# Jittor/PointCloudLib

Measured on AMD Instinct MI355X. Metric: point-clouds/sec fwd+bwd, PointNet++ SSG B=32 N=1024, higher is better.
Workload: dtype f32; 1 GPU; PointNet++ SSG cls train step (fwd+bwd+SGD), B=32/GPU, N=1024 xyz+normal, gauss_ball clouds (BASELINE configs[1]); global_batch=32, n_points=1024, parallelism=dp1, launch=eager, grad_overlap=False, cpu_affinity=numa node 1 (gpu0), 128 cpus, world_size=1, sync_bn=False, entry_points=per-stack (pcl_mlp_stack_*_f32)

## Files before the change

### include/pcl_hip.h

```cpp
#ifndef PCL_HIP_H
#define PCL_HIP_H

#include <stddef.h>
#include <stdint.h>

#ifdef __cplusplus
extern "C" {
#endif

#define PCL_OK 0
#define PCL_EINVAL (-1)
#define PCL_EHIP (-2)
#define PCL_ENOSUP (-3)
#define PCL_EWS (-4)

int pcl_version(void);
void pcl_time_tagged_launch(void* start_event, void* stop_event, const char* tag);
void pcl_time_next_launch(void* start_event, void* stop_event);
const char* pcl_last_launch_kernel(void);
const char* pcl_last_error(void);

int pcl_optimal_block(int batch_size);

void pcl_set_fps_tuning(int threads_per_cloud, int issue_priority);
int pcl_fps_f32(const float* xyz, int B, int N, int m, int tie_stride, double skip_sqnorm_le,
                const int32_t* start_idx, int32_t* idx_out, float* new_xyz_out, void* stream);

int pcl_fps_ragged_f32(const float* xyz, const int32_t* n_valid, int B, int N, int m, int tie_stride, double skip_sqnorm_le,
                       const int32_t* start_idx, int32_t* idx_out, float* new_xyz_out, void* stream);

int pcl_ball_query_f32(const float* new_xyz, const float* xyz, int B, int m, int N, float radius,
                       int nsample, int32_t* idx_out, int32_t* cnt_out, void* stream);
int pcl_ball_query_multi_f32(const float* new_xyz, const float* xyz, int B, int m, int N, int n_radii, const float* radii,
                             const int32_t* nsamples, int32_t* const* idx_out, int32_t* const* cnt_out, void* stream);
int pcl_ball_query_ragged_f32(const float* new_xyz, const float* xyz, const int32_t* n_valid, int B, int m, int N, float radius,
                              int nsample, int32_t* idx_out, int32_t* cnt_out, void* stream);
int pcl_ball_query_multi_ragged_f32(const float* new_xyz, const float* xyz, const int32_t* n_valid, int B, int m, int N, int n_radii,
                                    const float* radii, const int32_t* nsamples, int32_t* const* idx_out, int32_t* const* cnt_out,
                                    void* stream);

int pcl_group_f32(const float* xyz, const float* new_xyz, const float* feat, const int32_t* idx,
                  int B, int N, int m, int ns, int C, int use_xyz, float* out, void* stream);
int pcl_group_bwd_f32(const float* gout, const int32_t* idx, int B, int N, int m, int ns, int C,
                      int use_xyz, float* gfeat, void* stream);
int pcl_group_all_f32(const float* xyz, const float* feat, int B, int N, int C, int use_xyz,
                      float* out, void* stream);
int pcl_group_all_bwd_f32(const float* gout, int B, int N, int C, int use_xyz, float* gfeat,
                          void* stream);
int pcl_gather_rows_f32(const float* src, const int32_t* idx, int B, int N, int M, int C, float* out,
                        void* stream);
int pcl_gather_rows_bwd_f32(const float* gout, const int32_t* idx, int B, int N, int M, int C,
                            float* gsrc, void* stream);

int pcl_edge_feature_f32(const float* x, const int32_t* idx, int B, int N, int k, int C, float* out, void* stream);
int pcl_edge_feature_bwd_f32(const float* gout, const int32_t* idx, int B, int N, int k, int C, float* gx,
                             void* stream);

size_t pcl_knn_workspace_bytes(int B, int C, int Nr, int Nq, int k);
int pcl_knn_f32(const float* ref, const float* qry, int B, int C, int Nr, int Nq, int k,
                int32_t* idx_out, void* workspace, size_t workspace_bytes, void* stream);
int pcl_knn_nk_supported(int Nr);
int pcl_knn_nk_f32(const float* ref, const float* qry, int B, int C, int Nr, int Nq, int k, int32_t* idx_out, void* stream);
int pcl_knn_fma_f32(const float* ref, const float* qry, int B, int C, int Nr, int Nq, int k,
                    int32_t* idx_out, void* workspace, size_t workspace_bytes, void* stream);
int pcl_knn_point_matmul_f32(const float* xyz, const float* new_xyz, int B, int N, int S, int k, int fma_dot, int32_t* idx_out,
                             void* stream);

int pcl_three_nn_f32(const float* xyz1, const float* xyz2, int B, int N, int S, int32_t* idx3,
                     float* w3, void* stream);
int pcl_three_nn_ragged_f32(const float* xyz1, const int32_t* n1_valid, const float* xyz2, const int32_t* n2_valid, int B, int N,
                            int S, int32_t* idx3, float* w3, void* stream);
int pcl_three_interp_f32(const float* points2, const int32_t* idx3, const float* w3, int B, int N,
                         int S, int D, float* out, void* stream);
int pcl_three_interp_bwd_f32(const float* gout, const int32_t* idx3, const float* w3, int B, int N,
                             int S, int D, float* gpoints2, void* stream);

int pcl_density_f32(const float* xyz, int B, int N, float bandwidth, float* density_out, void* stream);

int pcl_group_linear_stat_rows(int B, int m);
int pcl_group_linear_f32(const float* xyz, const float* new_xyz, const float* Uf, const float* Wx, const float* feat_small,
                         const float* Wf_small, int CF, int ldw, const int32_t* idx, const int32_t* cnt, const int32_t* group_off,
                         int B, int N, int m, int ns, int C1, float* Y, int32_t* row_meta, int32_t* row_src,
                         float* row_loc , float* row_feat ,
                         double* stats_ws, void* stream);
int pcl_group_linear_bwd_f32(const float* row_loc, const float* row_feat, int CF, const float* dU, const float* Y,
                             const float* a, const float* k1, const float* k2, const float* mu, const int32_t* row_src,
                             const int32_t* n_rows_dev , int B, int N, int C1, float* dUf,
                             float* dWx_part, float* dWf_part, float* dW0, int ldw, int off, void* stream);
int pcl_group_rows_transpose_supported(int N, int m, int ns);
int pcl_group_rows_transpose_i32(const int32_t* row_src, const int32_t* group_off, int B, int N, int m, int ns, int32_t* in_off,
                                 int32_t* in_rows, void* stream);
int pcl_group_linear_bwd_gather_supported(int C1);
void pcl_set_pointconv_paths(int bwd_w_rows);
void pcl_set_scatter_form(int gather);
int pcl_group_linear_bwd_gather_f32(const float* row_loc, const float* dU, const float* Y, const float* a, const float* k1,
                                    const float* k2, const float* mu, const int32_t* in_off, const int32_t* in_rows, int B, int N,
                                    int C1, float* dUf, float* dWx_part, float* dW0, int ldw, void* stream);
int pcl_group_linear_bwd_regen_supported(int C1, int CF);
int pcl_group_linear_bwd_regen_f32(const float* row_loc, const float* row_feat, const float* Wx, const float* Wf_small, int CF, int ldw,
// ... 144 lines not shown
                            const int32_t* arg, const float* gz, int ns, const float* W, const float* Xprev,
                            const float* prev_scale, const float* prev_shift, float prev_slope, int masked, int P, int Cout, int Cin,
                            float* dUprev, double* stats_ws, int first_col, void* workspace, size_t workspace_bytes, void* stream);
int pcl_linear_bwd_pair_finish_f32(const void* workspace, size_t workspace_bytes, int P, int Cout, int Cin, float* dW, int dw_ld,
                                   const double* stats_ws, int stat_rows, const float* gamma_prev, const float* mean_prev,
                                   const float* invstd_prev, int P_bn, float* dgamma_prev, float* dbeta_prev,
                                   float* a_prev, float* k1_prev, float* k2_prev, float* dbias_zero_prev, void* stream);
void pcl_set_bwd_pair(int on);
int pcl_get_bwd_pair(void);
void pcl_set_matrix_form(int form);
int pcl_get_matrix_form(void);
int pcl_linear_bwd_fused_supported(int Cout, int Cin);
int pcl_linear_bwd_fused_stat_rows(int P, int Cin);
size_t pcl_linear_bwd_fused_workspace_bytes(int P, int Cout, int Cin);
int pcl_linear_bwd_fused_rows_f32(const float* dU, const float* Y, const float* a, const float* k1, const float* k2, const float* mu,
                                  const int32_t* arg, const float* gz, int ns, const float* W, int P, int Cout, int Cin,
                                  const float* Yprev, const float* prev_scale, const float* prev_shift, float prev_slope,
                                  float* dUprev, double* stats_ws, void* workspace, size_t workspace_bytes,
                                  const int32_t* row_meta, const int32_t* n_rows_dev, void* stream);
int pcl_linear_bwd_fused_finish_f32(const void* workspace, size_t workspace_bytes, int P, int Cout, int Cin, float* dW,
                                    const double* stats_ws, const float* gamma_prev, const float* mean_prev,
                                    const float* invstd_prev, int P_bn, float* dgamma_prev, float* dbeta_prev, float* a_prev,
                                    float* k1_prev, float* k2_prev, float* dbias_zero_prev, void* stream);
size_t pcl_linear_bwd_dw_workspace_bytes(int P, int Cout, int Cin);
int pcl_linear_bwd_dw_f32(const float* dU, const float* Y, const float* a, const float* k1, const float* k2, const float* mu,
                          const int32_t* arg, const float* gz, int ns, const float* Xprev,
                          const float* prev_scale, const float* prev_shift, float prev_slope, int P, int Cout,
                          int Cin, float* dW, void* workspace, size_t workspace_bytes, void* stream);

#define PCL_STACK_MAX_LAYERS 8
typedef struct pcl_stack_layer_t {
    const float* W;
    const float* bias;
    const float* gamma;
    const float* beta;
    float* running_mean;
    float* running_var;
    float* dW;
    float* dbias;
    float* dgamma;
    float* dbeta;
} pcl_stack_layer_t;
typedef struct pcl_mlp_stack_t {
    int32_t struct_bytes;
    int32_t n_layers;
    int32_t c[PCL_STACK_MAX_LAYERS + 1];
    int32_t P;
    int32_t pool;
    int32_t grouped;
    int32_t x_grad_from;
    int32_t need_dx;
    int32_t B, N, m, Cf, use_xyz;
    float slope, out_slope, eps, momentum;
    const float* x;
    const float* xyz;
    const float* new_xyz;
    const float* feature;
    float* Wf_dense;
    const int32_t* idx;
    const int32_t* cnt;
    const int32_t* group_off;
    pcl_stack_layer_t layer[PCL_STACK_MAX_LAYERS];
    float* out;
    void* save;
    size_t save_bytes;
    void* tmp;
    size_t tmp_bytes;
    const float* gout;
    float* dx;
    void* stream;
    int32_t defer_act;
    int32_t ext_stat_rows;
    const double* ext_stats;
    int32_t flush_k;
    int32_t gout_ld;
} pcl_mlp_stack_t;
int pcl_mlp_stack_last(const pcl_mlp_stack_t* desc, size_t* y_offset, size_t* scale_offset, size_t* shift_offset);
int pcl_mlp_stack_sizes(const pcl_mlp_stack_t* desc, size_t* save_bytes, size_t* fwd_tmp_bytes, size_t* bwd_tmp_bytes);
int pcl_mlp_stack_fwd_f32(const pcl_mlp_stack_t* desc);
int pcl_mlp_stack_bwd_f32(const pcl_mlp_stack_t* desc);

int pcl_frag_stat_rows(int P);
int pcl_frag_max_rows(void);
void pcl_frag_set_tuning(int max_rows, int force_tn, int force_ksw, int dw_tm, int dw_tn, int dw_ksw, int dw_ksg);
int pcl_frag_linear_fwd_f32(const float* X, int ldx, const float* W, int ldw, const float* bias, const float* in_scale,
                            const float* in_shift, float in_slope, int P, int Cin, int Cout, float* Y, int ldy,
                            float* Y_lo , double* stats_ws,
                            int flush_k, void* stream);
int pcl_frag_dy_f32(const float* dU, const float* Y, const float* a, const float* k1, const float* k2, const float* mu,
                    const int32_t* arg, const float* gz, int ns, int P, int C, float* dy, uint32_t* zero_words, int n_zero, void* stream);
int pcl_frag_linear_bwd_dx_f32(const float* dy, const float* W, int ldw, int P, int Cout, int Cin, const float* Yprev, int ldyp,
                               const float* prev_scale, const float* prev_shift, float prev_slope, float* dUprev, int ldu,
                               double* stats_ws, int first_col, void* stream);
size_t pcl_frag_dw_workspace_bytes(int P, int Cout, int Cin);
int pcl_frag_dw_counter_words(int P, int Cout, int Cin);
int pcl_frag_linear_bwd_dw_f32(const float* dy, const float* X, int ldx, const float* prev_scale, const float* prev_shift, float prev_slope,
                               int P, int Cout, int Cin, float* dW, int ldo, void* workspace, size_t workspace_bytes, int counters_cleared,
                               void* stream);

int pcl_group_offsets_i32(const int32_t* cnt, int G, int32_t* group_off, void* stream);
int pcl_group_offsets_multi_i32(int n, const int32_t* const* cnt, int G, int32_t* const* group_off, void* stream);
int pcl_group_compact_f32(const float* xyz, const float* new_xyz, const float* feat, const int32_t* idx,
                          const int32_t* cnt, const int32_t* group_off, int B, int N, int m, int ns, int C, int use_xyz,
                          int row_stride , float* rows,
                          int32_t* row_meta, int32_t* row_src, void* stream);
int pcl_linear_fwd_rows_f32(const float* X, const float* W, const float* bias, const float* in_scale,
                            const float* in_shift, float in_slope, int P, int Cin, int Cout, float* Y,
                            double* stats_ws, const int32_t* row_meta, const int32_t* n_rows_dev, void* stream);
int pcl_bn_act_max_rows_f32(const float* Y, const int32_t* group_off, const float* scale, const float* shift,
                            float slope, int G, int C, float* out, int32_t* arg, float* ymax, void* stream);
int pcl_linear_bwd_dx_rows_f32(const float* dU, const float* Y, const float* a, const float* k1, const float* k2, const float* mu,
                               const int32_t* arg, const float* gz, int ns, const float* W, int P, int Cout,
                               int Cin, const float* Yprev, const float* prev_scale, const float* prev_shift,
                               float prev_slope, float* dUprev, double* stats_ws, const int32_t* row_meta,
                               const int32_t* n_rows_dev, int first_col ,
                               int cin_stride , void* stream);
int pcl_linear_bwd_dw_rows_f32(const float* dU, const float* Y, const float* a, const float* k1, const float* k2, const float* mu,
                               const int32_t* arg, const float* gz, int ns, const float* Xprev,
                               const float* prev_scale, const float* prev_shift, float prev_slope, int P, int Cout,
                               int Cin, float* dW, void* workspace, size_t workspace_bytes, const int32_t* row_meta,
                               const int32_t* n_rows_dev, int dw_ld, void* stream);
int pcl_scatter_rows_add_f32(const float* grows, const int32_t* row_src, const int32_t* n_rows_dev, int rows_cap,
                             int D, int off, int C, int n_dst_rows, float* gfeat, void* stream);

int pcl_xconv_core_supported(int K, int dm, int C);
int pcl_xconv_core_partials(int R, int C);
int pcl_xconv_core_fwd_f32(const float* X, const float* F1, int C1, const float* F2, int C2, const float* wd, const float* bias,
                           int R, int K, int dm, float* D, void* stream);
int pcl_xconv_core_bwd_f32(const float* X, const float* F1, int C1, const float* F2, int C2, const float* wd, const float* dD,
                           int R, int K, int dm, float* dX, float* dF1, float* dF2, float* dwd_part, float* dbias_part,
// ... 57 lines not shown
```

### pointcloudlib_amd/csrc/group.hip

```cpp
#include "common.h"

namespace pcl {

__device__ __forceinline__ int in_cloud(int k, int N) { return min(max(k, 0), N - 1); }

constexpr int GT = 256;

__global__ __launch_bounds__(GT) void group_fwd_kernel(const float* __restrict__ xyz, const float* __restrict__ new_xyz,
                                                       const float* __restrict__ feat, const int32_t* __restrict__ idx,
                                                       int N, int m, int ns, int C, int use_xyz, size_t total,
                                                       float* __restrict__ out) {
    const int D = (use_xyz ? 3 : 0) + C;
    const int off = use_xyz ? 3 : 0;
    for (size_t g = (size_t)blockIdx.x * GT + threadIdx.x; g < total; g += (size_t)gridDim.x * GT) {
        const size_t row = g / D;
        const int c = (int)(g - row * D);
        const size_t bj = row / ns;
        const size_t b = bj / m;
        const int k = in_cloud(idx[row], N);
        float v;
        if (c < off) v = __fsub_rn(xyz[(b * N + k) * 3 + c], new_xyz[bj * 3 + c]);
        else v = feat[(b * N + k) * C + (c - off)];
        out[g] = v;
    }
}

__global__ __launch_bounds__(GT) void group_bwd_kernel(const float* __restrict__ gout, const int32_t* __restrict__ idx,
                                                       int N, int m, int ns, int C, int use_xyz, size_t total,
                                                       float* __restrict__ gfeat) {
    const int D = (use_xyz ? 3 : 0) + C;
    const int off = use_xyz ? 3 : 0;
    for (size_t g = (size_t)blockIdx.x * GT + threadIdx.x; g < total; g += (size_t)gridDim.x * GT) {
        const size_t row = g / C;
        const int c = (int)(g - row * C);
        const size_t b = row / ((size_t)m * ns);
        const int k = in_cloud(idx[row], N);
        unsafeAtomicAdd(&gfeat[(b * N + k) * C + c], gout[row * D + off + c]);
    }
}

__global__ __launch_bounds__(GT) void group_all_kernel(const float* __restrict__ xyz, const float* __restrict__ feat,
                                                       int C, int use_xyz, size_t total, float* __restrict__ out) {
    const int D = (use_xyz ? 3 : 0) + C;
    const int off = use_xyz ? 3 : 0;
    for (size_t g = (size_t)blockIdx.x * GT + threadIdx.x; g < total; g += (size_t)gridDim.x * GT) {
        const size_t p = g / D;
        const int c = (int)(g - p * D);
        out[g] = c < off ? xyz[p * 3 + c] : feat[p * C + (c - off)];
    }
}

__global__ __launch_bounds__(GT) void group_all_bwd_kernel(const float* __restrict__ gout, int C, int use_xyz,
                                                           size_t total, float* __restrict__ gfeat) {
    const int D = (use_xyz ? 3 : 0) + C;
    const int off = use_xyz ? 3 : 0;
    for (size_t g = (size_t)blockIdx.x * GT + threadIdx.x; g < total; g += (size_t)gridDim.x * GT) {
        const size_t p = g / C;
        const int c = (int)(g - p * C);
        gfeat[g] = gout[p * D + off + c];
    }
}

__global__ __launch_bounds__(GT) void gather_rows_kernel(const float* __restrict__ src, const int32_t* __restrict__ idx,
                                                         int N, int M, int C, size_t total, float* __restrict__ out) {
    for (size_t g = (size_t)blockIdx.x * GT + threadIdx.x; g < total; g += (size_t)gridDim.x * GT) {
        const size_t row = g / C;
        const int c = (int)(g - row * C);
        const size_t b = row / M;
        out[g] = src[(b * N + in_cloud(idx[row], N)) * C + c];
    }
}

__global__ __launch_bounds__(GT) void gather_rows_bwd_kernel(const float* __restrict__ gout, const int32_t* __restrict__ idx,
                                                             int N, int M, int C, size_t total, float* __restrict__ gsrc) {
    for (size_t g = (size_t)blockIdx.x * GT + threadIdx.x; g < total; g += (size_t)gridDim.x * GT) {
        const size_t row = g / C;
        const int c = (int)(g - row * C);
        const size_t b = row / M;
        unsafeAtomicAdd(&gsrc[(b * N + in_cloud(idx[row], N)) * C + c], gout[g]);
    }
}


__global__ __launch_bounds__(GT) void edge_feature_kernel(const float* __restrict__ x, const int32_t* __restrict__ idx,
                                                          int N, int k, int C, size_t total, float* __restrict__ out) {
    const int D = 2 * C;
    for (size_t g = (size_t)blockIdx.x * GT + threadIdx.x; g < total; g += (size_t)gridDim.x * GT) {
        const size_t row = g / D;
        const int c = (int)(g - row * D);
        const size_t bn = row / k;
        const size_t b = bn / N;
        if (c < C) out[g] = __fsub_rn(x[(b * N + in_cloud(idx[row], N)) * C + c], x[bn * C + c]);
        else out[g] = x[bn * C + (c - C)];
    }
}

__global__ __launch_bounds__(GT) void edge_feature_bwd_center_kernel(const float* __restrict__ gout, int k, int C,
                                                                     size_t total, float* __restrict__ gx) {
    const int D = 2 * C;
    for (size_t g = (size_t)blockIdx.x * GT + threadIdx.x; g < total; g += (size_t)gridDim.x * GT) {
        const size_t bn = g / C;
        const int c = (int)(g - bn * C);
        const float* base = gout + bn * k * D;
        float s = 0.f;
// ... 9 lines not shown
        const size_t row = g / C;
        const int c = (int)(g - row * C);
        const size_t b = row / ((size_t)N * k);
        unsafeAtomicAdd(&gx[(b * N + in_cloud(idx[row], N)) * C + c], gout[row * D + c]);
    }
}

static inline int grid_for(size_t total) {
    size_t blocks = (total + GT - 1) / GT;
    if (blocks > 256 * 16) blocks = 256 * 16;
    if (blocks < 1) blocks = 1;
    return (int)blocks;
}

}
using namespace pcl;

extern "C" int pcl_group_f32(const float* xyz, const float* new_xyz, const float* feat, const int32_t* idx, int B,
                             int N, int m, int ns, int C, int use_xyz, float* out, void* stream) {
    PCL_REQUIRE(idx && out, "pcl_group_f32: null pointer");
    PCL_REQUIRE(!use_xyz || (xyz && new_xyz), "pcl_group_f32: use_xyz needs xyz and new_xyz");
    PCL_REQUIRE(C == 0 || feat, "pcl_group_f32: C=%d needs feat", C);
    PCL_REQUIRE(B >= 0 && N >= 1 && m >= 0 && ns >= 1 && C >= 0 && (use_xyz || C > 0), "pcl_group_f32: bad sizes");
    const size_t total = (size_t)B * m * ns * ((use_xyz ? 3 : 0) + C);
    if (!total) return PCL_OK;
    hipLaunchKernelGGL(group_fwd_kernel, dim3(grid_for(total)), dim3(GT), 0, as_stream(stream), xyz, new_xyz, feat, idx,
                       N, m, ns, C, use_xyz, total, out);
    return check_launch("pcl_group_f32");
}

extern "C" int pcl_group_bwd_f32(const float* gout, const int32_t* idx, int B, int N, int m, int ns, int C,
                                 int use_xyz, float* gfeat, void* stream) {
    PCL_REQUIRE(gout && idx && gfeat, "pcl_group_bwd_f32: null pointer");
    PCL_REQUIRE(B >= 0 && N >= 1 && m >= 0 && ns >= 1 && C >= 1, "pcl_group_bwd_f32: bad sizes");
    hipStream_t st = as_stream(stream);
    if ((size_t)B * N * C) {
        hipError_t e = hipMemsetAsync(gfeat, 0, sizeof(float) * (size_t)B * N * C, st);
        if (e != hipSuccess) return fail(PCL_EHIP, "pcl_group_bwd_f32: memset: %s", hipGetErrorString(e));
    }
    const size_t total = (size_t)B * m * ns * C;
    if (!total) return PCL_OK;
    hipLaunchKernelGGL(group_bwd_kernel, dim3(grid_for(total)), dim3(GT), 0, st, gout, idx, N, m, ns, C, use_xyz, total, gfeat);
    return check_launch("pcl_group_bwd_f32");
}

extern "C" int pcl_group_all_f32(const float* xyz, const float* feat, int B, int N, int C, int use_xyz, float* out,
                                 void* stream) {
    PCL_REQUIRE(out && (!use_xyz || xyz) && (C == 0 || feat), "pcl_group_all_f32: null pointer");
    PCL_REQUIRE(B >= 0 && N >= 0 && C >= 0 && (use_xyz || C > 0), "pcl_group_all_f32: bad sizes");
    const size_t total = (size_t)B * N * ((use_xyz ? 3 : 0) + C);
    if (!total) return PCL_OK;
    hipLaunchKernelGGL(group_all_kernel, dim3(grid_for(total)), dim3(GT), 0, as_stream(stream), xyz, feat, C, use_xyz, total, out);
    return check_launch("pcl_group_all_f32");
}

extern "C" int pcl_group_all_bwd_f32(const float* gout, int B, int N, int C, int use_xyz, float* gfeat, void* stream) {
    PCL_REQUIRE(gout && gfeat && C >= 1 && B >= 0 && N >= 0, "pcl_group_all_bwd_f32: bad arguments");
    const size_t total = (size_t)B * N * C;
    if (!total) return PCL_OK;
    hipLaunchKernelGGL(group_all_bwd_kernel, dim3(grid_for(total)), dim3(GT), 0, as_stream(stream), gout, C, use_xyz, total, gfeat);
    return check_launch("pcl_group_all_bwd_f32");
}

extern "C" int pcl_gather_rows_f32(const float* src, const int32_t* idx, int B, int N, int M, int C, float* out,
                                   void* stream) {
    PCL_REQUIRE(src && idx && out && B >= 0 && N >= 1 && M >= 0 && C >= 1, "pcl_gather_rows_f32: bad arguments");
    const size_t total = (size_t)B * M * C;
    if (!total) return PCL_OK;
    hipLaunchKernelGGL(gather_rows_kernel, dim3(grid_for(total)), dim3(GT), 0, as_stream(stream), src, idx, N, M, C, total, out);
    return check_launch("pcl_gather_rows_f32");
}

extern "C" int pcl_gather_rows_bwd_f32(const float* gout, const int32_t* idx, int B, int N, int M, int C, float* gsrc,
                                       void* stream) {
    PCL_REQUIRE(gout && idx && gsrc && B >= 0 && N >= 1 && M >= 0 && C >= 1, "pcl_gather_rows_bwd_f32: bad arguments");
    hipStream_t st = as_stream(stream);
    if ((size_t)B * N * C) {
        hipError_t e = hipMemsetAsync(gsrc, 0, sizeof(float) * (size_t)B * N * C, st);
        if (e != hipSuccess) return fail(PCL_EHIP, "pcl_gather_rows_bwd_f32: memset: %s", hipGetErrorString(e));
    }
    const size_t total = (size_t)B * M * C;
    if (!total) return PCL_OK;
    hipLaunchKernelGGL(gather_rows_bwd_kernel, dim3(grid_for(total)), dim3(GT), 0, st, gout, idx, N, M, C, total, gsrc);
    return check_launch("pcl_gather_rows_bwd_f32");
}

extern "C" int pcl_edge_feature_f32(const float* x, const int32_t* idx, int B, int N, int k, int C, float* out, void* stream) {
    PCL_REQUIRE(x && idx && out && B >= 0 && N >= 1 && k >= 1 && C >= 1, "pcl_edge_feature_f32: bad arguments");
    const size_t total = (size_t)B * N * k * 2 * C;
    if (!total) return PCL_OK;
    hipLaunchKernelGGL(edge_feature_kernel, dim3(grid_for(total)), dim3(GT), 0, as_stream(stream), x, idx, N, k, C, total, out);
    return check_launch("pcl_edge_feature_f32");
}

extern "C" int pcl_edge_feature_bwd_f32(const float* gout, const int32_t* idx, int B, int N, int k, int C, float* gx,
                                        void* stream) {
    PCL_REQUIRE(gout && idx && gx && B >= 0 && N >= 1 && k >= 1 && C >= 1, "pcl_edge_feature_bwd_f32: bad arguments");
    hipStream_t st = as_stream(stream);
    const size_t tc = (size_t)B * N * C;
    if (!tc) return PCL_OK;
    hipLaunchKernelGGL(edge_feature_bwd_center_kernel, dim3(grid_for(tc)), dim3(GT), 0, st, gout, k, C, tc, gx);
    int rc = check_launch("pcl_edge_feature_bwd_f32(center)");
    if (rc) return rc;
    const size_t tn = tc * k;
    hipLaunchKernelGGL(edge_feature_bwd_nbr_kernel, dim3(grid_for(tn)), dim3(GT), 0, st, gout, idx, N, k, C, tn, gx);
    return check_launch("pcl_edge_feature_bwd_f32(nbr)");
// ... 2 lines not shown
```

### pointcloudlib_amd/csrc/mlp.hip

```cpp
#include <cstdlib>
#include "common.h"
#if defined(__HIP_DEVICE_COMPILE__) && !defined(__gfx950__)
#error "mlp.hip is written for gfx950 (MI355X) only: its buffer addressing relies on the range check covering the scalar offset (tools/ubench/bufcheck.hip)"
#endif

#ifndef PCL_EXP
#define PCL_EXP 0
#endif

namespace pcl {

typedef float f32x16 __attribute__((ext_vector_type(16)));

constexpr int BK = 32, LDS_LD = BK + 4;
constexpr int MLP_T = 256;
constexpr int STAT_ROWS = 1024;

enum AMode { A_PLAIN = 0, A_BNACT = 1, A_DY = 2, A_DY_SPARSE = 3 };
enum EMode { E_STORE_STATS = 0, E_MASK_STORE_STATS = 1, E_STORE = 2 };

struct LinArgs {
    const float* A;
    const float* A2;
    int ldb;
// ... 813 lines not shown
                    if (lh == 0 && cin && row0 < p.M) {
                        const size_t o = (size_t)(row0 / GM) * p.N + col;
                        p.gmax[o] = vmax; p.gmin[o] = vmin; p.gamax[o] = imax; p.gamin[o] = imin;
                    }
                }
            }
        }
    }

    if constexpr (EM != E_STORE) {
        __syncthreads();
        double* red = reinterpret_cast<double*>(sA);
#pragma unroll
        for (int tn = 0; tn < TN; ++tn) {
            double s = st_s[tn], q = st_q[tn];
            s += __shfl_xor(s, 32); q += __shfl_xor(q, 32);
            if (lh == 0) { red[((wave * TN + tn) * 32 + lr) * 2 + 0] = s; red[((wave * TN + tn) * 32 + lr) * 2 + 1] = q; }
        }
        __syncthreads();
        if (tid < TBN) {
            const int c = tid, wcc = c / (32 * TN), tn = (c >> 5) % TN, l = c & 31;
            const int col = n0 + c;
            if (col < p.N) {
                double s = 0.0, q = 0.0;
#pragma unroll
                for (int w = 0; w < 2; ++w) {
                    const int wv = w * 2 + wcc;
                    s += red[((wv * TN + tn) * 32 + l) * 2 + 0]; q += red[((wv * TN + tn) * 32 + l) * 2 + 1];
                }
                double* dst = p.stats + (size_t)bx * 2 * p.N;
                dst[col] = s; dst[p.N + col] = q;
            }
        }
    }
}
template <int AM, int EM, bool VEC, int TN, int GM, bool RAG, int TM = 2, bool SP = false>
__global__ __launch_bounds__(MLP_T, 2) void linear_nt_kernel(const LinArgs p_in) {
    linear_nt_body<AM, EM, VEC, TN, GM, RAG, TM, SP>(p_in, (int)blockIdx.x);
}

struct DwArgs {
    const float* A; const float* A2;
    const float* sc; const float* sh; const float* k2; const float* mu;
    const int32_t* arg; const float* gz; int ns;
    const float* Bsrc; const float* bsc; const float* bsh;
    float bslope;
    float* part;
    const int* p_dev;
    const int2* rmeta;
    int P, I, J;
    int a_mode, b_mode;
    int gx, ti, tj;
    int ldo;
};

constexpr int DW_BP = 32;

template <bool VEC, int W>
struct DwStage {
    static constexpr int CPR = VEC ? W / 4 : W;
    static constexpr int RP = MLP_T / CPR;
    static constexpr int NI = DW_BP / RP;
    float4 v[VEC ? NI : 1], v2[VEC ? NI : 1], vg[VEC ? NI : 1];
    int4 vi[VEC ? NI : 1];
    float s[VEC ? 1 : NI], s2[VEC ? 1 : NI], sg[VEC ? 1 : NI];
    int si[VEC ? 1 : NI];
    float rw[NI];
    int rs[NI];
    int2 raw[NI];
    int p0;
};

template <bool VEC, int W, bool RAG>
__device__ __forceinline__ void dw_fetch_meta(const DwArgs& p, int p0, int tid, DwStage<VEC, W>& st) {
    using S = DwStage<VEC, W>;
    if constexpr (RAG) {
#pragma unroll
        for (int i = 0; i < S::NI; ++i) st.raw[i] = p.rmeta[min(p0 + tid / S::CPR + S::RP * i, p.P - 1)];
    }
}

template <int AM, bool VEC, int W, bool RAG>
__device__ __forceinline__ void dw_load_a(const DwArgs& p, int p0, int c0, int tid, DwStage<VEC, W>& st) {
    using S = DwStage<VEC, W>;
    st.p0 = p0;
    const int c = min(c0 + (tid % S::CPR) * (VEC ? 4 : 1), p.I - (VEC ? 4 : 1));
#pragma unroll
    for (int i = 0; i < S::NI; ++i) {
        const int r = min(p0 + tid / S::CPR + S::RP * i, p.P - 1);
        const size_t off = (size_t)r * p.I + c;
        int g = 0, srow = 0;
        float w = 1.f;
        if constexpr (RAG) row_meta(st.raw[i], g, srow, w);
        else if constexpr (AM == A_DY_SPARSE) { g = r / p.ns; srow = r - g * p.ns; }
        st.rw[i] = w; st.rs[i] = srow;
        if constexpr (AM == A_PLAIN) {
            if constexpr (VEC) st.v[i] = *reinterpret_cast<const float4*>(p.A + off);
            else st.s[i] = p.A[off];
        } else if constexpr (VEC) {
            st.v2[i] = *reinterpret_cast<const float4*>(p.A2 + off);
            if constexpr (AM == A_DY) st.v[i] = *reinterpret_cast<const float4*>(p.A + off);
            else {
                const size_t go = (size_t)g * p.I + c;
                st.vi[i] = *reinterpret_cast<const int4*>(p.arg + go);
                st.vg[i] = *reinterpret_cast<const float4*>(p.gz + go);
            }
// ... 8 lines not shown
        }
    }
}

template <int AM, bool VEC, int W>
__device__ __forceinline__ void dw_store_a(const DwArgs& p, float* sX, int c0, int tid, const DwStage<VEC, W>& st,
                                           float4 sc, float4 sh, float4 k2, float4 mu) {
    using S = DwStage<VEC, W>;
    const int cl = (tid % S::CPR) * (VEC ? 4 : 1);
    const bool cin = c0 + cl < p.I;
#pragma unroll
    for (int i = 0; i < S::NI; ++i) {
        const int rl = tid / S::CPR + S::RP * i;
        const int r = st.p0 + rl;
        const bool in = cin && r < p.P;
        if constexpr (AM == A_PLAIN) {
            if constexpr (VEC) *reinterpret_cast<float4*>(&sX[rl * (W + 4) + cl]) = in ? st.v[i] : make_float4(0, 0, 0, 0);
            else sX[rl * (W + 4) + cl] = in ? st.s[i] : 0.f;
        } else if constexpr (VEC) {
            float4 a = make_float4(0, 0, 0, 0);
            if (in) {
                float4 du;
                if constexpr (AM == A_DY) du = st.v[i];
                else {
                    const int srow = st.rs[i];
                    const int4 ar = st.vi[i];
                    const float4 gz = st.vg[i];
                    du.x = ar.x == srow ? gz.x : 0.f; du.y = ar.y == srow ? gz.y : 0.f;
                    du.z = ar.z == srow ? gz.z : 0.f; du.w = ar.w == srow ? gz.w : 0.f;
                }
                const float4 y = st.v2[i];
                const float w = st.rw[i];
                a.x = fmaf(sc.x, du.x, -w * fmaf(k2.x, y.x - mu.x, sh.x)); a.y = fmaf(sc.y, du.y, -w * fmaf(k2.y, y.y - mu.y, sh.y));
                a.z = fmaf(sc.z, du.z, -w * fmaf(k2.z, y.z - mu.z, sh.z)); a.w = fmaf(sc.w, du.w, -w * fmaf(k2.w, y.w - mu.w, sh.w));
            }
            *reinterpret_cast<float4*>(&sX[rl * (W + 4) + cl]) = a;
        } else {
            float a = 0.f;
            if (in) {
                float du;
                if constexpr (AM == A_DY) du = st.s[i];
                else du = st.si[i] == st.rs[i] ? st.sg[i] : 0.f;
                a = fmaf(sc.x, du, -st.rw[i] * fmaf(k2.x, st.s2[i] - mu.x, sh.x));
            }
            sX[rl * (W + 4) + cl] = a;
        }
    }
}

template <bool VEC, int W>
__device__ __forceinline__ void dw_load_b(const DwArgs& p, int p0, int c0, int tid, DwStage<VEC, W>& st) {
    using S = DwStage<VEC, W>;
    st.p0 = p0;
    const int c = min(c0 + (tid % S::CPR) * (VEC ? 4 : 1), p.J - (VEC ? 4 : 1));
#pragma unroll
    for (int i = 0; i < S::NI; ++i) {
        const int r = min(p0 + tid / S::CPR + S::RP * i, p.P - 1);
        const size_t off = (size_t)r * p.J + c;
        if constexpr (VEC) st.v[i] = *reinterpret_cast<const float4*>(p.Bsrc + off);
        else st.s[i] = p.Bsrc[off];
    }
}

template <bool VEC, int W>
__device__ __forceinline__ void dw_store_b(const DwArgs& p, float* sX, int c0, int tid, const DwStage<VEC, W>& st,
                                           float4 sc, float4 sh) {
    using S = DwStage<VEC, W>;
    const int cl = (tid % S::CPR) * (VEC ? 4 : 1);
    const bool cin = c0 + cl < p.J;
    const bool act = p.b_mode == A_BNACT;
#pragma unroll
    for (int i = 0; i < S::NI; ++i) {
        const int rl = tid / S::CPR + S::RP * i;
        const bool in = cin && st.p0 + rl < p.P;
        if constexpr (VEC) {
            float4 b = make_float4(0, 0, 0, 0);
            if (in) {
                b = st.v[i];
                if (act) {
                    b.x = lrelu(fmaf(sc.x, b.x, sh.x), p.bslope); b.y = lrelu(fmaf(sc.y, b.y, sh.y), p.bslope);
                    b.z = lrelu(fmaf(sc.z, b.z, sh.z), p.bslope); b.w = lrelu(fmaf(sc.w, b.w, sh.w), p.bslope);
                }
            }
            *reinterpret_cast<float4*>(&sX[rl * (W + 4) + cl]) = b;
        } else {
            float b = 0.f;
            if (in) { b = st.s[i]; if (act) b = lrelu(fmaf(sc.x, b, sh.x), p.bslope); }
            sX[rl * (W + 4) + cl] = b;
        }
    }
}

template <int AM, bool VEC, int TM, int TN, bool RAG>
__device__ __forceinline__ void linear_dw_body(const DwArgs& p_in, const int block) {
    DwArgs p = p_in;
    if (p.p_dev) p.P = *p.p_dev;
    constexpr int WI = 64 * TM, WJ = 64 * TN;
    __shared__ __attribute__((aligned(16))) float sA[DW_BP * (WI + 4)];
    __shared__ __attribute__((aligned(16))) float sB[DW_BP * (WJ + 4)];
    const int tid = threadIdx.x, lane = tid & 63, wave = tid >> 6;
    const int wr = wave >> 1, wc = wave & 1, lr = lane & 31, lh = lane >> 5;
    int bx, bt;
    tile_of_block(block, p.gx, p.ti * p.tj, bx, bt);
    const int i0 = (bt % p.ti) * WI, j0 = (bt / p.ti) * WJ;
    const int chunks = (p.P + DW_BP - 1) / DW_BP;
    f32x16 acc[TM][TN];
#pragma unroll
    for (int i = 0; i < TM; ++i)
#pragma unroll
        for (int j = 0; j < TN; ++j)
#pragma unroll
// ... 1658 lines not shown
            else PCL_LAUNCH_TIMED((linear_nt_kernel<AM, EM, false, 1, 0, false, 1>), grid, dim3(MLP_T), st, a);
            return check_launch("pcl_linear");
        }
    }
    if (narrow || AM >= A_DY) {
        if (vec) PCL_LAUNCH_TIMED((linear_nt_kernel<AM, EM, true, 1, GM, RAG>), grid, dim3(MLP_T), st, a);
        else if constexpr (AM == A_DY_SPARSE && RAG && GM == 0) {
            PCL_LAUNCH_TIMED((linear_nt_kernel<AM, EM, false, 1, GM, RAG, 1>), grid, dim3(MLP_T), st, a);
        } else PCL_LAUNCH_TIMED((linear_nt_kernel<AM, EM, false, 1, GM, RAG>), grid, dim3(MLP_T), st, a);
    } else {
        if constexpr (AM < A_DY) {
            if (vec) PCL_LAUNCH_TIMED((linear_nt_kernel<AM, EM, true, 2, GM, RAG>), grid, dim3(MLP_T), st, a);
            else PCL_LAUNCH_TIMED((linear_nt_kernel<AM, EM, false, 2, GM, RAG>), grid, dim3(MLP_T), st, a);
        }
    }
    return check_launch("pcl_linear");
}

static int linear_stat_rows(int M, int N, bool bwd, bool rag) {
    int gx, n_tiles; bool narrow, low;
    linear_grid(M, N, bwd, rag, gx, n_tiles, narrow, low);
    return gx;
}

static int launch_linear(const LinArgs& a, hipStream_t st) {
    if (fwd_res_eligible(a)) return launch_fwd_res(a, linear_stat_rows(a.M, a.N, false, a.rmeta != nullptr), st);
    if (a.rmeta) {
        if (a.a_mode == A_PLAIN && a.e_mode == E_STORE_STATS) return launch_linear_t<A_PLAIN, E_STORE_STATS, 0, true>(a, st);
        if (a.a_mode == A_BNACT && a.e_mode == E_STORE_STATS) return launch_linear_t<A_BNACT, E_STORE_STATS, 0, true>(a, st);
        if (a.a_mode == A_DY && a.e_mode == E_MASK_STORE_STATS) return launch_linear_t<A_DY, E_MASK_STORE_STATS, 0, true>(a, st);
        if (a.a_mode == A_DY && a.e_mode == E_STORE) return launch_linear_t<A_DY, E_STORE, 0, true>(a, st);
        if (a.a_mode == A_DY_SPARSE && a.e_mode == E_MASK_STORE_STATS) return launch_linear_t<A_DY_SPARSE, E_MASK_STORE_STATS, 0, true>(a, st);
        if (a.a_mode == A_DY_SPARSE && a.e_mode == E_STORE) return launch_linear_t<A_DY_SPARSE, E_STORE, 0, true>(a, st);
        return fail(PCL_EINVAL, "pcl_linear: unsupported ragged mode combination %d/%d", a.a_mode, a.e_mode);
    }
    if (a.e_mode == E_STORE_STATS && a.gmax) {
        if (a.a_mode == A_PLAIN && a.ns == 64) return launch_linear_t<A_PLAIN, E_STORE_STATS, 64>(a, st);
        if (a.a_mode == A_BNACT && a.ns == 64) return launch_linear_t<A_BNACT, E_STORE_STATS, 64>(a, st);
        if (a.a_mode == A_PLAIN && a.ns == 32) return launch_linear_t<A_PLAIN, E_STORE_STATS, 32>(a, st);
        if (a.a_mode == A_BNACT && a.ns == 32) return launch_linear_t<A_BNACT, E_STORE_STATS, 32>(a, st);
        return fail(PCL_EINVAL, "pcl_linear_fwd_gmax_f32: group size %d not supported (32 or 64)", a.ns);
    }
    if (a.a_mode == A_PLAIN && a.e_mode == E_STORE_STATS) return launch_linear_t<A_PLAIN, E_STORE_STATS>(a, st);
    if (a.a_mode == A_BNACT && a.e_mode == E_STORE_STATS) return launch_linear_t<A_BNACT, E_STORE_STATS>(a, st);
    if (a.a_mode == A_PLAIN && a.e_mode == E_STORE) return launch_linear_t<A_PLAIN, E_STORE>(a, st);
    if (a.a_mode == A_BNACT && a.e_mode == E_STORE) return launch_linear_t<A_BNACT, E_STORE>(a, st);
    if (a.a_mode == A_DY && a.e_mode == E_MASK_STORE_STATS) return launch_linear_t<A_DY, E_MASK_STORE_STATS>(a, st);
    if (a.a_mode == A_DY && a.e_mode == E_STORE) return launch_linear_t<A_DY, E_STORE>(a, st);
    if (a.a_mode == A_DY_SPARSE && a.e_mode == E_MASK_STORE_STATS) return launch_linear_t<A_DY_SPARSE, E_MASK_STORE_STATS>(a, st);
    if (a.a_mode == A_DY_SPARSE && a.e_mode == E_STORE) return launch_linear_t<A_DY_SPARSE, E_STORE>(a, st);
    return fail(PCL_EINVAL, "pcl_linear: unsupported mode combination %d/%d", a.a_mode, a.e_mode);
}

}
using namespace pcl;

extern "C" int pcl_mlp_stat_rows(int P, int C, int flags) {
    if (P < 1 || C < 1) return 1;
    return linear_stat_rows(P, C, (flags & 1) != 0, (flags & 2) != 0);
}

extern "C" int pcl_linear_fwd_rows_f32(const float* X, const float* W, const float* bias, const float* in_scale,
                                       const float* in_shift, float in_slope, int P, int Cin, int Cout, float* Y,
                                       double* stats_ws, const int32_t* row_meta, const int32_t* n_rows_dev, void* stream) {
    PCL_REQUIRE(X && W && Y, "pcl_linear_fwd_f32: null pointer");
    PCL_REQUIRE(stats_ws || !row_meta, "pcl_linear_fwd_rows_f32: the stats-free form (stats_ws NULL) takes plain rows only");
    PCL_REQUIRE(P >= 1 && Cin >= 1 && Cout >= 1, "pcl_linear_fwd_f32: bad sizes P=%d Cin=%d Cout=%d", P, Cin, Cout);
    PCL_REQUIRE((in_scale == nullptr) == (in_shift == nullptr), "pcl_linear_fwd_f32: in_scale/in_shift must come together");
    PCL_REQUIRE((row_meta == nullptr) == (n_rows_dev == nullptr), "pcl_linear_fwd_rows_f32: row_meta and n_rows_dev come together");
    LinArgs a = {};
    a.A = X; a.B = W; a.bias = bias; a.sc = in_scale; a.sh = in_shift; a.slope = in_slope;
    a.C = Y; a.stats = stats_ws; a.M = P; a.N = Cout; a.K = Cin; a.ldc = Cout;
    a.rmeta = reinterpret_cast<const int2*>(row_meta); a.m_dev = n_rows_dev;
    a.a_mode = in_scale ? A_BNACT : A_PLAIN; a.e_mode = stats_ws ? E_STORE_STATS : E_STORE;
    return launch_linear(a, as_stream(stream));
}

extern "C" int pcl_linear_fwd_f32(const float* X, const float* W, const float* bias, const float* in_scale,
                                  const float* in_shift, float in_slope, int P, int Cin, int Cout, float* Y,
                                  double* stats_ws, void* stream) {
    return pcl_linear_fwd_rows_f32(X, W, bias, in_scale, in_shift, in_slope, P, Cin, Cout, Y, stats_ws, nullptr, nullptr, stream);
}

extern "C" int pcl_linear_fwd_gmax_f32(const float* X, const float* W, const float* bias, const float* in_scale,
                                       const float* in_shift, float in_slope, int P, int Cin, int Cout, int ns, float* Y,
                                       double* stats_ws, float* gmax, float* gmin, int32_t* gamax, int32_t* gamin,
                                       void* stream) {
    PCL_REQUIRE(X && W && Y && stats_ws && gmax && gmin && gamax && gamin, "pcl_linear_fwd_gmax_f32: null pointer");
    PCL_REQUIRE(P >= 1 && Cin >= 1 && Cout >= 1 && (ns == 32 || ns == 64) && P % ns == 0,
                "pcl_linear_fwd_gmax_f32: bad sizes P=%d Cin=%d Cout=%d ns=%d (ns must be 32 or 64 and divide P)", P, Cin, Cout, ns);
    PCL_REQUIRE((in_scale == nullptr) == (in_shift == nullptr), "pcl_linear_fwd_gmax_f32: in_scale/in_shift must come together");
    LinArgs a = {};
    a.A = X; a.B = W; a.bias = bias; a.sc = in_scale; a.sh = in_shift; a.slope = in_slope;
    a.C = Y; a.stats = stats_ws; a.M = P; a.N = Cout; a.K = Cin; a.ldc = Cout; a.ns = ns;
    a.gmax = gmax; a.gmin = gmin; a.gamax = gamax; a.gamin = gamin;
    a.a_mode = in_scale ? A_BNACT : A_PLAIN; a.e_mode = E_STORE_STATS;
    return launch_linear(a, as_stream(stream));
}

__global__ __launch_bounds__(256) void group_minmax_finalize_t_kernel(const float* __restrict__ gmax, const float* __restrict__ gmin,
                                                                      const int32_t* __restrict__ gamax, const int32_t* __restrict__ gamin,
                                                                      const float* __restrict__ scale, const float* __restrict__ shift,
                                                                      float slope, int C, int N, int tiles_c, size_t tiles, float* __restrict__ out,
                                                                      int32_t* __restrict__ arg, float* __restrict__ ymax,
                                                                      float* __restrict__ out2, int ld2, float* __restrict__ out_t) {
    __shared__ float tile[32][33];
// ... 23 lines not shown
        const size_t b = g0 / N, n0 = g0 % N;
#pragma unroll
        for (int i = 0; i < 4; ++i) {
            const int cl = ty + 8 * i;
            if (c0 + cl < C) out_t[(b * C + c0 + cl) * (size_t)N + n0 + tx] = tile[tx][cl];
        }
        __syncthreads();
    }
}

extern "C" int pcl_group_minmax_finalize_t_f32(const float* gmax, const float* gmin, const int32_t* gamax, const int32_t* gamin,
                                               const float* scale, const float* shift, float slope, int B, int N, int C, float* out,
                                               int32_t* arg, float* ymax, float* out2, int out2_ld, float* out_t, void* stream) {
    PCL_REQUIRE(gmax && gmin && gamax && gamin && scale && shift && out && arg && ymax && out_t && B >= 1 && N >= 32 && N % 32 == 0 && C >= 1 &&
                (!out2 || out2_ld >= C), "pcl_group_minmax_finalize_t_f32: bad arguments (N a multiple of 32)");
    const int tiles_c = (C + 31) / 32;
    const size_t tiles = (size_t)B * N / 32 * tiles_c;
    const int blocks = tiles < 8192 ? (int)tiles : 8192;
    hipLaunchKernelGGL(group_minmax_finalize_t_kernel, dim3(blocks), dim3(256), 0, as_stream(stream), gmax, gmin, gamax, gamin, scale, shift, slope, C, N,
                       tiles_c, tiles, out, arg, ymax, out2, out2_ld, out_t);
    return check_launch("pcl_group_minmax_finalize_t_f32");
}
extern "C" int pcl_group_minmax_finalize_f32(const float* gmax, const float* gmin, const int32_t* gamax, const int32_t* gamin,
                                             const float* scale, const float* shift, float slope, int G, int C, float* out,
                                             int32_t* arg, float* ymax, void* stream) {
    return pcl_group_minmax_finalize2_f32(gmax, gmin, gamax, gamin, scale, shift, slope, G, C, out, arg, ymax, nullptr, 0, stream);
}
extern "C" int pcl_group_minmax_finalize2_f32(const float* gmax, const float* gmin, const int32_t* gamax, const int32_t* gamin,
                                              const float* scale, const float* shift, float slope, int G, int C, float* out,
                                              int32_t* arg, float* ymax, float* out2, int out2_ld, void* stream) {
    PCL_REQUIRE(gmax && gmin && gamax && gamin && scale && shift && out && arg && ymax && G >= 1 && C >= 1 && (!out2 || out2_ld >= C),
                "pcl_group_minmax_finalize_f32: bad arguments");
    const size_t total = (size_t)G * C;
    int blocks = (int)((total + 255) / 256);
    if (blocks > 4096) blocks = 4096;
    hipLaunchKernelGGL(group_minmax_finalize_kernel, dim3(blocks), dim3(256), 0, as_stream(stream), gmax, gmin, gamax, gamin, scale,
                       shift, slope, C, total, out, arg, ymax, out2, out2_ld);
    return check_launch("pcl_group_minmax_finalize_f32");
}

extern "C" int pcl_linear_bwd_dx_f32(const float* dU, const float* Y, const float* a_, const float* k1, const float* k2, const float* mu,
                                     const int32_t* arg, const float* gz, int ns, const float* W, int P, int Cout,
                                     int Cin, const float* Yprev, const float* prev_scale, const float* prev_shift,
                                     float prev_slope, float* dUprev, double* stats_ws, void* stream) {
    return pcl_linear_bwd_dx_rows_f32(dU, Y, a_, k1, k2, mu, arg, gz, ns, W, P, Cout, Cin, Yprev, prev_scale, prev_shift, prev_slope,
                                      dUprev, stats_ws, nullptr, nullptr, 0, 0, stream);
}

extern "C" int pcl_linear_bwd_dx_rows_f32(const float* dU, const float* Y, const float* a_, const float* k1, const float* k2, const float* mu,
                                          const int32_t* arg, const float* gz, int ns, const float* W, int P, int Cout,
                                          int Cin, const float* Yprev, const float* prev_scale, const float* prev_shift,
                                          float prev_slope, float* dUprev, double* stats_ws, const int32_t* row_meta,
                                          const int32_t* n_rows_dev, int first_col, int cin_stride, void* stream) {
    PCL_REQUIRE(Y && a_ && k1 && k2 && mu && W && dUprev, "pcl_linear_bwd_dx_f32: null pointer");
    PCL_REQUIRE((dU != nullptr) != (arg != nullptr && gz != nullptr), "pcl_linear_bwd_dx_f32: pass dU or (arg,gz)");
    PCL_REQUIRE(P >= 1 && Cin >= 1 && Cout >= 1 && (dU || ns >= 1), "pcl_linear_bwd_dx_f32: bad sizes");
    PCL_REQUIRE(!Yprev || (prev_scale && prev_shift && stats_ws), "pcl_linear_bwd_dx_f32: masked mode needs scale/shift/stats");
    LinArgs a = {};
    a.A = dU; a.A2 = Y; a.B = W; a.sc = a_; a.sh = k1; a.k2 = k2; a.mu = mu; a.arg = arg; a.gz = gz; a.ns = ns;
    a.C = dUprev; a.stats = stats_ws; a.Yprev = Yprev; a.esc = prev_scale; a.esh = prev_shift; a.eslope = prev_slope;
    PCL_REQUIRE(first_col >= 0 && first_col < Cin && (first_col == 0 || !Yprev), "pcl_linear_bwd_dx_rows_f32: first_col=%d only for the input gradient", first_col);
    a.M = P; a.N = Cin; a.K = Cout; a.n_begin = first_col; a.ldc = a.ldb = cin_stride > 0 ? cin_stride : Cin;
    PCL_REQUIRE(a.ldc >= Cin && (a.ldc == Cin || !Yprev), "pcl_linear_bwd_dx_rows_f32: cin_stride=%d", cin_stride);
    a.rmeta = reinterpret_cast<const int2*>(row_meta); a.m_dev = n_rows_dev;
    a.a_mode = dU ? A_DY : A_DY_SPARSE; a.e_mode = Yprev ? E_MASK_STORE_STATS : E_STORE;
    return launch_linear(a, as_stream(stream));
}

extern "C" size_t pcl_linear_bwd_dw_workspace_bytes(int P, int Cout, int Cin) {
    if (P < 1 || Cout < 1 || Cin < 1) return 0;
    int gx, ti, tj, tm, tn;
    dw_grid(P, Cout, Cin, gx, ti, tj, tm, tn);
    return sizeof(float) * (size_t)gx * Cout * Cin;
}

extern "C" int pcl_linear_bwd_dw_f32(const float* dU, const float* Y, const float* a_, const float* k1, const float* k2, const float* mu,
                                     const int32_t* arg, const float* gz, int ns, const float* Xprev,
                                     const float* prev_scale, const float* prev_shift, float prev_slope, int P, int Cout,
                                     int Cin, float* dW, void* workspace, size_t workspace_bytes, void* stream) {
    return pcl_linear_bwd_dw_rows_f32(dU, Y, a_, k1, k2, mu, arg, gz, ns, Xprev, prev_scale, prev_shift, prev_slope, P, Cout, Cin, dW,
                                      workspace, workspace_bytes, nullptr, nullptr, 0, stream);
}

extern "C" int pcl_linear_bwd_dw_rows_f32(const float* dU, const float* Y, const float* a_, const float* k1, const float* k2, const float* mu,
                                          const int32_t* arg, const float* gz, int ns, const float* Xprev,
                                          const float* prev_scale, const float* prev_shift, float prev_slope, int P, int Cout,
                                          int Cin, float* dW, void* workspace, size_t workspace_bytes, const int32_t* row_meta,
                                          const int32_t* n_rows_dev, int dw_ld, void* stream) {
    PCL_REQUIRE(Y && a_ && k1 && k2 && mu && Xprev && dW, "pcl_linear_bwd_dw_f32: null pointer");
    PCL_REQUIRE(dw_ld == 0 || dw_ld >= Cin, "pcl_linear_bwd_dw_f32: dw_ld=%d < Cin=%d", dw_ld, Cin);
    PCL_REQUIRE((dU != nullptr) != (arg != nullptr && gz != nullptr), "pcl_linear_bwd_dw_f32: pass dU or (arg,gz)");
    PCL_REQUIRE((prev_scale == nullptr) == (prev_shift == nullptr), "pcl_linear_bwd_dw_f32: scale/shift together");
    PCL_REQUIRE(P >= 1 && Cin >= 1 && Cout >= 1 && (dU || ns >= 1), "pcl_linear_bwd_dw_f32: bad sizes");
    const size_t need = pcl_linear_bwd_dw_workspace_bytes(P, Cout, Cin);
    if (!workspace || workspace_bytes < need) return fail(PCL_EWS, "pcl_linear_bwd_dw_f32: workspace %zu < %zu", workspace_bytes, need);
    hipStream_t st = as_stream(stream);
    int gx, ti, tj, tm, tn;
    dw_grid(P, Cout, Cin, gx, ti, tj, tm, tn);
    DwArgs d = {};
    d.A = dU; d.A2 = Y; d.sc = a_; d.sh = k1; d.k2 = k2; d.mu = mu; d.arg = arg; d.gz = gz; d.ns = ns;
    d.Bsrc = Xprev; d.bsc = prev_scale; d.bsh = prev_shift; d.bslope = prev_slope;
    d.part = static_cast<float*>(workspace); d.P = P; d.I = Cout; d.J = Cin;
    d.rmeta = reinterpret_cast<const int2*>(row_meta); d.p_dev = n_rows_dev;
    d.a_mode = dU ? A_DY : A_DY_SPARSE; d.b_mode = prev_scale ? A_BNACT : A_PLAIN;
    const bool vec = (Cout % 4 == 0) && (Cin % 4 == 0) && al16(Y, Xprev, dU) && (!gz || al16(gz, arg));
    d.gx = gx; d.ti = ti; d.tj = tj; d.ldo = Cin;
    const bool direct = gx == 1;
    if (direct) { d.part = dW; d.ldo = dw_ld ? dw_ld : Cin; }
    dim3 grid(gx * ti * tj);
    if (dU) { if (vec) launch_dw_t<A_DY, true>(d, grid, tm, tn, st); else launch_dw_t<A_DY, false>(d, grid, tm, tn, st); }
    else { if (vec) launch_dw_t<A_DY_SPARSE, true>(d, grid, tm, tn, st); else launch_dw_t<A_DY_SPARSE, false>(d, grid, tm, tn, st); }
    int rc = check_launch("pcl_linear_bwd_dw_f32");
    if (rc || direct) return rc;
    const size_t n = (size_t)Cout * Cin;
    const int blocks = (int)((n + 31) / 32);
    hipLaunchKernelGGL(reduce_rows_kernel, dim3(blocks), dim3(256), 0, st, d.part, gx, n, Cin, dw_ld ? dw_ld : Cin, dW);
    return check_launch("pcl_linear_bwd_dw_f32(reduce)");
}

extern "C" int pcl_linear_bwd_pair_supported(int P, int Cout, int Cin, int first_col) {
    if (!g_lab.bwd_pair || P < 1 || Cout <= 64 || Cin <= 64 || (g_lab.split_mfma & 2)) return 0;
    int gx, ti, tj, tm, tn;
    dw_grid(P, Cout, Cin, gx, ti, tj, tm, tn);
    if (gx == 1 || tm != 2 || tn != 2) return 0;
    int gxl, n_tiles; bool narrow, low;
    linear_grid(P, Cin - first_col, true, false, gxl, n_tiles, narrow, low);
    return low ? 1 : 0;
}

extern "C" int pcl_linear_bwd_pair_f32(const float* dU, const float* Y, const float* a_, const float* k1, const float* k2, const float* mu,
                                       const int32_t* arg, const float* gz, int ns, const float* W, const float* Xprev,
                                       const float* prev_scale, const float* prev_shift, float prev_slope, int masked, int P, int Cout, int Cin,
                                       float* dUprev, double* stats_ws, int first_col, void* workspace, size_t workspace_bytes, void* stream) {
    PCL_REQUIRE(Y && a_ && k1 && k2 && mu && W && Xprev && dUprev, "pcl_linear_bwd_pair_f32: null pointer");
    PCL_REQUIRE((dU != nullptr) != (arg != nullptr && gz != nullptr), "pcl_linear_bwd_pair_f32: pass dU or (arg,gz)");
    PCL_REQUIRE((prev_scale == nullptr) == (prev_shift == nullptr), "pcl_linear_bwd_pair_f32: scale/shift together");
    PCL_REQUIRE(!masked || (prev_scale && stats_ws), "pcl_linear_bwd_pair_f32: masked mode needs scale/shift/stats");
    PCL_REQUIRE(first_col >= 0 && first_col < Cin && (first_col == 0 || !masked), "pcl_linear_bwd_pair_f32: first_col=%d only for the input gradient", first_col);
    PCL_REQUIRE(pcl_linear_bwd_pair_supported(P, Cout, Cin, first_col), "pcl_linear_bwd_pair_f32: shape P=%d Cout=%d Cin=%d not eligible", P, Cout, Cin);
    const size_t need = pcl_linear_bwd_dw_workspace_bytes(P, Cout, Cin);
    if (!workspace || workspace_bytes < need) return fail(PCL_EWS, "pcl_linear_bwd_pair_f32: workspace %zu < %zu", workspace_bytes, need);
    hipStream_t st = as_stream(stream);
    int gx, ti, tj, tm, tn;
    dw_grid(P, Cout, Cin, gx, ti, tj, tm, tn);
    DwArgs d = {};
    d.A = dU; d.A2 = Y; d.sc = a_; d.sh = k1; d.k2 = k2; d.mu = mu; d.arg = arg; d.gz = gz; d.ns = ns;
    d.Bsrc = Xprev; d.bsc = prev_scale; d.bsh = prev_shift; d.bslope = prev_slope;
    d.part = static_cast<float*>(workspace); d.P = P; d.I = Cout; d.J = Cin;
    d.a_mode = dU ? A_DY : A_DY_SPARSE; d.b_mode = prev_scale ? A_BNACT : A_PLAIN;
    d.gx = gx; d.ti = ti; d.tj = tj; d.ldo = Cin;
    LinArgs a = {};
    a.A = dU; a.A2 = Y; a.B = W; a.sc = a_; a.sh = k1; a.k2 = k2; a.mu = mu; a.arg = arg; a.gz = gz; a.ns = ns;
    a.C = dUprev; a.stats = stats_ws; a.Yprev = masked ? Xprev : nullptr; a.esc = prev_scale; a.esh = prev_shift; a.eslope = prev_slope;
    a.M = P; a.N = Cin; a.K = Cout; a.n_begin = first_col; a.ldc = a.ldb = Cin;
    a.a_mode = d.a_mode; a.e_mode = masked ? E_MASK_STORE_STATS : E_STORE;
    int gxl, n_tiles; bool narrow, low;
    linear_grid(P, Cin - first_col, true, false, gxl, n_tiles, narrow, low);
    a.gx = gxl; a.nt = n_tiles;
    const bool vec_dw = (Cout % 4 == 0) && (Cin % 4 == 0) && al16(Y, Xprev, dU) && (!gz || al16(gz, arg));
    const bool vec_nt = (a.K % 4 == 0) && al16(a.A, a.B, a.A2) && a.ldb % 4 == 0;
    const int n_dw = gx * ti * tj;
    if (vec_dw != vec_nt) {
        if (dU) { if (vec_dw) launch_dw_t<A_DY, true>(d, dim3(n_dw), tm, tn, st); else launch_dw_t<A_DY, false>(d, dim3(n_dw), tm, tn, st); }
        else { if (vec_dw) launch_dw_t<A_DY_SPARSE, true>(d, dim3(n_dw), tm, tn, st); else launch_dw_t<A_DY_SPARSE, false>(d, dim3(n_dw), tm, tn, st); }
        if (const int rc = check_launch("pcl_linear_bwd_pair_f32(dw)")) return rc;
        return launch_linear(a, st);
    }
    const bool vec = vec_dw;
    const dim3 grid(n_dw + gxl * n_tiles), blk(MLP_T);
#define PCL_PAIR(AMv, EMv, VECv) PCL_LAUNCH_TIMED((linear_bwd_pair_kernel<AMv, EMv, VECv>), grid, blk, st, d, a, n_dw)
    if (dU) {
        if (masked) { if (vec) PCL_PAIR(A_DY, E_MASK_STORE_STATS, true); else PCL_PAIR(A_DY, E_MASK_STORE_STATS, false); }
        else { if (vec) PCL_PAIR(A_DY, E_STORE, true); else PCL_PAIR(A_DY, E_STORE, false); }
    } else {
        if (masked) { if (vec) PCL_PAIR(A_DY_SPARSE, E_MASK_STORE_STATS, true); else PCL_PAIR(A_DY_SPARSE, E_MASK_STORE_STATS, false); }
        else { if (vec) PCL_PAIR(A_DY_SPARSE, E_STORE, true); else PCL_PAIR(A_DY_SPARSE, E_STORE, false); }
    }
#undef PCL_PAIR
    return check_launch("pcl_linear_bwd_pair_f32");
}

namespace pcl {
int pair_finish_impl(const void* workspace, size_t workspace_bytes, int P, int Cout, int Cin, float* dW, int dw_ld,
                     const double* stats_ws, int stat_rows, const float* gamma_prev, const float* mean_prev,
                     const float* invstd_prev, int P_bn, float* dgamma_prev, float* dbeta_prev,
                     float* a_prev, float* k1_prev, float* k2_prev, float* dbias_zero_prev, void* stream,
                     const float* xpart, int xrows, int xC1, int xld, float* xdW0);
}
extern "C" int pcl_linear_bwd_pair_finish_f32(const void* workspace, size_t workspace_bytes, int P, int Cout, int Cin, float* dW, int dw_ld,
                                              const double* stats_ws, int stat_rows, const float* gamma_prev, const float* mean_prev,
                                              const float* invstd_prev, int P_bn, float* dgamma_prev, float* dbeta_prev,
                                              float* a_prev, float* k1_prev, float* k2_prev, float* dbias_zero_prev, void* stream) {
    return pair_finish_impl(workspace, workspace_bytes, P, Cout, Cin, dW, dw_ld, stats_ws, stat_rows, gamma_prev, mean_prev, invstd_prev, P_bn, dgamma_prev,
                            dbeta_prev, a_prev, k1_prev, k2_prev, dbias_zero_prev, stream, nullptr, 0, 0, 0, nullptr);
}
int pcl::pair_finish_impl(const void* workspace, size_t workspace_bytes, int P, int Cout, int Cin, float* dW, int dw_ld,
                          const double* stats_ws, int stat_rows, const float* gamma_prev, const float* mean_prev,
                          const float* invstd_prev, int P_bn, float* dgamma_prev, float* dbeta_prev,
                          float* a_prev, float* k1_prev, float* k2_prev, float* dbias_zero_prev, void* stream,
                          const float* xpart, int xrows, int xC1, int xld, float* xdW0) {
    PCL_REQUIRE(workspace && dW && P >= 1 && Cout >= 1 && Cin >= 1 && (dw_ld == 0 || dw_ld >= Cin), "pcl_linear_bwd_pair_finish_f32: bad arguments");
    const size_t need = pcl_linear_bwd_dw_workspace_bytes(P, Cout, Cin);
    if (workspace_bytes < need) return fail(PCL_EWS, "pcl_linear_bwd_pair_finish_f32: workspace %zu < %zu", workspace_bytes, need);
    int gx, ti, tj, tm, tn;
    dw_grid(P, Cout, Cin, gx, ti, tj, tm, tn);
    BnConstsArgs q = {};
    int extra = 0;
    if (stats_ws) {
        PCL_REQUIRE(mean_prev && invstd_prev && a_prev && k1_prev && k2_prev && P_bn >= 1 && stat_rows >= 1, "pcl_linear_bwd_pair_finish_f32: null pointer");
        q = BnConstsArgs{stats_ws, stat_rows, gamma_prev, mean_prev, invstd_prev, P_bn, Cin, dgamma_prev, dbeta_prev, a_prev, k1_prev, k2_prev, dbias_zero_prev};
        extra = (Cin + 3) / 4;
    }
    const size_t n = (size_t)Cout * Cin;
    const int nred = (int)((n + 31) / 32);
    FinishXJob xj = {nullptr, 0, 0, 0, nullptr, 0};
    int xblocks = 0;
    if (xpart && xdW0) { xj = FinishXJob{xpart, xrows, xC1, xld, xdW0, nred + extra}; xblocks = (xC1 * 3 + 3) / 4; }
    hipLaunchKernelGGL(fused_finish_kernel, dim3(nred + extra + xblocks), dim3(256), 0, as_stream(stream), static_cast<const float*>(workspace), gx, n, Cin, dW, nred, q,
                       dw_ld, xj);
    return check_launch("pcl_linear_bwd_pair_finish_f32");
}

extern "C" int pcl_bn_bwd_dy_supported(int P, int C) { return P >= 1 && C >= 32 && C % 32 == 0; }

extern "C" int pcl_bn_bwd_dy_f32(const double* stats_ws, int stat_rows, const float* gamma, const float* mean, const float* invstd, int P_bn, int C,
                                 float* dgamma, float* dbeta, float* a_out, float* k1, float* k2, float* dbias_zero, const float* dU, const float* Y,
                                 const int32_t* arg, const float* gz, int ns, int P, float* dy, void* stream) {
    PCL_REQUIRE(stats_ws && mean && invstd && a_out && k1 && k2 && Y && dy, "pcl_bn_bwd_dy_f32: null pointer");
    PCL_REQUIRE(stat_rows >= 1 && P_bn >= 1 && pcl_bn_bwd_dy_supported(P, C), "pcl_bn_bwd_dy_f32: bad sizes P=%d C=%d (C must be a multiple of 32) stat_rows=%d", P, C, stat_rows);
    PCL_REQUIRE((dU != nullptr) != (arg != nullptr && gz != nullptr), "pcl_bn_bwd_dy_f32: pass dU or (arg, gz)");
    PCL_REQUIRE(dU || ns >= 1, "pcl_bn_bwd_dy_f32: ns = %d", ns);
    PCL_REQUIRE(al16(Y, dy, dU) && (!gz || al16(gz, arg)), "pcl_bn_bwd_dy_f32: operands must be 16-byte aligned");
    BnDyArgs a = {};
    a.q = BnConstsArgs{stats_ws, stat_rows, gamma, mean, invstd, P_bn, C, dgamma, dbeta, a_out, k1, k2, dbias_zero};
    a.dU = dU; a.Y = Y; a.arg = arg; a.gz = gz; a.ns = ns; a.dy = dy; a.M = P;
    const int cg = C / 32;
    int rs = (512 + cg - 1) / cg;
    if (rs > (P + 63) / 64) rs = (P + 63) / 64;
    if (rs < 1) rs = 1;
    hipLaunchKernelGGL(bn_bwd_dy_kernel, dim3(cg, rs), dim3(256), 0, as_stream(stream), a);
    return check_launch("pcl_bn_bwd_dy_f32");
}

static void dw_plain_grid(int P, int I, int J, int& gx, int& ti, int& tj, int& tm, int& tn) {
    dw_grid(P, I, J, gx, ti, tj, tm, tn);
    if (g_lab.dw_force_gx) {
        const int chunks = (P + DW_BP - 1) / DW_BP;
        gx = g_lab.dw_force_gx < chunks ? g_lab.dw_force_gx : chunks;
    }
}
extern "C" size_t pcl_linear_bwd_dw_plain_workspace_bytes(int P, int Cout, int Cin) {
    if (P < 1 || Cout < 1 || Cin < 1) return 0;
    int gx, ti, tj, tm, tn;
    dw_plain_grid(P, Cout, Cin, gx, ti, tj, tm, tn);
    return sizeof(float) * (size_t)gx * Cout * Cin;
}
extern "C" int pcl_linear_bwd_dw_plain_f32(const float* dy, const float* Xprev, const float* prev_scale, const float* prev_shift, float prev_slope, int P,
                                           int Cout, int Cin, float* dW, void* workspace, size_t workspace_bytes, int dw_ld, void* stream) {
    PCL_REQUIRE(dy && Xprev && dW, "pcl_linear_bwd_dw_plain_f32: null pointer");
    PCL_REQUIRE(dw_ld == 0 || dw_ld >= Cin, "pcl_linear_bwd_dw_plain_f32: dw_ld=%d < Cin=%d", dw_ld, Cin);
    PCL_REQUIRE((prev_scale == nullptr) == (prev_shift == nullptr), "pcl_linear_bwd_dw_plain_f32: scale/shift together");
    PCL_REQUIRE(P >= 1 && Cin >= 1 && Cout >= 1, "pcl_linear_bwd_dw_plain_f32: bad sizes");
    const size_t need = pcl_linear_bwd_dw_plain_workspace_bytes(P, Cout, Cin);
    if (!workspace || workspace_bytes < need) return fail(PCL_EWS, "pcl_linear_bwd_dw_plain_f32: workspace %zu < %zu", workspace_bytes, need);
    hipStream_t st = as_stream(stream);
    int gx, ti, tj, tm, tn;
    dw_plain_grid(P, Cout, Cin, gx, ti, tj, tm, tn);
    DwArgs d = {};
    d.A = dy; d.Bsrc = Xprev; d.bsc = prev_scale; d.bsh = prev_shift; d.bslope = prev_slope;
    d.part = static_cast<float*>(workspace); d.P = P; d.I = Cout; d.J = Cin;
    d.a_mode = A_PLAIN; d.b_mode = prev_scale ? A_BNACT : A_PLAIN;
    const bool vec = (Cout % 4 == 0) && (Cin % 4 == 0) && al16(dy, Xprev);
    d.gx = gx; d.ti = ti; d.tj = tj; d.ldo = Cin;
    const bool direct = gx == 1;
    if (direct) { d.part = dW; d.ldo = dw_ld ? dw_ld : Cin; }
    dim3 grid(gx * ti * tj);
    if (vec) launch_dw_t2<A_PLAIN, true, false>(d, grid, tm, tn, st); else launch_dw_t2<A_PLAIN, false, false>(d, grid, tm, tn, st);
    int rc = check_launch("pcl_linear_bwd_dw_plain_f32");
    if (rc || direct) return rc;
    const size_t n = (size_t)Cout * Cin;
    const int blocks = (int)((n + 31) / 32);
    hipLaunchKernelGGL(reduce_rows_kernel, dim3(blocks), dim3(256), 0, st, d.part, gx, n, Cin, dw_ld ? dw_ld : Cin, dW);
    return check_launch("pcl_linear_bwd_dw_plain_f32(reduce)");
}

extern "C" int pcl_linear_bwd_fused_supported(int Cout, int Cin) {
    return ((Cout == 64 || Cout == 128) && (Cin == 64 || Cin == 128)) || (Cout == 256 && Cin == 128);
}
extern "C" int pcl_linear_bwd_fused_stat_rows(int P, int Cin) { return P < 1 ? 1 : fb_grid(P, Cin); }
extern "C" size_t pcl_linear_bwd_fused_workspace_bytes(int P, int Cout, int Cin) {
    if (P < 1 || Cout < 1 || Cin < 1) return 0;
    return sizeof(float) * (size_t)fb_grid(P, Cin) * fb_ksplit(Cout, Cin) * Cout * Cin;
}

template <bool SPARSE, bool RAG>
static int launch_fb(const FbArgs& a_in, int Cout, int Cin, hipStream_t st) {
#if PCL_EXP == 7
    FbArgs a = a_in;
    {
        static int n_launch[2][8][8];
        a.lab_slot = n_launch[SPARSE][Cout / 64][Cin / 64]++;
    }
#else
    const FbArgs& a = a_in;
#endif
    const dim3 grid(a.gx), blk(FB_T);
#define PCL_FB(CO, CI) PCL_LAUNCH_TIMED((linear_bwd_fused_kernel<SPARSE, RAG, CO, CI>), grid, blk, st, a)
    if (Cout == 64 && Cin == 64) PCL_FB(1, 1);
    else if (Cout == 64 && Cin == 128) PCL_FB(1, 2);
    else if (Cout == 128 && Cin == 64) {
        if (g_lab.fb_two) PCL_LAUNCH_TIMED((linear_bwd_fused_kernel<SPARSE, RAG, 2, 1, true>), grid, blk, st, a);
        else PCL_FB(2, 1);
    }
    else if (Cout == 128 && Cin == 128) PCL_FB(2, 2);
    else PCL_FB(4, 2);
#undef PCL_FB
    return check_launch("pcl_linear_bwd_fused_rows_f32");
}

extern "C" int pcl_linear_bwd_fused_rows_f32(const float* dU, const float* Y, const float* a_, const float* k1, const float* k2, const float* mu,
                                             const int32_t* arg, const float* gz, int ns, const float* W, int P, int Cout, int Cin,
                                             const float* Yprev, const float* prev_scale, const float* prev_shift, float prev_slope,
                                             float* dUprev, double* stats_ws, void* workspace, size_t workspace_bytes,
                                             const int32_t* row_meta, const int32_t* n_rows_dev, void* stream) {
    PCL_REQUIRE(Y && a_ && k1 && k2 && mu && W && Yprev && prev_scale && prev_shift && dUprev && stats_ws, "pcl_linear_bwd_fused_rows_f32: null pointer");
    PCL_REQUIRE((dU != nullptr) != (arg != nullptr && gz != nullptr), "pcl_linear_bwd_fused_rows_f32: pass dU or (arg,gz)");
// ... 186 lines not shown
```

### pointcloudlib_amd/csrc/stack.hip

```cpp
#include "common.h"
#include <string.h>

namespace pcl {

static inline size_t al256(size_t n) { return (n + 255) & ~(size_t)255; }

struct Carver {
    char* base; size_t off;
    explicit Carver(void* p) : base(static_cast<char*>(p)), off(0) {}
    template <typename T> T* take(size_t count) {
        T* r = base ? reinterpret_cast<T*>(base + off) : nullptr;
        off += al256(count * sizeof(T));
        return r;
    }
};

struct SaveLayout {
    float* Y[PCL_STACK_MAX_LAYERS];
    float* vec[PCL_STACK_MAX_LAYERS];
    int32_t* arg; float* ymax;
    int32_t* row_meta; int32_t* row_src; float* row_loc; float* row_feat;
    int32_t* in_off; int32_t* in_rows;
    float* Uf;
    size_t bytes;
// ... 128 lines not shown
    size_t wsb = 0;
    for (int l = 0; l < L; ++l) {
        if (l == 0 && d.grouped) continue;
        const int cin = d.c[l], cout = d.c[l + 1];
        size_t b = pcl_linear_bwd_dw_workspace_bytes(d.P, cout, cin);
        if (fewrow_layer(d, l)) {
            const size_t f = pcl_linear_bwd_dw_plain_workspace_bytes(d.P, cout, cin);
            if (f > b) b = f;
        }
        if (l > 0 && pcl_linear_bwd_fused_supported(cout, cin)) {
            const size_t f = pcl_linear_bwd_fused_workspace_bytes(d.P, cout, cin);
            if (f > b) b = f;
        }
        if (b > wsb) wsb = b;
    }
    t.ws_bytes = wsb;
    t.ws = c.take<float>((wsb + 3) / 4);
    for (int l = 0; l < L; ++l)
        if (fewrow_layer(d, l)) t.dy_l[l] = c.take<float>((size_t)d.P * d.c[l + 1]);
    if (side_dw(d)) {
        for (int l = 0; l < L; ++l) {
            t.consts_l[l] = c.take<float>((size_t)3 * d.c[l + 1]);
            if (l < L - 1 || !G) t.dU_l[l] = c.take<float>((size_t)d.P * d.c[l + 1]);
        }
    }
    if (d.grouped) {
        const int rows = pcl_group_linear_stat_rows(d.B, d.m), C1 = d.c[1];
        if (grouped_wide(d)) {
            t.dUf = c.take<float>(((size_t)d.B * d.N * C1 + 3) / 4 * 4);
            t.unit = c.take<float>((size_t)3 * C1);
            t.ptws_bytes = pcl_linear_bwd_dw_workspace_bytes(d.B * d.N, C1, d.Cf);
            t.ptws = c.take<float>((t.ptws_bytes + 3) / 4);
        }
        if (d.use_xyz) t.dWxp = c.take<float>((size_t)rows * C1 * 3);
        if (grouped_inline(d)) t.dWfp = c.take<float>((size_t)rows * C1 * d.Cf);
    }
    t.bytes = c.off;
    return t;
}

bool narrow_supported(const pcl_mlp_stack_t& d);
size_t narrow_save_bytes();
size_t narrow_fwd_tmp_bytes();
size_t narrow_bwd_tmp_bytes();
int narrow_fwd(const pcl_mlp_stack_t& d);
int narrow_bwd(const pcl_mlp_stack_t& d);
int maxgrad_prep_impl(const float* gout, const float* out, const float* ymax, float slope, int G, int C, float* gz, double* stats_ws,
                      int* stat_rows_out, void* stream, float* zero, size_t n_zero, float* ones, int n_one, int n_one0, int ldg);
int pair_finish_impl(const void* workspace, size_t workspace_bytes, int P, int Cout, int Cin, float* dW, int dw_ld,
                     const double* stats_ws, int stat_rows, const float* gamma_prev, const float* mean_prev,
                     const float* invstd_prev, int P_bn, float* dgamma_prev, float* dbeta_prev,
                     float* a_prev, float* k1_prev, float* k2_prev, float* dbias_zero_prev, void* stream,
                     const float* xpart, int xrows, int xC1, int xld, float* xdW0);
int group_linear_fwd_impl(const float* xyz, const float* new_xyz, const float* Uf, const float* Wx, const float* feat_small,
                          const float* Wf_small, int CF, int ldw, const int32_t* idx, const int32_t* cnt, const int32_t* group_off, int B,
                          int N, int m, int ns, int C1, float* Y, int32_t* row_meta, int32_t* row_src, float* row_loc, float* row_feat,
                          double* stats_ws, void* stream, int phase, const float* dense_src, float* dense_dst, int dense_cols);
int group_linear_bwd_impl(const float* row_loc, const float* row_feat, int CF, const float* dU, const float* Y, const float* a,
                          const float* k1, const float* k2, const float* mu, const int32_t* row_src, const int32_t* n_rows_dev, int B, int N,
                          int C1, float* dUf, float* dWx_part, float* dWf_part, float* dW0, int ldw, int off, void* stream, bool duf_is_zero);

__global__ __launch_bounds__(256) void aux_fill_kernel(float4* zero, size_t n4, float* ones, int n_one, int n_zero) {
    for (size_t e = (size_t)blockIdx.x * 256 + threadIdx.x; e < n4; e += (size_t)gridDim.x * 256) zero[e] = make_float4(0.f, 0.f, 0.f, 0.f);
    if (blockIdx.x == 0 && ones)
        for (int e = threadIdx.x; e < n_one + n_zero; e += 256) ones[e] = e < n_one ? 1.f : 0.f;
}

static int validate(const pcl_mlp_stack_t* dp, const char* who) {
    PCL_REQUIRE(dp, "%s: null descriptor", who);
    const pcl_mlp_stack_t& d = *dp;
    PCL_REQUIRE(d.struct_bytes == (int32_t)sizeof(pcl_mlp_stack_t), "%s: descriptor is %d bytes, this library expects %zu (header mismatch)",
                who, d.struct_bytes, sizeof(pcl_mlp_stack_t));
    PCL_REQUIRE(d.n_layers >= 1 && d.n_layers <= PCL_STACK_MAX_LAYERS, "%s: n_layers=%d (1..%d)", who, d.n_layers, PCL_STACK_MAX_LAYERS);
    PCL_REQUIRE(d.P >= 1, "%s: P=%d", who, d.P);
    for (int l = 0; l <= d.n_layers; ++l) PCL_REQUIRE(d.c[l] >= 1, "%s: c[%d]=%d", who, l, d.c[l]);
    PCL_REQUIRE(d.pool >= 0 && (d.pool == 0 || d.grouped || d.P % d.pool == 0), "%s: pool=%d does not divide P=%d", who, d.pool, d.P);
    PCL_REQUIRE(!d.defer_act || d.pool == 0 || d.grouped, "%s: defer_act: a plain stack must have no max (a grouped one keeps its rows: no pooling)", who);
    if (d.grouped) {
        PCL_REQUIRE(d.n_layers >= 2, "%s: a grouped stack needs >= 2 layers (the folded layer's gradient arrives dense from the second)", who);
        PCL_REQUIRE(d.B >= 1 && d.N >= 1 && d.m >= 1 && d.pool >= 1 && d.P == d.B * d.m * d.pool, "%s: grouped: P=%d must be B*m*ns = %d*%d*%d", who, d.P, d.B, d.m, d.pool);
        PCL_REQUIRE(d.idx && d.cnt && d.group_off && d.xyz && d.new_xyz, "%s: grouped: null index / coordinate pointer", who);
        PCL_REQUIRE(d.Cf >= 0 && (d.Cf == 0 || d.feature), "%s: grouped: Cf=%d without features", who, d.Cf);
        PCL_REQUIRE(d.use_xyz || d.Cf > 0, "%s: grouped: neither coordinates nor features", who);
        PCL_REQUIRE(d.c[0] == (d.use_xyz ? 3 : 0) + d.Cf, "%s: grouped: c[0]=%d must be the first layer's fan-in %d", who, d.c[0], (d.use_xyz ? 3 : 0) + d.Cf);
        PCL_REQUIRE(!grouped_wide(d) || d.Wf_dense, "%s: grouped: wide features need Wf_dense", who);
        PCL_REQUIRE(!d.layer[0].bias || grouped_wide(d), "%s: grouped: a conv bias of the folded first layer rides in the per-point product (wide features only)", who);
    } else {
        PCL_REQUIRE(d.x, "%s: null input", who);
    }
    for (int l = 0; l < d.n_layers; ++l)
        PCL_REQUIRE(d.layer[l].W && d.layer[l].gamma && d.layer[l].beta, "%s: layer %d: W / gamma / beta must be given (training-mode BatchNorm on every layer)", who, l);
    PCL_REQUIRE(d.flush_k == 0 || d.flush_k == 8 || d.flush_k == 32, "%s: flush_k = %d (0, 8 or 32)", who, d.flush_k);
    return PCL_OK;
}

#define PCL_TRY(expr) do { int rc_ = (expr); if (rc_) return rc_; } while (0)

static void tagf(const char* fmt, int a, int b) {
    char buf[32];
    snprintf(buf, sizeof buf, fmt, a, b);
    set_launch_tag(buf);
}

struct PadItem { const float* src; float* dst; int rows, cols, lds, ldd, rows_p, cols_p; };
constexpr int PAD_ITEMS = PCL_STACK_MAX_LAYERS * 6;
struct PadTable {
// ... 11 lines not shown
}
static int launch_pad(const PadTable& t, void* st) {
    if (t.n == 0) return PCL_OK;
    hipLaunchKernelGGL(pad_copy_kernel, dim3(16, t.n), dim3(256), 0, as_stream(st), t);
    return check_launch("pcl_mlp_stack(pad)");
}
static inline int padded_width(const pcl_mlp_stack_t& d, int l) {
    if (l >= 1 && l < d.n_layers && d.c[l] == 96 && d.P >= 32768 && !d.defer_act) return 128;
    return d.c[l];
}
struct PadPlan {
    bool on;
    int cp[PCL_STACK_MAX_LAYERS + 1];
    size_t w_off[PCL_STACK_MAX_LAYERS], v_off[PCL_STACK_MAX_LAYERS], save_floats;
    size_t dw_off[PCL_STACK_MAX_LAYERS], dv_off[PCL_STACK_MAX_LAYERS], bwd_floats;
    bool wpad[PCL_STACK_MAX_LAYERS], opad[PCL_STACK_MAX_LAYERS];
};
static PadPlan pad_plan(const pcl_mlp_stack_t& d) {
    PadPlan p = {};
    const int L = d.n_layers;
    for (int l = 0; l <= L; ++l) { p.cp[l] = padded_width(d, l); p.on = p.on || p.cp[l] != d.c[l]; }
    if (!p.on) return p;
    size_t so = 0, bo = 0;
    auto take = [](size_t& o, size_t n) { const size_t r = o; o += (n + 63) & ~(size_t)63; return r; };
    for (int l = 0; l < L; ++l) {
        p.opad[l] = p.cp[l + 1] != d.c[l + 1];
        p.wpad[l] = p.opad[l] || p.cp[l] != d.c[l];
        if (p.wpad[l]) { p.w_off[l] = take(so, (size_t)p.cp[l + 1] * p.cp[l]); p.dw_off[l] = take(bo, (size_t)p.cp[l + 1] * p.cp[l]); }
        if (p.opad[l]) { p.v_off[l] = take(so, (size_t)5 * p.cp[l + 1]); p.dv_off[l] = take(bo, (size_t)3 * p.cp[l + 1]); }
    }
    p.save_floats = so; p.bwd_floats = bo;
    return p;
}
static pcl_mlp_stack_t padded_desc(const pcl_mlp_stack_t& d, const PadPlan& p, float* save_x, float* bwd_x) {
    pcl_mlp_stack_t q = d;
    const int L = d.n_layers;
    for (int l = 0; l <= L; ++l) q.c[l] = p.cp[l];
    for (int l = 0; l < L; ++l) {
        pcl_stack_layer_t& y = q.layer[l];
        if (p.wpad[l]) { y.W = save_x + p.w_off[l]; y.dW = bwd_x ? bwd_x + p.dw_off[l] : nullptr; }
        if (p.opad[l]) {
            float* v = save_x + p.v_off[l];
            const int cp = p.cp[l + 1];
            y.gamma = v; y.beta = v + cp;
            y.running_mean = d.layer[l].running_mean ? v + 2 * cp : nullptr; y.running_var = d.layer[l].running_var ? v + 3 * cp : nullptr;
            y.bias = d.layer[l].bias ? v + 4 * cp : nullptr;
            if (bwd_x) { float* g = bwd_x + p.dv_off[l]; y.dgamma = g; y.dbeta = g + cp; y.dbias = d.layer[l].bias ? g + 2 * cp : nullptr; }
            else { y.dgamma = y.dbeta = y.dbias = nullptr; }
        }
    }
    return q;
}

}
using namespace pcl;

static int stack_sizes_impl(const pcl_mlp_stack_t* d, size_t* save_bytes, size_t* fwd_tmp_bytes, size_t* bwd_tmp_bytes);
static int stack_fwd_impl(const pcl_mlp_stack_t* dp);
static int stack_bwd_impl(const pcl_mlp_stack_t* dp);

extern "C" int pcl_mlp_stack_sizes(const pcl_mlp_stack_t* d, size_t* save_bytes, size_t* fwd_tmp_bytes, size_t* bwd_tmp_bytes) {
    PCL_TRY(validate(d, "pcl_mlp_stack_sizes"));
    const PadPlan p = narrow_supported(*d) ? PadPlan{} : pad_plan(*d);
    if (!p.on) return stack_sizes_impl(d, save_bytes, fwd_tmp_bytes, bwd_tmp_bytes);
    const pcl_mlp_stack_t q = padded_desc(*d, p, reinterpret_cast<float*>(uintptr_t(4096)), reinterpret_cast<float*>(uintptr_t(4096)));
    size_t sv = 0, ft = 0, bt = 0;
    PCL_TRY(stack_sizes_impl(&q, &sv, &ft, &bt));
    if (save_bytes) *save_bytes = al256(sv) + p.save_floats * 4;
    if (fwd_tmp_bytes) *fwd_tmp_bytes = ft;
    if (bwd_tmp_bytes) *bwd_tmp_bytes = al256(bt) + p.bwd_floats * 4;
    return PCL_OK;
}

extern "C" int pcl_mlp_stack_fwd_f32(const pcl_mlp_stack_t* dp) {
    PCL_TRY(validate(dp, "pcl_mlp_stack_fwd_f32"));
    const pcl_mlp_stack_t& d = *dp;
    const PadPlan p = narrow_supported(d) ? PadPlan{} : pad_plan(d);
    if (!p.on) return stack_fwd_impl(dp);
    PCL_REQUIRE(d.save && d.tmp, "pcl_mlp_stack_fwd_f32: null save / tmp");
    size_t sv = 0, ft = 0, bt = 0;
    pcl_mlp_stack_t q = padded_desc(d, p, nullptr, nullptr);
    {
        pcl_mlp_stack_t probe = padded_desc(d, p, reinterpret_cast<float*>(uintptr_t(4096)), nullptr);
        PCL_TRY(stack_sizes_impl(&probe, &sv, &ft, &bt));
    }
    if (d.save_bytes < al256(sv) + p.save_floats * 4) return fail(PCL_EWS, "pcl_mlp_stack_fwd_f32: save %zu < %zu", d.save_bytes, al256(sv) + p.save_floats * 4);
    float* sx = reinterpret_cast<float*>(static_cast<char*>(d.save) + al256(sv));
    q = padded_desc(d, p, sx, nullptr);
    q.save_bytes = sv;
    PadTable t = {};
    const int L = d.n_layers;
    for (int l = 0; l < L; ++l) {
        const pcl_stack_layer_t& y = d.layer[l];
        bool ok = true;
        if (p.wpad[l]) ok = t.push(PadItem{y.W, sx + p.w_off[l], d.c[l + 1], d.c[l], d.c[l], p.cp[l], p.cp[l + 1], p.cp[l]}) && ok;
        if (p.opad[l]) {
            float* v = sx + p.v_off[l];
            const int c = d.c[l + 1], cp = p.cp[l + 1];
            const float* srcs[5] = {y.gamma, y.beta, y.running_mean, y.running_var, y.bias};
            for (int k = 0; k < 5; ++k) if (srcs[k]) ok = t.push(PadItem{srcs[k], v + (size_t)k * cp, 1, c, c, cp, 1, cp}) && ok;
        }
        PCL_REQUIRE(ok, "pcl_mlp_stack_fwd_f32: more padded layers than the pad table holds");
    }
    PCL_TRY(launch_pad(t, d.stream));
    PCL_TRY(stack_fwd_impl(&q));
    PadTable u = {};
    for (int l = 0; l < L; ++l) {
        if (!p.opad[l]) continue;
        const pcl_stack_layer_t& y = d.layer[l];
        float* v = sx + p.v_off[l];
        const int c = d.c[l + 1], cp = p.cp[l + 1];
        bool ok = true;
        if (y.running_mean) ok = u.push(PadItem{v + 2 * (size_t)cp, y.running_mean, 1, c, cp, c, 0, 0}) && ok;
        if (y.running_var) ok = u.push(PadItem{v + 3 * (size_t)cp, y.running_var, 1, c, cp, c, 0, 0}) && ok;
        PCL_REQUIRE(ok, "pcl_mlp_stack_fwd_f32: more padded layers than the pad table holds");
    }
    return launch_pad(u, d.stream);
}

extern "C" int pcl_mlp_stack_bwd_f32(const pcl_mlp_stack_t* dp) {
    PCL_TRY(validate(dp, "pcl_mlp_stack_bwd_f32"));
    const pcl_mlp_stack_t& d = *dp;
    const PadPlan p = narrow_supported(d) ? PadPlan{} : pad_plan(d);
    if (!p.on) return stack_bwd_impl(dp);
    PCL_REQUIRE(d.save && d.tmp, "pcl_mlp_stack_bwd_f32: null save / tmp");
    const int L = d.n_layers;
    for (int l = 0; l < L; ++l)
        PCL_REQUIRE(d.layer[l].dW && d.layer[l].dgamma && d.layer[l].dbeta && (!d.layer[l].bias || d.layer[l].dbias), "pcl_mlp_stack_bwd_f32: layer %d: null gradient output", l);
    size_t sv = 0, ft = 0, bt = 0;
    {
        pcl_mlp_stack_t probe = padded_desc(d, p, reinterpret_cast<float*>(uintptr_t(4096)), reinterpret_cast<float*>(uintptr_t(4096)));
        PCL_TRY(stack_sizes_impl(&probe, &sv, &ft, &bt));
    }
    if (d.save_bytes < al256(sv) + p.save_floats * 4 || d.tmp_bytes < al256(bt) + p.bwd_floats * 4)
        return fail(PCL_EWS, "pcl_mlp_stack_bwd_f32: save %zu < %zu or tmp %zu < %zu", d.save_bytes, al256(sv) + p.save_floats * 4, d.tmp_bytes, al256(bt) + p.bwd_floats * 4);
    float* sx = reinterpret_cast<float*>(static_cast<char*>(d.save) + al256(sv));
    float* bx = reinterpret_cast<float*>(static_cast<char*>(d.tmp) + al256(bt));
    pcl_mlp_stack_t q = padded_desc(d, p, sx, bx);
    q.save_bytes = sv; q.tmp_bytes = bt;
    PCL_TRY(stack_bwd_impl(&q));
    PadTable u = {};
    for (int l = 0; l < L; ++l) {
        const pcl_stack_layer_t& y = d.layer[l];
        bool ok = true;
        if (p.wpad[l]) ok = u.push(PadItem{bx + p.dw_off[l], y.dW, d.c[l + 1], d.c[l], p.cp[l], d.c[l], 0, 0}) && ok;
        if (p.opad[l]) {
            float* g = bx + p.dv_off[l];
            const int c = d.c[l + 1], cp = p.cp[l + 1];
            ok = u.push(PadItem{g, y.dgamma, 1, c, cp, c, 0, 0}) && ok;
            ok = u.push(PadItem{g + cp, y.dbeta, 1, c, cp, c, 0, 0}) && ok;
            if (y.bias) ok = u.push(PadItem{g + 2 * (size_t)cp, y.dbias, 1, c, cp, c, 0, 0}) && ok;
        }
        PCL_REQUIRE(ok, "pcl_mlp_stack_bwd_f32: more padded layers than the pad table holds");
    }
    return launch_pad(u, d.stream);
}

static int stack_sizes_impl(const pcl_mlp_stack_t* d, size_t* save_bytes, size_t* fwd_tmp_bytes, size_t* bwd_tmp_bytes) {
    PCL_TRY(validate(d, "pcl_mlp_stack_sizes"));
    if (narrow_supported(*d)) {
        if (save_bytes) *save_bytes = narrow_save_bytes();
        if (fwd_tmp_bytes) *fwd_tmp_bytes = narrow_fwd_tmp_bytes();
        if (bwd_tmp_bytes) *bwd_tmp_bytes = narrow_bwd_tmp_bytes();
        return PCL_OK;
    }
    if (save_bytes) *save_bytes = save_layout(*d, nullptr).bytes;
    if (fwd_tmp_bytes) *fwd_tmp_bytes = fwd_tmp(*d, nullptr).bytes;
    if (bwd_tmp_bytes) *bwd_tmp_bytes = bwd_tmp(*d, nullptr).bytes;
    return PCL_OK;
}

extern "C" int pcl_mlp_stack_last(const pcl_mlp_stack_t* d, size_t* y_offset, size_t* scale_offset, size_t* shift_offset) {
    PCL_TRY(validate(d, "pcl_mlp_stack_last"));
    char* const base = reinterpret_cast<char*>(uintptr_t(4096));
    const SaveLayout s = save_layout(*d, base);
    const int L = d->n_layers;
    if (y_offset) *y_offset = (size_t)(reinterpret_cast<char*>(s.Y[L - 1]) - base);
    if (scale_offset) *scale_offset = (size_t)(reinterpret_cast<char*>(s.vec[L - 1]) - base);
    if (shift_offset) *shift_offset = (size_t)(reinterpret_cast<char*>(s.vec[L - 1] + d->c[L]) - base);
    return PCL_OK;
}

static int stack_fwd_impl(const pcl_mlp_stack_t* dp) {
    PCL_TRY(validate(dp, "pcl_mlp_stack_fwd_f32"));
    const pcl_mlp_stack_t& d = *dp;
    PCL_REQUIRE((d.out || d.defer_act) && d.save && d.tmp, "pcl_mlp_stack_fwd_f32: null out / save / tmp");
    if (narrow_supported(d)) {
        if (d.save_bytes < narrow_save_bytes() || d.tmp_bytes < narrow_fwd_tmp_bytes())
            return fail(PCL_EWS, "pcl_mlp_stack_fwd_f32: save %zu < %zu or tmp %zu < %zu", d.save_bytes, narrow_save_bytes(), d.tmp_bytes, narrow_fwd_tmp_bytes());
        return narrow_fwd(d);
    }
    const SaveLayout s = save_layout(d, d.save);
    const FwdTmp t = fwd_tmp(d, d.tmp);
    if (d.save_bytes < s.bytes || d.tmp_bytes < t.bytes)
        return fail(PCL_EWS, "pcl_mlp_stack_fwd_f32: save %zu < %zu or tmp %zu < %zu", d.save_bytes, s.bytes, d.tmp_bytes, t.bytes);
    const int L = d.n_layers, P = d.P;
    const int G = pooled_groups(d);
    const int32_t* rmeta = d.grouped ? s.row_meta : nullptr;
    const int32_t* nrows = d.grouped ? d.group_off + G : nullptr;
    void* st = d.stream;
    const float* cur = d.x;
    const float *in_scale = nullptr, *in_shift = nullptr;
    for (int l = 0; l < L; ++l) {
        const pcl_stack_layer_t& ly = d.layer[l];
        const int cin = d.c[l], cout = d.c[l + 1];
        float* Y = s.Y[l];
        int rows;
        if (l == 0 && d.grouped) {
            const int off = d.use_xyz ? 3 : 0, ldw = d.c[0];
            const bool inl = grouped_inline(d), wide = grouped_wide(d);
            float* const Uf = s.Uf ? s.Uf : t.Uf;
            if (wide) {
                PCL_TRY(group_linear_fwd_impl(d.xyz, d.new_xyz, nullptr, d.use_xyz ? ly.W : nullptr, nullptr, nullptr, 0, ldw, d.idx, d.cnt,
                                              d.group_off, d.B, d.N, d.m, d.pool, cout, Y, s.row_meta, s.row_src, s.row_loc, s.row_feat, t.stats,
                                              st, 1, ly.W + off, d.Wf_dense, d.Cf));
                tagf("pt%dx%d", d.Cf, cout);
                if (d.flush_k) PCL_TRY(pcl_frag_linear_fwd_f32(d.feature, d.Cf, d.Wf_dense, d.Cf, ly.bias, nullptr, nullptr, 0.f, d.B * d.N, d.Cf, cout, Uf, cout,
                                                               nullptr, nullptr, d.flush_k, st));
                else PCL_TRY(pcl_linear_fwd_rows_f32(d.feature, d.Wf_dense, ly.bias, nullptr, nullptr, 0.f, d.B * d.N, d.Cf, cout, Uf,
                                                     t.pt_stats, nullptr, nullptr, st));
            }
            if (gather_scatter(d))
                PCL_TRY(pcl_group_rows_transpose_i32(s.row_src, d.group_off, d.B, d.N, d.m, d.pool, s.in_off, s.in_rows, st));
            tagf("glin%d", cout, 0);
            PCL_TRY(group_linear_fwd_impl(d.xyz, d.new_xyz, wide ? Uf : nullptr, d.use_xyz ? ly.W : nullptr, inl ? d.feature : nullptr,
                                          inl ? ly.W + off : nullptr, inl ? d.Cf : 0, ldw, d.idx, d.cnt, d.group_off, d.B, d.N, d.m,
                                          d.pool, cout, Y, s.row_meta, s.row_src, s.row_loc, s.row_feat, t.stats, st, wide ? 2 : 3, nullptr,
                                          nullptr, 0));
            rows = pcl_group_linear_stat_rows(d.B, d.m);
        } else if (l == L - 1 && use_gmax(d)) {
            tagf("fwd%dx%d", cin, cout);
            PCL_TRY(pcl_linear_fwd_gmax_f32(cur, ly.W, ly.bias, in_scale, in_shift, d.slope, P, cin, cout, d.pool, Y, t.stats, t.gmax,
                                            t.gmin, t.gamax, t.gamin, st));
            rows = pcl_mlp_stat_rows(P, cout, 0);
        } else if (frag_fwd(d)) {
            tagf("fwd%dx%d", cin, cout);
            PCL_TRY(pcl_frag_linear_fwd_f32(cur, cin, ly.W, cin, ly.bias, in_scale, in_shift, d.slope, P, cin, cout, Y, cout, nullptr, t.stats, d.flush_k, st));
            rows = pcl_frag_stat_rows(P);
        } else {
            tagf("fwd%dx%d", cin, cout);
            PCL_TRY(pcl_linear_fwd_rows_f32(cur, ly.W, ly.bias, in_scale, in_shift, d.slope, P, cin, cout, Y, t.stats, rmeta, nrows, st));
            rows = pcl_mlp_stat_rows(P, cout, d.grouped ? 2 : 0);
        }
        float* v = s.vec[l];
        PCL_TRY(pcl_bn_finalize_f32(t.stats, rows, ly.gamma, ly.beta, P, cout, d.eps, d.momentum, v, v + cout, v + 2 * cout, v + 3 * cout,
                                    ly.running_mean, ly.running_var, st));
        cur = Y; in_scale = v; in_shift = v + cout;
    }
    const int cl = d.c[L];
    if (G && !d.defer_act) {
        if (use_gmax(d)) PCL_TRY(pcl_group_minmax_finalize_f32(t.gmax, t.gmin, t.gamax, t.gamin, in_scale, in_shift, d.out_slope, G, cl, d.out, s.arg, s.ymax, st));
        else if (d.grouped) { tagf("maxrows%d", cl, 0); PCL_TRY(pcl_bn_act_max_rows_f32(cur, d.group_off, in_scale, in_shift, d.out_slope, G, cl, d.out, s.arg, s.ymax, st)); }
        else { tagf("max%d", cl, 0); PCL_TRY(pcl_bn_act_max_f32(cur, in_scale, in_shift, d.out_slope, G, d.pool, cl, d.out, s.arg, s.ymax, st)); }
    } else if (!d.defer_act) {
        PCL_TRY(pcl_bn_act_f32(cur, in_scale, in_shift, d.out_slope, P, cl, d.out, st));
    }
    set_launch_tag("");
    return PCL_OK;
}

static int stack_bwd_impl(const pcl_mlp_stack_t* dp) {
    PCL_TRY(validate(dp, "pcl_mlp_stack_bwd_f32"));
    const pcl_mlp_stack_t& d = *dp;
    PCL_REQUIRE((d.out || d.defer_act) && d.save && d.tmp && d.gout, "pcl_mlp_stack_bwd_f32: null out / save / tmp / gout");
    PCL_REQUIRE(d.gout_ld == 0 || d.gout_ld == d.c[d.n_layers] || (d.gout_ld > d.c[d.n_layers] && !d.defer_act && pooled_groups(d) > 0),
                "pcl_mlp_stack_bwd_f32: gout_ld %d (a row stride for gout is taken by pooled stacks only, and is at least the width %d)", d.gout_ld, d.c[d.n_layers]);
    PCL_REQUIRE(!d.defer_act || (d.ext_stats && d.ext_stat_rows >= 1), "pcl_mlp_stack_bwd_f32: defer_act needs ext_stats / ext_stat_rows");
    if (narrow_supported(d)) {
        if (d.save_bytes < narrow_save_bytes() || d.tmp_bytes < narrow_bwd_tmp_bytes())
            return fail(PCL_EWS, "pcl_mlp_stack_bwd_f32: save %zu < %zu or tmp %zu < %zu", d.save_bytes, narrow_save_bytes(), d.tmp_bytes, narrow_bwd_tmp_bytes());
        for (int l = 0; l < d.n_layers; ++l)
            PCL_REQUIRE(d.layer[l].dW && d.layer[l].dgamma && d.layer[l].dbeta && (!d.layer[l].bias || d.layer[l].dbias),
                        "pcl_mlp_stack_bwd_f32: layer %d: null gradient output", l);
        return narrow_bwd(d);
    }
    const SaveLayout s = save_layout(d, d.save);
    const BwdTmp t = bwd_tmp(d, d.tmp);
    if (d.save_bytes < s.bytes || d.tmp_bytes < t.bytes)
        return fail(PCL_EWS, "pcl_mlp_stack_bwd_f32: save %zu < %zu or tmp %zu < %zu", d.save_bytes, s.bytes, d.tmp_bytes, t.bytes);
    const int L = d.n_layers, P = d.P;
    const int G = pooled_groups(d);
    const int ns = d.pool ? d.pool : 1;
    for (int l = 0; l < L; ++l)
        PCL_REQUIRE(d.layer[l].dW && d.layer[l].dgamma && d.layer[l].dbeta && (!d.layer[l].bias || d.layer[l].dbias),
                    "pcl_mlp_stack_bwd_f32: layer %d: null gradient output", l);
    const int32_t* rmeta = d.grouped ? s.row_meta : nullptr;
    const int32_t* nrows = d.grouped ? d.group_off + G : nullptr;
    void* st = d.stream;
    const int cl = d.c[L];
    int rows = 0, cur_stats = 0, cur_du = 0, cur_c = 0;
    const float* dU = nullptr;
    const double* ext_stats = nullptr;
    bool sparse;
    const float* vL = s.vec[L - 1];
// ... 44 lines not shown
            PCL_TRY(pcl_bn_bwd_dy_f32(ext_stats ? ext_stats : t.stats[cur_stats], rows, ly.gamma, mean, invstd, P, cout, ly.dgamma, ly.dbeta, a, k1, k2,
                                      ly.dbias, sparse ? nullptr : dU, s.Y[l], sparse ? s.arg : nullptr, sparse ? t.gz : nullptr, ns, P, t.dy_l[l], st));
        else if (!have_pre)
            PCL_TRY(pcl_bn_bwd_consts_f32(ext_stats ? ext_stats : t.stats[cur_stats], rows, ly.gamma, mean, invstd, P, cout, ly.dgamma, ly.dbeta, a, k1,
                                          k2, ly.dbias, st));
        if (ext_stats) { ext_stats = nullptr; cur_stats = 1 - cur_stats; }
        have_pre = false;
        if (l == 0 && d.grouped) {
            const int off = d.use_xyz ? 3 : 0, fan_in = d.c[0], C1 = cout;
            const bool inl = grouped_inline(d), wide = grouped_wide(d);
            const bool pt_pair = wide && d.need_dx && pcl_linear_bwd_pair_supported(d.B * d.N, C1, d.Cf, 0);
            const bool x_in_finish = pt_pair && gather_scatter(d) && t.dWxp;
            tagf("glinbwd%d", C1, 0);
            if (gather_scatter(d))
                PCL_TRY(pcl_group_linear_bwd_gather_regen_f32(s.row_loc, dU, s.Uf, d.use_xyz ? ly.W : nullptr, fan_in, a, k1, k2, mean, s.in_off,
                                                              s.in_rows, d.B, d.N, C1, t.dUf, t.dWxp,
                                                              (t.dWxp && !x_in_finish) ? ly.dW : nullptr, fan_in, st));
            else if (!t.dUf && (t.dWxp || t.dWfp) && pcl_group_linear_bwd_regen_supported(C1, inl ? d.Cf : 0) && al16(dU))
                PCL_TRY(pcl_group_linear_bwd_regen_f32(s.row_loc, s.row_feat, d.use_xyz ? ly.W : nullptr, inl ? ly.W + off : nullptr, inl ? d.Cf : 0,
                                                       fan_in, dU, a, k1, k2, mean, nrows, C1, t.dWxp, t.dWfp, ly.dW, fan_in, off, st));
            else
            PCL_TRY(group_linear_bwd_impl(s.row_loc, s.row_feat, inl ? d.Cf : 0, dU, s.Y[0], a, k1, k2, mean, s.row_src, nrows, d.B, d.N, C1,
                                          t.dUf, t.dWxp, t.dWfp, (t.dWxp || t.dWfp) ? ly.dW : nullptr, fan_in, off, st, true));
            if (wide) {
                float* one = t.unit;
                float* zero = one + C1;
                const int Pp = d.B * d.N;
                if (pt_pair) {
                    PCL_REQUIRE(d.dx, "pcl_mlp_stack_bwd_f32: need_dx without dx");
                    tagf("ptpair%dx%d", C1, d.Cf);
                    PCL_TRY(pcl_linear_bwd_pair_f32(t.dUf, t.dUf, one, zero, zero, zero, nullptr, nullptr, 1, d.Wf_dense, d.feature, nullptr, nullptr, 0.f, 0, Pp,
                                                    C1, d.Cf, d.dx, nullptr, 0, t.ptws, t.ptws_bytes, st));
                    PCL_TRY(pair_finish_impl(t.ptws, t.ptws_bytes, Pp, C1, d.Cf, ly.dW + off, fan_in, nullptr, 0, nullptr, nullptr, nullptr, 0,
                                             nullptr, nullptr, nullptr, nullptr, nullptr, nullptr, st,
                                             x_in_finish ? t.dWxp : nullptr, pcl_group_linear_stat_rows(d.B, d.m), C1, fan_in, ly.dW));
                    break;
                }
                tagf("ptdw%dx%d", C1, d.Cf);
                PCL_TRY(pcl_linear_bwd_dw_rows_f32(t.dUf, t.dUf, one, zero, zero, zero, nullptr, nullptr, 1, d.feature, nullptr, nullptr, 0.f, Pp,
                                                   C1, d.Cf, ly.dW + off, t.ptws, t.ptws_bytes, nullptr, nullptr, fan_in, st));
                if (d.need_dx) {
                    PCL_REQUIRE(d.dx, "pcl_mlp_stack_bwd_f32: need_dx without dx");
                    tagf("ptdx%dx%d", C1, d.Cf);
                    PCL_TRY(pcl_linear_bwd_dx_rows_f32(t.dUf, t.dUf, one, zero, zero, zero, nullptr, nullptr, 1, d.Wf_dense, Pp, C1, d.Cf, nullptr,
                                                       nullptr, nullptr, 0.f, d.dx, nullptr, nullptr, nullptr, 0, 0, st));
                }
            }
            break;
        }
        const float* Xprev = l > 0 ? s.Y[l - 1] : d.x;
        const float* psc = l > 0 ? s.vec[l - 1] : nullptr;
        const float* psh = l > 0 ? s.vec[l - 1] + cin : nullptr;
        const float* Yl = s.Y[l];
        if (l > 0 && fused_bwd_enabled() && pcl_linear_bwd_fused_supported(cout, cin)) {
            float* dUp = t.dU[cur_du];
            double* stn = t.stats[1 - cur_stats];
            tagf("fb%dx%d", cout, cin);
            PCL_TRY(pcl_linear_bwd_fused_rows_f32(dU, Yl, a, k1, k2, mean, sparse ? s.arg : nullptr, sparse ? t.gz : nullptr, ns, ly.W, P, cout, cin,
                                                  Xprev, psc, psh, d.slope, dUp, stn, t.ws, t.ws_bytes, rmeta, nrows, st));
            const pcl_stack_layer_t& lp = d.layer[l - 1];
            float* kp = t.consts[1 - cur_c];
            const float* vp = s.vec[l - 1];
            PCL_TRY(pcl_linear_bwd_fused_finish_f32(t.ws, t.ws_bytes, P, cout, cin, ly.dW, stn, lp.gamma, vp + 2 * cin, vp + 3 * cin, P, lp.dgamma,
                                                    lp.dbeta, kp, kp + cin, kp + 2 * cin, lp.dbias, st));
            have_pre = true;
            dU = dUp; sparse = false; cur_du = 1 - cur_du; cur_stats = 1 - cur_stats; cur_c = 1 - cur_c;
            rows = pcl_linear_bwd_fused_stat_rows(P, cin);
            continue;
        }
        if (!sd && !fr && !rmeta && (l > 0 || d.need_dx) && pcl_linear_bwd_pair_supported(P, cout, cin, l == 0 ? d.x_grad_from : 0)) {
            float* dUp = l > 0 ? t.dU[cur_du] : d.dx;
            PCL_REQUIRE(dUp, "pcl_mlp_stack_bwd_f32: need_dx without dx");
            double* stn = l > 0 ? t.stats[1 - cur_stats] : nullptr;
            tagf("pair%dx%d", cout, cin);
            PCL_TRY(pcl_linear_bwd_pair_f32(dU, Yl, a, k1, k2, mean, sparse ? s.arg : nullptr, sparse ? t.gz : nullptr, ns, ly.W, Xprev, psc, psh, d.slope,
                                            l > 0 ? 1 : 0, P, cout, cin, dUp, stn, l == 0 ? d.x_grad_from : 0, t.ws, t.ws_bytes, st));
            if (l > 0) {
                const pcl_stack_layer_t& lp = d.layer[l - 1];
                float* kp = t.consts[1 - cur_c];
                const float* vp = s.vec[l - 1];
                const int rows_below = pcl_mlp_stat_rows(P, cin, 1);
                PCL_TRY(pcl_linear_bwd_pair_finish_f32(t.ws, t.ws_bytes, P, cout, cin, ly.dW, 0, stn, rows_below, lp.gamma, vp + 2 * cin, vp + 3 * cin, P,
                                                       lp.dgamma, lp.dbeta, kp, kp + cin, kp + 2 * cin, lp.dbias, st));
                have_pre = true;
                rows = rows_below;
                dU = dUp; sparse = false; cur_du = 1 - cur_du; cur_stats = 1 - cur_stats; cur_c = 1 - cur_c;
            } else
                PCL_TRY(pcl_linear_bwd_pair_finish_f32(t.ws, t.ws_bytes, P, cout, cin, ly.dW, 0, nullptr, 0, nullptr, nullptr, nullptr, 0, nullptr, nullptr,
                                                       nullptr, nullptr, nullptr, nullptr, st));
            continue;
        }
        void* dw_st = st;
        if (sd) {
            if (hipEventRecord(sc->fork, as_stream(st)) != hipSuccess || hipStreamWaitEvent(sc->st, sc->fork, 0) != hipSuccess)
                return fail(PCL_EHIP, "pcl_mlp_stack_bwd_f32: fork to the side stream failed");
            dw_st = sc->st; join.forked = true;
        }
        tagf("dw%dx%d", cout, cin);
        if (fr) {
            PCL_TRY(pcl_linear_bwd_dw_plain_f32(t.dy_l[l], Xprev, psc, psh, d.slope, P, cout, cin, ly.dW, t.ws, t.ws_bytes, 0, dw_st));
            if (l > 0 || d.need_dx) {
                float* dUp = l > 0 ? (sd ? t.dU_l[l - 1] : t.dU[cur_du]) : d.dx;
                PCL_REQUIRE(dUp, "pcl_mlp_stack_bwd_f32: need_dx without dx");
                double* stn = l > 0 ? t.stats[1 - cur_stats] : nullptr;
                tagf("dx%dx%d", cout, cin);
                PCL_TRY(pcl_frag_linear_bwd_dx_f32(t.dy_l[l], ly.W, cin, P, cout, cin, l > 0 ? Xprev : nullptr, cin, l > 0 ? psc : nullptr, l > 0 ? psh : nullptr,
                                                   d.slope, dUp, cin, stn, l == 0 ? d.x_grad_from : 0, st));
                if (l > 0) {
                    rows = frag_stat_rows(P);
                    dU = dUp; sparse = false; cur_du = 1 - cur_du; cur_stats = 1 - cur_stats; cur_c = 1 - cur_c;
                }
            }
            continue;
        }
        PCL_TRY(pcl_linear_bwd_dw_rows_f32(dU, Yl, a, k1, k2, mean, sparse ? s.arg : nullptr, sparse ? t.gz : nullptr, ns, Xprev, psc, psh, d.slope,
                                           P, cout, cin, ly.dW, t.ws, t.ws_bytes, rmeta, nrows, 0, dw_st));
        if (l > 0 || d.need_dx) {
            float* dUp = l > 0 ? (sd ? t.dU_l[l - 1] : t.dU[cur_du]) : d.dx;
            PCL_REQUIRE(dUp, "pcl_mlp_stack_bwd_f32: need_dx without dx");
            double* stn = l > 0 ? t.stats[1 - cur_stats] : nullptr;
            tagf("dx%dx%d", cout, cin);
            PCL_TRY(pcl_linear_bwd_dx_rows_f32(dU, Yl, a, k1, k2, mean, sparse ? s.arg : nullptr, sparse ? t.gz : nullptr, ns, ly.W, P, cout, cin,
                                               l > 0 ? Xprev : nullptr, psc, psh, d.slope, dUp, stn, rmeta, nrows, l == 0 ? d.x_grad_from : 0, 0, st));
            if (l > 0) {
                rows = pcl_mlp_stat_rows(P, cin, 1 | (rmeta ? 2 : 0));
                dU = dUp; sparse = false; cur_du = 1 - cur_du; cur_stats = 1 - cur_stats; cur_c = 1 - cur_c;
            }
        }
    }
    PCL_TRY(join.now());
    set_launch_tag("");
    return PCL_OK;
}

extern "C" int pcl_mlp_fewrow_layer(int P, int Cout, int Cin, int first_layer) {
    if (!g_lab.fewrow || !frag_rows_eligible(P)) return 0;
    if (!first_layer && fused_bwd_enabled() && pcl_linear_bwd_fused_supported(Cout, Cin)) return 0;
    return pcl_bn_bwd_dy_supported(P, Cout);
}
```

### pointcloudlib_amd/misc/mlp_hip.py

```python
import ctypes
import os

import torch

from .. import _lib, syncbn

_P = lambda t: None if t is None else t.data_ptr()
_FUSED_BWD = os.environ.get("PCL_FUSED_BWD", "1") != "0"


def _stream():
    return torch._C._cuda_getCurrentRawStream(torch.cuda.current_device())


def _rows_cost(nrows_dev, P, per_row, const):
    if nrows_dev is None:
        return per_row * P + const
    return lambda: per_row * int(nrows_dev.item()) + const


def _empty(shape, dev, dtype=torch.float32):
    return torch.empty(shape, dtype=dtype, device=dev)


class _Pack:

    def __init__(self):
        self.tensors, self.layout = [], []

    def add(self, name, t):
        self.layout.append((name, None if t is None else len(self.tensors), False))
        if t is not None:
            self.tensors.append(t)

    def add_list(self, name, ts):
        idx = []
        for t in ts:
            idx.append(None if t is None else len(self.tensors))
            if t is not None:
                self.tensors.append(t)
        self.layout.append((name, idx, True))

    @staticmethod
    def unpack(layout, saved):
        out = {}
        for name, idx, is_list in layout:
            if is_list:
                out[name] = [None if i is None else saved[i] for i in idx]
            else:
                out[name] = None if idx is None else saved[idx]
        return out


_UNIT_CONSTS = {}


def _unit_consts(dev, c):
    key = (dev.type, dev.index, c)
    v = _UNIT_CONSTS.get(key)
    if v is None:
        v = _UNIT_CONSTS[key] = (torch.ones(c, device=dev), torch.zeros(c, device=dev))
    return v


class _FusedMLP(torch.autograd.Function):

    @staticmethod
    def forward(ctx, x, cfg, *params):
        ns, slope, eps, momentum, training, bn, last_act, rowset, x_grad_from, link = cfg[:10]
        flush_k = cfg[10] if len(cfg) > 10 else 0
        L = len(params) // 6
        dev = x.device
        x = x.contiguous()
        P, C0 = x.shape
        Pbn = P
        rmeta = nrows = None
        if rowset is not None:
            assert ns == rowset.ns and P == rowset.capacity
            rmeta, nrows = rowset.row_meta, rowset.n_rows_dev
        st = _stream()
        Ys, scales, shifts, means, invstds = [], [], [], [], []
        cur, in_scale, in_shift = x, None, None
        cin = C0
        W0p = None
        for l in range(L):
            W, bias, gamma, beta, rmean, rvar = params[6 * l:6 * l + 6]
            cout = W.shape[0]
            if l == 0 and link is None and W.shape[1] != cin:
                assert W.shape[1] < cin, f"input has {cin} columns, first layer expects {W.shape[1]}"
                W = W0p = torch.nn.functional.pad(W.detach(), (0, cin - W.shape[1]))
            fused_max = (l == L - 1) and ns in (32, 64) and rowset is None and not flush_k
            folded = l == 0 and link is not None
            flushed = bool(flush_k) and rowset is None and not folded
            if folded:
                assert cout == cin and L >= 2, "folded first layer: x must be the layer's own output"
                Y, stats, rows = x, link.stats, link.rows
            else:
                Y = _empty((P, cout), dev)
                rows = _lib.size_query("pcl_frag_stat_rows", P) if flushed else _lib.size_query("pcl_mlp_stat_rows", P, cout, 2 if rowset is not None else 0)
                stats = _empty((rows, 2, cout), dev, torch.float64)
            if folded:
                pass
            elif flushed:
                _lib.call("pcl_frag_linear_fwd_f32", _P(cur), cin, _P(W), cin, _P(bias), _P(in_scale), _P(in_shift), slope, P, cin, cout, _P(Y), cout,
                          None, _P(stats), flush_k, st, algo_bytes=4 * P * (cin + cout) + 4 * cin * cout, algo_flops=2 * P * cin * cout, tag=f"fwd{cin}x{cout}")
            elif fused_max:
                G = P // ns
                gmax, gmin = _empty((G, cout), dev), _empty((G, cout), dev)
                gamax, gamin = _empty((G, cout), dev, torch.int32), _empty((G, cout), dev, torch.int32)
                _lib.call("pcl_linear_fwd_gmax_f32", _P(cur), _P(W), _P(bias), _P(in_scale), _P(in_shift), slope, P, cin,
                          cout, ns, _P(Y), _P(stats), _P(gmax), _P(gmin), _P(gamax), _P(gamin), st,
                          algo_bytes=4 * P * (cin + cout) + 4 * cin * cout, algo_flops=2 * P * cin * cout,
                          tag=f"fwd{cin}x{cout}")
            else:
                _lib.call("pcl_linear_fwd_rows_f32", _P(cur), _P(W), _P(bias), _P(in_scale), _P(in_shift), slope, P, cin, cout,
                          _P(Y), _P(stats), _P(rmeta), _P(nrows), st,
                          algo_bytes=_rows_cost(nrows, P, 4 * (cin + cout), 4 * cin * cout),
                          algo_flops=_rows_cost(nrows, P, 2 * cin * cout, 0), tag=f"fwd{cin}x{cout}")
            if bn and training:
                scale, shift, mean, invstd = _empty((4, cout), dev).unbind(0)
                f_stats, f_rows, f_P = (stats, rows, Pbn) if not syncbn.active() else syncbn.reduce_rows(stats, rows, Pbn)
                _lib.call("pcl_bn_finalize_f32", _P(f_stats), f_rows, _P(gamma), _P(beta), f_P, cout, eps, momentum, _P(scale),
                          _P(shift), _P(mean), _P(invstd), _P(rmean), _P(rvar), st)
            elif bn:
                invstd = torch.rsqrt(rvar + eps)
                mean = rmean
                scale = gamma * invstd
                shift = beta - scale * rmean
            else:
                scale, shift = _unit_consts(dev, cout)
                mean, invstd = shift, scale
            Ys.append(Y); scales.append(scale); shifts.append(shift); means.append(mean); invstds.append(invstd)
            cur, in_scale, in_shift, cin = Y, scale, shift, cout
        out_slope = slope if last_act else 1.0
        if ns:
            G = P // ns
            out = _empty((G, cin), dev)
            arg = _empty((G, cin), dev, torch.int32)
            ymax = _empty((G, cin), dev)
            if fused_max:
                _lib.call("pcl_group_minmax_finalize_f32", _P(gmax), _P(gmin), _P(gamax), _P(gamin), _P(in_scale),
                          _P(in_shift), out_slope, G, cin, _P(out), _P(arg), _P(ymax), st)
            elif rowset is not None:
# ... 356 lines not shown
                _lib.call("pcl_linear_bwd_dw_rows_f32", _P(dUf), _P(dUf), _P(one), _P(zero), _P(zero), _P(zero), None, None, 1,
                          _P(feat2), None, None, 0.0, P, C1, C, _P(dW0[:, off:]), _P(ws), nbytes, None, None, fan_in, st,
                          tag=f"ptdw{C1}x{C}")
            if ctx.needs_input_grad[2]:
                dfeat = _empty((P, C), dev)
                _lib.call("pcl_linear_bwd_dx_rows_f32", _P(dUf), _P(dUf), _P(one), _P(zero), _P(zero), _P(zero), None, None, 1,
                          _P(Wf), P, C1, C, None, None, None, 0.0, _P(dfeat), None, None, None, 0, 0, st, tag=f"ptdx{C1}x{C}")
                dfeat = dfeat.view(B, N, C)
        return None, None, dfeat, dW0, None, None, None, None, None


def can_fold_first_layer(module, use_xyz, feature):
    return (module.n_layers >= 2 and module.biases is None and module.spec[1] <= 256 and (use_xyz or feature is not None))


def grouped_mlp(module, xyz, new_xyz, feature, idx, cnt, group_off, use_xyz):
    from .ops import RowSet
    if not xyz.is_cuda:
        raise RuntimeError("fused HIP MLP needs GPU tensors (no CPU fallback)")
    B, m, ns = idx.shape
    if _stack_eligible(module):
        return stack_grouped(module, xyz.contiguous(), new_xyz.contiguous(), feature, idx, cnt, group_off, use_xyz)
    link = _Link()
    Y0, row_meta, row_src = _GroupLinear.apply(xyz.contiguous(), new_xyz.contiguous(), feature, module.weights[0], idx, cnt,
                                               group_off, link, bool(use_xyz))
    rowset = RowSet(B, m, ns, row_meta, row_src, group_off)
    params = []
    for i in range(module.n_layers):
        params += [module.weights[i] if i > 0 else None, None,
                   module.gammas[i] if module.bn else None, module.betas[i] if module.bn else None,
                   getattr(module, f"running_mean_{i}") if module.bn else None,
                   getattr(module, f"running_var_{i}") if module.bn else None]
    params[0] = module.weights[0].detach()
    cfg = (ns, module.slope, module.eps, module.momentum, module.training, module.bn, module.last_act, rowset, 0, link)
    params, finish = _profiling_pad(module, B * m * ns, params, folded_first=True)
    out = _FusedMLP.apply(Y0, cfg, *params)
    if finish is not None:
        finish()
    return out.reshape(B, m, out.shape[-1])


USE_STACK = os.environ.get("PCL_STACK", "1") != "0"
_MAXL = _lib.define("PCL_STACK_MAX_LAYERS")
_CLayer = _lib.struct("pcl_stack_layer_t")
_CStack = _lib.struct("pcl_mlp_stack_t")


_GOUT_IN_PLACE = __import__("os").environ.get("PCL_GOUT_IN_PLACE", "1") != "0"
COUNTERS = {"strided_gout": 0}


class _StackPlan:
    __slots__ = ("desc", "ref", "save_bytes", "fwd_tmp", "bwd_tmp", "G", "cl", "L", "has_bias", "gsizes", "gshapes", "gtotal",
                 "spec", "grouped", "wide", "off", "P", "c0", "defer", "last_off", "out_slope")


_PLANS = {}
_lib.on_switch_change(_PLANS.clear)


def _stack_plan(module, P, c0, pool, grouped, geom, need_dx, x_grad_from, defer=False):
    flush_k = int(getattr(module, "flush_k", 0))
    key = (id(module), P, c0, pool, grouped, geom, need_dx, x_grad_from, module.slope, module.last_act, defer,
           module.eps, module.momentum, module.biases is not None, flush_k)
    plan = _PLANS.get(key)
    if plan is not None and plan.spec is module.spec:
        return plan
    L = module.n_layers
    d = _CStack()
    d.struct_bytes = ctypes.sizeof(_CStack)
    d.n_layers = L
    spec = module.spec
    d.c[0] = c0
    for l in range(L):
        d.c[l + 1] = spec[l + 1]
    d.P, d.pool, d.grouped, d.x_grad_from, d.need_dx = P, pool, int(grouped), int(x_grad_from), int(need_dx)
    d.defer_act = int(defer)
    d.flush_k = flush_k
    if grouped:
        d.B, d.N, d.m, d.Cf, d.use_xyz = geom
    d.slope, d.out_slope, d.eps, d.momentum = module.slope, (module.slope if module.last_act else 1.0), module.eps, module.momentum
    d.x = 1
    d.xyz = d.new_xyz = d.idx = d.cnt = d.group_off = 1
    d.feature = d.Wf_dense = 1
    for l in range(L):
        d.layer[l].W = d.layer[l].gamma = d.layer[l].beta = 1
    sv, ft, bt = ctypes.c_size_t(), ctypes.c_size_t(), ctypes.c_size_t()
    _lib.check(_lib.lib().pcl_mlp_stack_sizes(ctypes.byref(d), ctypes.byref(sv), ctypes.byref(ft), ctypes.byref(bt)), "pcl_mlp_stack_sizes")
    plan = _StackPlan()
    plan.desc, plan.ref = d, ctypes.byref(d)
    plan.save_bytes, plan.fwd_tmp, plan.bwd_tmp = sv.value, ft.value, bt.value
    plan.defer, plan.last_off, plan.out_slope = bool(defer), None, (module.slope if module.last_act else 1.0)
    if defer:
        yo, so, ho = ctypes.c_size_t(), ctypes.c_size_t(), ctypes.c_size_t()
        _lib.check(_lib.lib().pcl_mlp_stack_last(ctypes.byref(d), ctypes.byref(yo), ctypes.byref(so), ctypes.byref(ho)), "pcl_mlp_stack_last")
        plan.last_off = (yo.value, so.value, ho.value)
    plan.L, plan.cl, plan.spec, plan.grouped, plan.P, plan.c0 = L, spec[L], module.spec, grouped, P, c0
    plan.G = (geom[0] * geom[2]) if grouped else (P // pool if pool else 0)
    plan.has_bias = module.biases is not None
    plan.off = 3 if (grouped and geom[4]) else 0
    plan.wide = bool(grouped and geom[3] > 0 and (geom[3] > 4 or need_dx))
    sizes, shapes = [], []
    for l in range(L):
        cin, cout = (c0 if l == 0 else spec[l]), spec[l + 1]
        sizes += [cout * cin, cout, cout] + ([cout] if plan.has_bias else [])
        shapes.append((cout, cin))
    plan.gsizes, plan.gshapes, plan.gtotal = sizes, shapes, sum(sizes)
    _PLANS[key] = plan
    return plan


class per_kernel_path:

    def __enter__(self):
        global USE_STACK
        from . import head
        self.prev = (USE_STACK, head.USE_STACK)
        USE_STACK = head.USE_STACK = False

    def __exit__(self, *a):
        global USE_STACK
        from . import head
        USE_STACK, head.USE_STACK = self.prev


def _stack_eligible(module):
    return (USE_STACK and module.bn and module.training and module.n_layers <= _MAXL and not syncbn.active())


class _StackFn(torch.autograd.Function):

    @staticmethod
    def forward(ctx, t_in, aux, *params):
        plan, geo, running = aux[0], aux[1], aux[2]
        d = type(plan.desc).from_buffer_copy(plan.desc)
        L = plan.L
        dev = params[0].device
        npl = 4 if plan.has_bias else 3
        st = _stream()
        save = torch.empty((plan.save_bytes,), dtype=torch.uint8, device=dev)
        tmp = torch.empty((plan.fwd_tmp,), dtype=torch.uint8, device=dev)
        if plan.defer:
            yo, so, ho = plan.last_off
            out = save[yo:yo + 4 * plan.P * plan.cl].view(torch.float32).view(plan.P, plan.cl)
            link = aux[3]
            link.scale = save[so:so + 4 * plan.cl].view(torch.float32)
            link.shift = save[ho:ho + 4 * plan.cl].view(torch.float32)
            link.slope = plan.out_slope
        else:
            out = torch.empty((plan.G if plan.G else plan.P, plan.cl), dtype=torch.float32, device=dev)
        Wf = None
        if plan.grouped:
            xyz, new_xyz, idx, cnt, group_off = geo
            d.xyz, d.new_xyz, d.idx, d.cnt, d.group_off = xyz.data_ptr(), new_xyz.data_ptr(), idx.data_ptr(), cnt.data_ptr(), group_off.data_ptr()
            d.feature = None if t_in is None else t_in.data_ptr()
            if plan.wide:
                Wf = torch.empty((params[0].shape[0], params[0].shape[1] - plan.off), dtype=torch.float32, device=dev)
            d.Wf_dense = None if Wf is None else Wf.data_ptr()
            d.x = None
        else:
            d.x = t_in.data_ptr()
        for l in range(L):
            ly, q = d.layer[l], params[npl * l:npl * l + npl]
            ly.W, ly.gamma, ly.beta = q[0].data_ptr(), q[1].data_ptr(), q[2].data_ptr()
            ly.bias = q[3].data_ptr() if plan.has_bias else None
            ly.running_mean, ly.running_var = running[2 * l].data_ptr(), running[2 * l + 1].data_ptr()
        d.out = None if plan.defer else out.data_ptr()
        d.save, d.save_bytes, d.tmp, d.tmp_bytes, d.stream = save.data_ptr(), plan.save_bytes, tmp.data_ptr(), plan.fwd_tmp, st
        _lib.call("pcl_mlp_stack_fwd_f32", ctypes.byref(d), tag="stack_fwd")
        ctx.plan = plan
        ctx.link = aux[3] if plan.defer else None
        ctx.save_for_backward(t_in, out, save, Wf, *(geo if plan.grouped else ()), *params)
        return out

    @staticmethod
    def backward(ctx, gout):
        plan = ctx.plan
        d = type(plan.desc).from_buffer_copy(plan.desc)
        L = plan.L
        sv = ctx.saved_tensors
        t_in, out, save, Wf = sv[0], sv[1], sv[2], sv[3]
        n0 = 4
        if plan.grouped:
            xyz, new_xyz, idx, cnt, group_off = sv[4:9]
            n0 = 9
        params = sv[n0:]
        dev = out.device
        npl = 4 if plan.has_bias else 3
        d.gout_ld = 0
        if (_GOUT_IN_PLACE and plan.G and not plan.defer and gout.dim() == 2 and gout.stride(1) == 1 and gout.stride(0) > gout.shape[1]
                and gout.stride(0) < 2 ** 31 and gout.dtype == torch.float32):
            d.gout_ld = gout.stride(0)
            COUNTERS["strided_gout"] += 1
        else:
            gout = gout.contiguous()
        tmp = torch.empty((plan.bwd_tmp,), dtype=torch.uint8, device=dev)
        flat = torch.empty((plan.gtotal,), dtype=torch.float32, device=dev)
        pieces = flat.split_with_sizes(plan.gsizes)
        dx = None
        need_dx = ctx.needs_input_grad[0]
        if need_dx:
            dx = torch.empty_like(t_in)
        if plan.grouped:
            d.xyz, d.new_xyz, d.idx, d.cnt, d.group_off = xyz.data_ptr(), new_xyz.data_ptr(), idx.data_ptr(), cnt.data_ptr(), group_off.data_ptr()
            d.feature = None if t_in is None else t_in.data_ptr()
            d.Wf_dense = None if Wf is None else Wf.data_ptr()
            d.x = None
        else:
            d.x = t_in.data_ptr()
        base, o = flat.data_ptr(), 0
        grads = []
        for l in range(L):
            ly, q = d.layer[l], params[npl * l:npl * l + npl]
            ly.W, ly.gamma, ly.beta = q[0].data_ptr(), q[1].data_ptr(), q[2].data_ptr()
            ly.bias = q[3].data_ptr() if plan.has_bias else None
            cout, cin = plan.gshapes[l]
            k = npl * l
            ly.dW = base + 4 * o; o += cout * cin
            ly.dgamma = base + 4 * o; o += cout
            ly.dbeta = base + 4 * o; o += cout
            grads += [pieces[k].view(cout, cin), pieces[k + 1], pieces[k + 2]]
            if plan.has_bias:
                ly.dbias = base + 4 * o; o += cout
                grads.append(pieces[k + 3])
            else:
                ly.dbias = None
        d.out = None if plan.defer else out.data_ptr()
        d.save, d.save_bytes, d.tmp, d.tmp_bytes = save.data_ptr(), plan.save_bytes, tmp.data_ptr(), plan.bwd_tmp
        d.gout, d.dx, d.stream = gout.data_ptr(), (None if dx is None else dx.data_ptr()), _stream()
        if plan.defer:
            link = ctx.link
            d.ext_stats, d.ext_stat_rows = link.stats.data_ptr(), link.rows
            link.stats = None
        _lib.call("pcl_mlp_stack_bwd_f32", ctypes.byref(d), tag="stack_bwd")
        return (dx, None) + tuple(grads)


def _stack_params(module):
    cached = module.__dict__.get("_stack_params_cache")
    if (cached is not None and cached[0][0] is module.weights[0] and cached[1][0] is module._buffers.get("running_mean_0")
            and cached[0][-1] is (module.biases[-1] if module.biases is not None else module.betas[-1]) and cached[1][-1] is module._buffers.get(f"running_var_{module.n_layers - 1}")):
        return cached
    ps, running = [], []
    for i in range(module.n_layers):
        ps += [module.weights[i], module.gammas[i], module.betas[i]] + ([module.biases[i]] if module.biases is not None else [])
        running += [getattr(module, f"running_mean_{i}"), getattr(module, f"running_var_{i}")]
    module.__dict__["_stack_params_cache"] = (ps, running)
    return ps, running


def stack_plain(module, x2, ns, x_grad_from):
    P, c0 = x2.shape
    need_dx = x2.requires_grad
    plan = _stack_plan(module, P, c0, ns, False, None, need_dx, x_grad_from if need_dx else 0)
    ps, running = _stack_params(module)
    return _StackFn.apply(x2, (plan, None, running), *ps)


class DeferLink:
    __slots__ = ("scale", "shift", "slope", "stats", "rows")

    def __init__(self):
        self.scale = self.shift = self.stats = None
        self.slope, self.rows = 0.0, 0


def stack_plain_deferred(module, x2):
    if not (_stack_eligible(module) and module.weights[0].shape[1] == x2.shape[1]):
        return None
    P, c0 = x2.shape
    need_dx = x2.requires_grad
    plan = _stack_plan(module, P, c0, 0, False, None, need_dx, 0, defer=True)
    ps, running = _stack_params(module)
    link = DeferLink()
    return _StackFn.apply(x2, (plan, None, running, link), *ps), link


_FULL = {}


def stack_grouped_deferred(module, xyz, new_xyz, feature, idx, use_xyz=True):
    if feature is None or feature.shape[-1] <= 4 or not use_xyz:
        return None
    if not (_stack_eligible(module) and module.n_layers >= 2 and module.spec[1] <= 256):
        return None
    B, m, ns = idx.shape
    N = xyz.shape[1]
    Cf = feature.shape[-1]
    key = (xyz.device, B * m, ns)
    full = _FULL.get(key)
    if full is None:
        full = _FULL[key] = (torch.full((B, m), ns, dtype=torch.int32, device=xyz.device),
                             (torch.arange(B * m + 1, dtype=torch.int64, device=xyz.device) * ns).to(torch.int32))
    cnt, group_off = full
    need_dx = feature.requires_grad
    plan = _stack_plan(module, B * m * ns, 3 + Cf, ns, True, (B, N, m, Cf, 1), need_dx, 0, defer=True)
    ps, running = _stack_params(module)
    link = DeferLink()
    Y = _StackFn.apply(feature.contiguous(), (plan, (xyz.contiguous(), new_xyz.contiguous(), idx.contiguous(), cnt, group_off), running, link), *ps)
    return Y, link


def stack_grouped(module, xyz, new_xyz, feature, idx, cnt, group_off, use_xyz):
    B, m, ns = idx.shape
    N = xyz.shape[1]
    Cf = 0 if feature is None else feature.shape[-1]
    need_dx = feature is not None and feature.requires_grad
    c0 = (3 if use_xyz else 0) + Cf
    plan = _stack_plan(module, B * m * ns, c0, ns, True, (B, N, m, Cf, int(bool(use_xyz))), need_dx, 0)
# ... 5 lines not shown
```

### pointcloudlib_amd/misc/ops.py

```python
import math

import os

import torch
from torch import nn

from .. import _lib

__all__ = [
    "optimal_block", "furthest_point_sample", "ball_query", "ball_query_multi", "group_offsets_multi", "group_points", "group_points_compact", "RowSet", "group_all",
    "index_points",
    "knn_indices", "edge_features", "three_nn", "three_interpolate", "row_offsets", "pack_rows", "unpack_rows", "interpolate_pack",
    "row_cloud", "packed_layout", "segment_max", "mlp_segment_max", "broadcast_rows",
    "FurthestPointSampler", "BallQueryGrouper", "GroupAll",
    "KNN", "PointNetFeaturePropagation",
]


def _dev(t, name, dtype=torch.float32):
    if t is None:
        return None
    if not t.is_cuda:
        raise RuntimeError(f"{name}: expected a tensor on the GPU (libpcl_hip has no CPU path), got {t.device}")
    if t.dtype != dtype:
        raise TypeError(f"{name}: expected {dtype}, got {t.dtype}")
    return t.contiguous()


def _p(t):
    return None if t is None else t.data_ptr()


def _stream():
    return torch._C._cuda_getCurrentRawStream(torch.cuda.current_device())


def _lengths(lengths, B, N, device, name="lengths", n_samples=None):
    if lengths is None:
        return None
    if isinstance(lengths, torch.Tensor) and lengths.is_cuda:
        if lengths.dtype != torch.int32:
            raise TypeError(f"{name}: a device tensor must be torch.int32, got {lengths.dtype}")
        if lengths.dim() != 1 or lengths.shape[0] != B:
            raise ValueError(f"{name}: expected shape [{B}], got {tuple(lengths.shape)}")
        if lengths.device != device:
            raise ValueError(f"{name}: on {lengths.device}, the clouds on {device}")
        return lengths.contiguous()
    host = lengths.detach() if isinstance(lengths, torch.Tensor) else torch.as_tensor(lengths)
    if host.dtype.is_floating_point or host.dtype == torch.bool or host.dtype.is_complex:
        raise TypeError(f"{name}: expected integers, got {host.dtype}")
    if host.dim() != 1 or host.shape[0] != B:
        raise ValueError(f"{name}: expected shape [{B}] (one count per cloud), got {tuple(host.shape)}")
    vals = host.tolist()
    for b, v in enumerate(vals):
        if not 1 <= v <= N:
            raise ValueError(f"{name}[{b}]={v} must be in [1, N={N}]")
        if n_samples is not None and v < n_samples:
            raise ValueError(f"{name}[{b}]={v} is less than n_samples={n_samples}: a cloud cannot be sampled beyond its own points")
    return torch.tensor(vals, dtype=torch.int32).to(device)


def _xyz_shape(xyz, name="xyz"):
    if not isinstance(xyz, torch.Tensor) or xyz.dim() != 3 or xyz.shape[2] != 3:
# ... 162 lines not shown
        ctx.save_for_backward(idx)
        ctx.dims = (B, N, m, ns, C, int(use_xyz))
        return out

    @staticmethod
    def backward(ctx, gout):
        (idx,) = ctx.saved_tensors
        B, N, m, ns, C, use_xyz = ctx.dims
        gfeat = None
        if C > 0 and ctx.needs_input_grad[2]:
            gout = _dev(gout, "grad")
            gfeat = torch.empty((B, N, C), dtype=torch.float32, device=gout.device)
            _lib.call("pcl_group_bwd_f32", _p(gout), _p(idx), B, N, m, ns, C, use_xyz, _p(gfeat), _stream(),
                      algo_bytes=B * (4 * m * ns * C + 4 * m * ns + 4 * N * C))
        return None, None, gfeat, None, None


def group_points(xyz, new_xyz, feature, idx, use_xyz=True):
    if not use_xyz and feature is None:
        raise ValueError("use_xyz=False needs features")
    return _GroupPoints.apply(xyz, new_xyz, feature, idx, bool(use_xyz))


_GROUP_ALL_BWD_VIEW = __import__("os").environ.get("PCL_GROUP_ALL_BWD_VIEW", "1") != "0"


class _GroupAll(torch.autograd.Function):
    @staticmethod
    def forward(ctx, xyz, feat, use_xyz):
        xyz = _dev(xyz, "xyz")
        feat = _dev(feat, "feature")
        B, N, _ = xyz.shape
        C = 0 if feat is None else feat.shape[2]
        D = (3 if use_xyz else 0) + C
        out = torch.empty((B, 1, N, D), dtype=torch.float32, device=xyz.device)
        _lib.call("pcl_group_all_f32", _p(xyz), _p(feat), B, N, C, int(use_xyz), _p(out), _stream())
        ctx.dims = (B, N, C, int(use_xyz))
        return out

    @staticmethod
    def backward(ctx, gout):
        B, N, C, use_xyz = ctx.dims
        gfeat = None
        if C > 0 and ctx.needs_input_grad[1]:
            D = (3 if use_xyz else 0) + C
            if _GROUP_ALL_BWD_VIEW and gout.is_contiguous() and gout.is_cuda and gout.dtype == torch.float32:
                return None, gout.view(B, N, D)[:, :, D - C:], None
            gout = _dev(gout, "grad")
            gfeat = torch.empty((B, N, C), dtype=torch.float32, device=gout.device)
            _lib.call("pcl_group_all_bwd_f32", _p(gout), B, N, C, use_xyz, _p(gfeat), _stream())
        return None, gfeat, None


class RowSet:

    def __init__(self, B, m, ns, row_meta, row_src, group_off):
        self.B, self.m, self.ns = B, m, ns
        self.G = B * m
        self.row_meta, self.row_src, self.group_off = row_meta, row_src, group_off
        self.n_rows_dev = group_off[self.G:]

    @property
    def capacity(self):
        return self.G * self.ns


def group_offsets(cnt):
    cnt = _dev(cnt, "cnt", torch.int32)
    G = cnt.numel()
    group_off = torch.empty((G + 1,), dtype=torch.int32, device=cnt.device)
    _lib.call("pcl_group_offsets_i32", _p(cnt), G, _p(group_off), _stream())
    return group_off


def group_offsets_multi(cnts):
    import ctypes
    cnts = [_dev(c, "cnt", torch.int32) for c in cnts]
    n, G = len(cnts), cnts[0].numel()
    if not 1 <= n <= BALL_QUERY_MULTI_MAX or any(c.numel() != G for c in cnts):
        raise ValueError("group_offsets_multi: 1..4 count arrays of equal size")
    offs = [torch.empty((G + 1,), dtype=torch.int32, device=cnts[0].device) for _ in range(n)]
    c_c = (ctypes.c_void_p * n)(*[t.data_ptr() for t in cnts])
    c_o = (ctypes.c_void_p * n)(*[t.data_ptr() for t in offs])
    _lib.call("pcl_group_offsets_multi_i32", n, c_c, G, c_o, _stream())
    return offs


class _GroupCompact(torch.autograd.Function):
    @staticmethod
    def forward(ctx, xyz, new_xyz, feat, idx, cnt, group_off, use_xyz, pad_to):
        idx = _dev(idx, "idx", torch.int32)
        cnt = _dev(cnt, "cnt", torch.int32)
        group_off = _dev(group_off, "group_off", torch.int32)
        B, m, ns = idx.shape
        xyz = _dev(xyz, "xyz")
        new_xyz = _dev(new_xyz, "new_xyz")
        feat = _dev(feat, "feature")
        N = xyz.shape[1]
        C = 0 if feat is None else feat.shape[2]
        D = (3 if use_xyz else 0) + C
        S = (D + pad_to - 1) // pad_to * pad_to
        cap = B * m * ns
        dev = idx.device
        rows = torch.empty((cap, S), dtype=torch.float32, device=dev)
        row_meta = torch.empty((cap, 2), dtype=torch.int32, device=dev)
        row_src = torch.empty((cap,), dtype=torch.int32, device=dev)
# ... 452 lines not shown
```

### pointcloudlib_amd/networks/cls/pointnet2.py

```python
import os
from typing import List, Optional

import torch
from torch import nn

from ...misc.head import fc_head
from ...misc.layers import PointwiseMLP
from ...misc.ops import (BALL_QUERY_MULTI_MAX, BallQueryGrouper, FurthestPointSampler, GroupAll, ball_query, ball_query_multi, group_offsets,
                         group_offsets_multi, group_points, _lengths)


_MULTI_BALL_QUERY = os.environ.get("PCL_MULTI_BALL_QUERY", "1") != "0"


class PointNetModuleBase(nn.Module):
    def __init__(self):
        super().__init__()
        self.n_points = None
        self.sampler = None
        self.groupers = None
        self.mlps = None
        self.compact_duplicates = True

    def build_mlps(self, mlp_spec: List[int], use_xyz: bool = True, bn: bool = True) -> PointwiseMLP:
        spec = list(mlp_spec)
        if use_xyz:
            spec[0] += 3
        return PointwiseMLP(spec, bias=not bn, bn=bn, slope=0.0)

    def sample(self, xyz: torch.Tensor, lengths=None):
        if self.n_points is None:
            if lengths is not None:
                raise NotImplementedError("GroupAll directly on a ragged cloud needs a masked max (out of scope, DESIGN.md section 14)")
            return None, [None] * len(self.groupers)
        if lengths is not None:
            lengths = _lengths(lengths, xyz.shape[0], xyz.shape[1], xyz.device, n_samples=self.n_points)
        new_xyz = self.sampler(xyz, lengths=lengths)
        out = []
        gs = list(self.groupers)
        if 1 < len(gs) <= BALL_QUERY_MULTI_MAX and _MULTI_BALL_QUERY:
            lists = ball_query_multi(new_xyz, xyz, [g.radius for g in gs], [g.n_samples for g in gs], return_cnt=True, lengths=lengths)
        else:
            lists = [ball_query(new_xyz, xyz, g.radius, g.n_samples, return_cnt=True, lengths=lengths) for g in gs]
        if self.compact_duplicates and 1 < len(gs) <= BALL_QUERY_MULTI_MAX and _MULTI_BALL_QUERY:
            offs = group_offsets_multi([cnt for _, cnt in lists])
        else:
            offs = [group_offsets(cnt) if self.compact_duplicates else None for _, cnt in lists]
        for (idx, cnt), off in zip(lists, offs):
            out.append((idx, cnt, off))
        return new_xyz, out

    def forward(self, xyz: torch.Tensor, feature: Optional[torch.Tensor], sampling=None, lengths=None):
        new_xyz, idxs = sampling if sampling is not None else self.sample(xyz, lengths)
        new_feature_list = []
        for grouper, mlp, ic in zip(self.groupers, self.mlps, idxs):
            if ic is None:
                grouped = grouper(new_xyz, xyz, feature)
                new_feature_list.append(mlp(grouped, group_max=grouped.shape[2]))
            elif self.compact_duplicates and mlp.resolved_backend(xyz) == "hip":
                new_feature_list.append(mlp.forward_grouped(xyz, new_xyz, feature, ic[0], ic[1], ic[2], grouper.use_xyz))
            else:
                grouped = group_points(xyz, new_xyz, feature, ic[0], grouper.use_xyz)
                new_feature_list.append(mlp(grouped, group_max=grouped.shape[2]))
        new_feature = new_feature_list[0] if len(new_feature_list) == 1 else torch.cat(new_feature_list, dim=-1)
        return new_xyz, new_feature

    def execute(self, *a, **k):
        return self(*a, **k)


class PointnetModule(PointNetModuleBase):
    def __init__(self, mlp: List[int], n_points=None, radius=None, n_samples=None, bn=True, use_xyz=True):
        super().__init__()
        self.n_points = n_points
        self.groupers = nn.ModuleList()
        if self.n_points is not None:
            self.sampler = FurthestPointSampler(n_points)
            self.groupers.append(BallQueryGrouper(radius, n_samples, use_xyz))
        else:
            self.groupers.append(GroupAll(use_xyz))
        self.mlps = nn.ModuleList()
        self.mlps.append(self.build_mlps(mlp, use_xyz, bn))


class PointnetModuleMSG(PointNetModuleBase):
    def __init__(self, n_points: int, radius: List[float], n_samples: List[int], mlps: List[List[int]], bn=True,
                 use_xyz=True):
        super().__init__()
        self.n_points = n_points
        self.sampler = FurthestPointSampler(n_points)
        self.groupers = nn.ModuleList()
        for r, s in zip(radius, n_samples):
            self.groupers.append(BallQueryGrouper(r, s, use_xyz))
        self.mlps = nn.ModuleList()
        for mlp in mlps:
            self.mlps.append(self.build_mlps(mlp, use_xyz, bn))


_AB_RECORD_STREAM = bool(os.environ.get("PCL_AB_RECORD_STREAM"))


_OWN_SAMPLING_STREAM = {}
_OWN_LAST_CONSUMER = {}


def sampling_stream(owner, stream, device=None):
    if isinstance(stream, str):
        if stream != "own":
            raise ValueError(f"stream={stream!r}: pass a torch.cuda.Stream, None or 'own'")
        dev = torch.cuda.current_device() if device is None or device.index is None else device.index
        s = _OWN_SAMPLING_STREAM.get(dev)
# ... 115 lines not shown
```

Measured before the change: 18450 point-clouds/s.

## Pad group-all rows and first-layer weights to a multiple-of-four pitch

Adds a group-all kernel that writes grouped rows with a leading dimension rounded up to a multiple of 4 and, in the same launch, writes a zero-padded copy of the first-layer weight matrix. The MLP stack forward and backward paths (dx, dW, fused pair) accept separate x and W strides, so the first layer can use float4 vectorised loads even when fan-in is not divisible by 4 (e.g. 3+256=259 in the SSG group-all stage). This adds a padded weight copy on every step and extra stride plumbing through several backward entry points, and it falls back to the old path when the module or stack reports it is ineligible.

```diff
diff --git a/include/pcl_hip.h b/include/pcl_hip.h
--- a/include/pcl_hip.h
+++ b/include/pcl_hip.h
@@ -45,6 +45,9 @@
                       int use_xyz, float* gfeat, void* stream);
 int pcl_group_all_f32(const float* xyz, const float* feat, int B, int N, int C, int use_xyz,
                       float* out, void* stream);
+int pcl_group_all_pitch_ld(int D);
+int pcl_group_all_pitch_f32(const float* xyz, const float* feat, int B, int N, int C, int use_xyz, int ld, float* out,
+                            const float* W, int Cout, float* Wp, void* stream);
 int pcl_group_all_bwd_f32(const float* gout, int B, int N, int C, int use_xyz, float* gfeat,
                           void* stream);
 int pcl_gather_rows_f32(const float* src, const int32_t* idx, int B, int N, int M, int C, float* out,
@@ -295,6 +298,7 @@
     int32_t need_dx;
     int32_t B, N, m, Cf, use_xyz;
     float slope, out_slope, eps, momentum;
+    int32_t x_ld;
     const float* x;
     const float* xyz;
     const float* new_xyz;
@@ -319,6 +323,7 @@
     int32_t gout_ld;
 } pcl_mlp_stack_t;
 int pcl_mlp_stack_last(const pcl_mlp_stack_t* desc, size_t* y_offset, size_t* scale_offset, size_t* shift_offset);
+int pcl_mlp_stack_pitch_supported(const pcl_mlp_stack_t* desc);
 int pcl_mlp_stack_sizes(const pcl_mlp_stack_t* desc, size_t* save_bytes, size_t* fwd_tmp_bytes, size_t* bwd_tmp_bytes);
 int pcl_mlp_stack_fwd_f32(const pcl_mlp_stack_t* desc);
 int pcl_mlp_stack_bwd_f32(const pcl_mlp_stack_t* desc);
diff --git a/pointcloudlib_amd/csrc/group.hip b/pointcloudlib_amd/csrc/group.hip
--- a/pointcloudlib_amd/csrc/group.hip
+++ b/pointcloudlib_amd/csrc/group.hip
@@ -50,6 +50,27 @@
     }
 }
 
+struct PadWJob { const float* src; float* dst; int rows, first, blocks; };
+__global__ __launch_bounds__(GT) void group_all_pitch_kernel(const float* __restrict__ xyz, const float* __restrict__ feat,
+                                                             int C, int use_xyz, int ld, size_t total, float* __restrict__ out,
+                                                             PadWJob wj) {
+    const int D = (use_xyz ? 3 : 0) + C;
+    const int off = use_xyz ? 3 : 0;
+    if ((int)blockIdx.x >= wj.first) {
+        const int n = wj.rows * ld;
+        for (int i = ((int)blockIdx.x - wj.first) * GT + (int)threadIdx.x; i < n; i += wj.blocks * GT) {
+            const int r = i / ld, c = i - r * ld;
+            wj.dst[i] = c < D ? wj.src[(size_t)r * D + c] : 0.f;
+        }
+        return;
+    }
+    for (size_t g = (size_t)blockIdx.x * GT + threadIdx.x; g < total; g += (size_t)wj.first * GT) {
+        const size_t p = g / ld;
+        const int c = (int)(g - p * ld);
+        out[g] = c < off ? xyz[p * 3 + c] : c < D ? feat[p * C + (c - off)] : 0.f;
+    }
+}
+
 __global__ __launch_bounds__(GT) void group_all_bwd_kernel(const float* __restrict__ gout, int C, int use_xyz,
                                                            size_t total, float* __restrict__ gfeat) {
     const int D = (use_xyz ? 3 : 0) + C;
@@ -165,6 +186,24 @@
     if (!total) return PCL_OK;
     hipLaunchKernelGGL(group_all_kernel, dim3(grid_for(total)), dim3(GT), 0, as_stream(stream), xyz, feat, C, use_xyz, total, out);
     return check_launch("pcl_group_all_f32");
+}
+
+extern "C" int pcl_group_all_pitch_ld(int D) { return D < 1 ? 0 : (D + 3) / 4 * 4; }
+
+extern "C" int pcl_group_all_pitch_f32(const float* xyz, const float* feat, int B, int N, int C, int use_xyz, int ld, float* out,
+                                       const float* W, int Cout, float* Wp, void* stream) {
+    PCL_REQUIRE(out && (!use_xyz || xyz) && (C == 0 || feat), "pcl_group_all_pitch_f32: null pointer");
+    PCL_REQUIRE(B >= 0 && N >= 0 && C >= 0 && (use_xyz || C > 0), "pcl_group_all_pitch_f32: bad sizes");
+    const int D = (use_xyz ? 3 : 0) + C;
+    PCL_REQUIRE(ld >= D && ld % 4 == 0, "pcl_group_all_pitch_f32: ld=%d must be a multiple of 4 and at least %d", ld, D);
+    PCL_REQUIRE((W == nullptr) == (Wp == nullptr) && (!W || Cout >= 1) && (size_t)(W ? Cout : 0) * ld < 0x7fffffffull,
+                "pcl_group_all_pitch_f32: W [Cout][%d] and Wp [Cout][%d] come together, Cout=%d", D, ld, Cout);
+    const size_t total = (size_t)B * N * ld;
+    if (!total && !W) return PCL_OK;
+    PadWJob wj = {W, Wp, W ? Cout : 0, total ? grid_for(total) : 0, 0};
+    if (W) { const int nb = (Cout * ld + GT - 1) / GT; wj.blocks = nb < 64 ? nb : 64; }
+    hipLaunchKernelGGL(group_all_pitch_kernel, dim3(wj.first + wj.blocks), dim3(GT), 0, as_stream(stream), xyz, feat, C, use_xyz, ld, total, out, wj);
+    return check_launch("pcl_group_all_pitch_f32");
 }
 
 extern "C" int pcl_group_all_bwd_f32(const float* gout, int B, int N, int C, int use_xyz, float* gfeat, void* stream) {
diff --git a/pointcloudlib_amd/csrc/mlp.hip b/pointcloudlib_amd/csrc/mlp.hip
--- a/pointcloudlib_amd/csrc/mlp.hip
+++ b/pointcloudlib_amd/csrc/mlp.hip
@@ -889,6 +889,7 @@
     int a_mode, b_mode;
     int gx, ti, tj;
     int ldo;
+    int ldb;
 };
 
 constexpr int DW_BP = 32;
@@ -1003,11 +1004,11 @@
 __device__ __forceinline__ void dw_load_b(const DwArgs& p, int p0, int c0, int tid, DwStage<VEC, W>& st) {
     using S = DwStage<VEC, W>;
     st.p0 = p0;
-    const int c = min(c0 + (tid % S::CPR) * (VEC ? 4 : 1), p.J - (VEC ? 4 : 1));
+    const int c = min(c0 + (tid % S::CPR) * (VEC ? 4 : 1), p.ldb - (VEC ? 4 : 1));
 #pragma unroll
     for (int i = 0; i < S::NI; ++i) {
         const int r = min(p0 + tid / S::CPR + S::RP * i, p.P - 1);
-        const size_t off = (size_t)r * p.J + c;
+        const size_t off = (size_t)r * p.ldb + c;
         if constexpr (VEC) st.v[i] = *reinterpret_cast<const float4*>(p.Bsrc + off);
         else st.s[i] = p.Bsrc[off];
     }
@@ -2772,6 +2773,22 @@
     return fail(PCL_EINVAL, "pcl_linear: unsupported mode combination %d/%d", a.a_mode, a.e_mode);
 }
 
+int dx_rows_impl(const float* dU, const float* Y, const float* a_, const float* k1, const float* k2, const float* mu, const int32_t* arg, const float* gz,
+                 int ns, const float* W, int P, int Cout, int Cin, const float* Yprev, const float* prev_scale, const float* prev_shift, float prev_slope,
+                 float* dUprev, double* stats_ws, const int32_t* row_meta, const int32_t* n_rows_dev, int first_col, int w_ld, int c_ld, void* stream);
+int dw_rows_impl(const float* dU, const float* Y, const float* a_, const float* k1, const float* k2, const float* mu, const int32_t* arg, const float* gz,
+                 int ns, const float* Xprev, const float* prev_scale, const float* prev_shift, float prev_slope, int P, int Cout, int Cin, float* dW,
+                 void* workspace, size_t workspace_bytes, const int32_t* row_meta, const int32_t* n_rows_dev, int dw_ld, int x_ld, void* stream);
+int bwd_pair_impl(const float* dU, const float* Y, const float* a_, const float* k1, const float* k2, const float* mu, const int32_t* arg, const float* gz,
+                  int ns, const float* W, const float* Xprev, const float* prev_scale, const float* prev_shift, float prev_slope, int masked, int P,
+                  int Cout, int Cin, float* dUprev, double* stats_ws, int first_col, void* workspace, size_t workspace_bytes, int x_ld, int w_ld,
+                  void* stream);
+int pair_finish_impl(const void* workspace, size_t workspace_bytes, int P, int Cout, int Cin, float* dW, int dw_ld,
+                     const double* stats_ws, int stat_rows, const float* gamma_prev, const float* mean_prev,
+                     const float* invstd_prev, int P_bn, float* dgamma_prev, float* dbeta_prev,
+                     float* a_prev, float* k1_prev, float* k2_prev, float* dbias_zero_prev, void* stream,
+                     const float* xpart, int xrows, int xC1, int xld, float* xdW0);
+
 }
 using namespace pcl;
 
@@ -2901,6 +2918,14 @@
                                           int Cin, const float* Yprev, const float* prev_scale, const float* prev_shift,
                                           float prev_slope, float* dUprev, double* stats_ws, const int32_t* row_meta,
                                           const int32_t* n_rows_dev, int first_col, int cin_stride, void* stream) {
+    return dx_rows_impl(dU, Y, a_, k1, k2, mu, arg, gz, ns, W, P, Cout, Cin, Yprev, prev_scale, prev_shift, prev_slope, dUprev, stats_ws, row_meta,
+                        n_rows_dev, first_col, cin_stride, cin_stride, stream);
+}
+int pcl::dx_rows_impl(const float* dU, const float* Y, const float* a_, const float* k1, const float* k2, const float* mu,
+                      const int32_t* arg, const float* gz, int ns, const float* W, int P, int Cout,
+                      int Cin, const float* Yprev, const float* prev_scale, const float* prev_shift,
+                      float prev_slope, float* dUprev, double* stats_ws, const int32_t* row_meta,
+                      const int32_t* n_rows_dev, int first_col, int w_ld, int c_ld, void* stream) {
     PCL_REQUIRE(Y && a_ && k1 && k2 && mu && W && dUprev, "pcl_linear_bwd_dx_f32: null pointer");
     PCL_REQUIRE((dU != nullptr) != (arg != nullptr && gz != nullptr), "pcl_linear_bwd_dx_f32: pass dU or (arg,gz)");
     PCL_REQUIRE(P >= 1 && Cin >= 1 && Cout >= 1 && (dU || ns >= 1), "pcl_linear_bwd_dx_f32: bad sizes");
@@ -2909,8 +2934,8 @@
     a.A = dU; a.A2 = Y; a.B = W; a.sc = a_; a.sh = k1; a.k2 = k2; a.mu = mu; a.arg = arg; a.gz = gz; a.ns = ns;
     a.C = dUprev; a.stats = stats_ws; a.Yprev = Yprev; a.esc = prev_scale; a.esh = prev_shift; a.eslope = prev_slope;
     PCL_REQUIRE(first_col >= 0 && first_col < Cin && (first_col == 0 || !Yprev), "pcl_linear_bwd_dx_rows_f32: first_col=%d only for the input gradient", first_col);
-    a.M = P; a.N = Cin; a.K = Cout; a.n_begin = first_col; a.ldc = a.ldb = cin_stride > 0 ? cin_stride : Cin;
-    PCL_REQUIRE(a.ldc >= Cin && (a.ldc == Cin || !Yprev), "pcl_linear_bwd_dx_rows_f32: cin_stride=%d", cin_stride);
+    a.M = P; a.N = Cin; a.K = Cout; a.n_begin = first_col; a.ldc = c_ld > 0 ? c_ld : Cin; a.ldb = w_ld > 0 ? w_ld : Cin;
+    PCL_REQUIRE(a.ldc >= Cin && a.ldb >= Cin && (a.ldc == Cin || !Yprev), "pcl_linear_bwd_dx_rows_f32: row strides %d (W) / %d (dUprev) for Cin=%d", w_ld, c_ld, Cin);
     a.rmeta = reinterpret_cast<const int2*>(row_meta); a.m_dev = n_rows_dev;
     a.a_mode = dU ? A_DY : A_DY_SPARSE; a.e_mode = Yprev ? E_MASK_STORE_STATS : E_STORE;
     return launch_linear(a, as_stream(stream));
@@ -2936,7 +2961,17 @@
                                           const float* prev_scale, const float* prev_shift, float prev_slope, int P, int Cout,
                                           int Cin, float* dW, void* workspace, size_t workspace_bytes, const int32_t* row_meta,
                                           const int32_t* n_rows_dev, int dw_ld, void* stream) {
+    return dw_rows_impl(dU, Y, a_, k1, k2, mu, arg, gz, ns, Xprev, prev_scale, prev_shift, prev_slope, P, Cout, Cin, dW, workspace, workspace_bytes,
+                        row_meta, n_rows_dev, dw_ld, 0, stream);
+}
+int pcl::dw_rows_impl(const float* dU, const float* Y, const float* a_, const float* k1, const float* k2, const float* mu,
+                      const int32_t* arg, const float* gz, int ns, const float* Xprev,
+                      const float* prev_scale, const float* prev_shift, float prev_slope, int P, int Cout,
+                      int Cin, float* dW, void* workspace, size_t workspace_bytes, const int32_t* row_meta,
+                      const int32_t* n_rows_dev, int dw_ld, int x_ld, void* stream) {
     PCL_REQUIRE(Y && a_ && k1 && k2 && mu && Xprev && dW, "pcl_linear_bwd_dw_f32: null pointer");
+    if (x_ld == 0) x_ld = Cin;
+    PCL_REQUIRE(x_ld >= Cin && (x_ld == Cin || !prev_scale), "pcl_linear_bwd_dw_f32: x_ld=%d (at least Cin=%d; a wider one takes plain rows only)", x_ld, Cin);
     PCL_REQUIRE(dw_ld == 0 || dw_ld >= Cin, "pcl_linear_bwd_dw_f32: dw_ld=%d < Cin=%d", dw_ld, Cin);
     PCL_REQUIRE((dU != nullptr) != (arg != nullptr && gz != nullptr), "pcl_linear_bwd_dw_f32: pass dU or (arg,gz)");
     PCL_REQUIRE((prev_scale == nullptr) == (prev_shift == nullptr), "pcl_linear_bwd_dw_f32: scale/shift together");
@@ -2952,8 +2987,8 @@
     d.part = static_cast<float*>(workspace); d.P = P; d.I = Cout; d.J = Cin;
     d.rmeta = reinterpret_cast<const int2*>(row_meta); d.p_dev = n_rows_dev;
     d.a_mode = dU ? A_DY : A_DY_SPARSE; d.b_mode = prev_scale ? A_BNACT : A_PLAIN;
-    const bool vec = (Cout % 4 == 0) && (Cin % 4 == 0) && al16(Y, Xprev, dU) && (!gz || al16(gz, arg));
-    d.gx = gx; d.ti = ti; d.tj = tj; d.ldo = Cin;
+    const bool vec = (Cout % 4 == 0) && (x_ld % 4 == 0) && al16(Y, Xprev, dU) && (!gz || al16(gz, arg));
+    d.gx = gx; d.ti = ti; d.tj = tj; d.ldo = Cin; d.ldb = x_ld;
     const bool direct = gx == 1;
     if (direct) { d.part = dW; d.ldo = dw_ld ? dw_ld : Cin; }
     dim3 grid(gx * ti * tj);
@@ -2981,7 +3016,18 @@
                                        const int32_t* arg, const float* gz, int ns, const float* W, const float* Xprev,
                                        const float* prev_scale, const float* prev_shift, float prev_slope, int masked, int P, int Cout, int Cin,
                                        float* dUprev, double* stats_ws, int first_col, void* workspace, size_t workspace_bytes, void* stream) {
+    return bwd_pair_impl(dU, Y, a_, k1, k2, mu, arg, gz, ns, W, Xprev, prev_scale, prev_shift, prev_slope, masked, P, Cout, Cin, dUprev, stats_ws,
+                         first_col, workspace, workspace_bytes, 0, 0, stream);
+}
+int pcl::bwd_pair_impl(const float* dU, const float* Y, const float* a_, const float* k1, const float* k2, const float* mu,
+                       const int32_t* arg, const float* gz, int ns, const float* W, const float* Xprev,
+                       const float* prev_scale, const float* prev_shift, float prev_slope, int masked, int P, int Cout, int Cin,
+                       float* dUprev, double* stats_ws, int first_col, void* workspace, size_t workspace_bytes, int x_ld, int w_ld, void* stream) {
     PCL_REQUIRE(Y && a_ && k1 && k2 && mu && W && Xprev && dUprev, "pcl_linear_bwd_pair_f32: null pointer");
+    if (x_ld == 0) x_ld = Cin;
+    if (w_ld == 0) w_ld = Cin;
+    PCL_REQUIRE(x_ld >= Cin && w_ld >= Cin && (x_ld == Cin || (!prev_scale && !masked)),
+                "pcl_linear_bwd_pair_f32: x_ld=%d / w_ld=%d (at least Cin=%d; a wider x_ld takes the stack's plain input only)", x_ld, w_ld, Cin);
     PCL_REQUIRE((dU != nullptr) != (arg != nullptr && gz != nullptr), "pcl_linear_bwd_pair_f32: pass dU or (arg,gz)");
     PCL_REQUIRE((prev_scale == nullptr) == (prev_shift == nullptr), "pcl_linear_bwd_pair_f32: scale/shift together");
     PCL_REQUIRE(!masked || (prev_scale && stats_ws), "pcl_linear_bwd_pair_f32: masked mode needs scale/shift/stats");
@@ -2997,16 +3043,16 @@
     d.Bsrc = Xprev; d.bsc = prev_scale; d.bsh = prev_shift; d.bslope = prev_slope;
     d.part = static_cast<float*>(workspace); d.P = P; d.I = Cout; d.J = Cin;
     d.a_mode = dU ? A_DY : A_DY_SPARSE; d.b_mode = prev_scale ? A_BNACT : A_PLAIN;
-    d.gx = gx; d.ti = ti; d.tj = tj; d.ldo = Cin;
+    d.gx = gx; d.ti = ti; d.tj = tj; d.ldo = Cin; d.ldb = x_ld;
     LinArgs a = {};
     a.A = dU; a.A2 = Y; a.B = W; a.sc = a_; a.sh = k1; a.k2 = k2; a.mu = mu; a.arg = arg; a.gz = gz; a.ns = ns;
     a.C = dUprev; a.stats = stats_ws; a.Yprev = masked ? Xprev : nullptr; a.esc = prev_scale; a.esh = prev_shift; a.eslope = prev_slope;
-    a.M = P; a.N = Cin; a.K = Cout; a.n_begin = first_col; a.ldc = a.ldb = Cin;
+    a.M = P; a.N = Cin; a.K = Cout; a.n_begin = first_col; a.ldc = x_ld; a.ldb = w_ld;
     a.a_mode = d.a_mode; a.e_mode = masked ? E_MASK_STORE_STATS : E_STORE;
     int gxl, n_tiles; bool narrow, low;
     linear_grid(P, Cin - first_col, true, false, gxl, n_tiles, narrow, low);
     a.gx = gxl; a.nt = n_tiles;
-    const bool vec_dw = (Cout % 4 == 0) && (Cin % 4 == 0) && al16(Y, Xprev, dU) && (!gz || al16(gz, arg));
+    const bool vec_dw = (Cout % 4 == 0) && (x_ld % 4 == 0) && al16(Y, Xprev, dU) && (!gz || al16(gz, arg));
     const bool vec_nt = (a.K % 4 == 0) && al16(a.A, a.B, a.A2) && a.ldb % 4 == 0;
     const int n_dw = gx * ti * tj;
     if (vec_dw != vec_nt) {
@@ -3029,13 +3075,6 @@
     return check_launch("pcl_linear_bwd_pair_f32");
 }
 
-namespace pcl {
-int pair_finish_impl(const void* workspace, size_t workspace_bytes, int P, int Cout, int Cin, float* dW, int dw_ld,
-                     const double* stats_ws, int stat_rows, const float* gamma_prev, const float* mean_prev,
-                     const float* invstd_prev, int P_bn, float* dgamma_prev, float* dbeta_prev,
-                     float* a_prev, float* k1_prev, float* k2_prev, float* dbias_zero_prev, void* stream,
-                     const float* xpart, int xrows, int xC1, int xld, float* xdW0);
-}
 extern "C" int pcl_linear_bwd_pair_finish_f32(const void* workspace, size_t workspace_bytes, int P, int Cout, int Cin, float* dW, int dw_ld,
                                               const double* stats_ws, int stat_rows, const float* gamma_prev, const float* mean_prev,
                                               const float* invstd_prev, int P_bn, float* dgamma_prev, float* dbeta_prev,
@@ -3120,7 +3159,7 @@
     d.part = static_cast<float*>(workspace); d.P = P; d.I = Cout; d.J = Cin;
     d.a_mode = A_PLAIN; d.b_mode = prev_scale ? A_BNACT : A_PLAIN;
     const bool vec = (Cout % 4 == 0) && (Cin % 4 == 0) && al16(dy, Xprev);
-    d.gx = gx; d.ti = ti; d.tj = tj; d.ldo = Cin;
+    d.gx = gx; d.ti = ti; d.tj = tj; d.ldo = d.ldb = Cin;
     const bool direct = gx == 1;
     if (direct) { d.part = dW; d.ldo = dw_ld ? dw_ld : Cin; }
     dim3 grid(gx * ti * tj);
diff --git a/pointcloudlib_amd/csrc/stack.hip b/pointcloudlib_amd/csrc/stack.hip
--- a/pointcloudlib_amd/csrc/stack.hip
+++ b/pointcloudlib_amd/csrc/stack.hip
@@ -204,6 +204,16 @@
                      const float* invstd_prev, int P_bn, float* dgamma_prev, float* dbeta_prev,
                      float* a_prev, float* k1_prev, float* k2_prev, float* dbias_zero_prev, void* stream,
                      const float* xpart, int xrows, int xC1, int xld, float* xdW0);
+int dx_rows_impl(const float* dU, const float* Y, const float* a_, const float* k1, const float* k2, const float* mu, const int32_t* arg, const float* gz,
+                 int ns, const float* W, int P, int Cout, int Cin, const float* Yprev, const float* prev_scale, const float* prev_shift, float prev_slope,
+                 float* dUprev, double* stats_ws, const int32_t* row_meta, const int32_t* n_rows_dev, int first_col, int w_ld, int c_ld, void* stream);
+int dw_rows_impl(const float* dU, const float* Y, const float* a_, const float* k1, const float* k2, const float* mu, const int32_t* arg, const float* gz,
+                 int ns, const float* Xprev, const float* prev_scale, const float* prev_shift, float prev_slope, int P, int Cout, int Cin, float* dW,
+                 void* workspace, size_t workspace_bytes, const int32_t* row_meta, const int32_t* n_rows_dev, int dw_ld, int x_ld, void* stream);
+int bwd_pair_impl(const float* dU, const float* Y, const float* a_, const float* k1, const float* k2, const float* mu, const int32_t* arg, const float* gz,
+                  int ns, const float* W, const float* Xprev, const float* prev_scale, const float* prev_shift, float prev_slope, int masked, int P,
+                  int Cout, int Cin, float* dUprev, double* stats_ws, int first_col, void* workspace, size_t workspace_bytes, int x_ld, int w_ld,
+                  void* stream);
 int group_linear_fwd_impl(const float* xyz, const float* new_xyz, const float* Uf, const float* Wx, const float* feat_small,
                           const float* Wf_small, int CF, int ldw, const int32_t* idx, const int32_t* cnt, const int32_t* group_off, int B,
                           int N, int m, int ns, int C1, float* Y, int32_t* row_meta, int32_t* row_src, float* row_loc, float* row_feat,
@@ -321,8 +331,24 @@
     return q;
 }
 
+static inline bool pitched(const pcl_mlp_stack_t& d) { return d.x_ld != 0; }
+static bool pitch_ok(const pcl_mlp_stack_t& d) {
+    if (d.grouped || d.flush_k || d.defer_act || d.x_ld <= d.c[0] || d.x_ld % 4 != 0) return false;
+    if (narrow_supported(d) || pad_plan(d).on) return false;
+    return !fewrow_layer(d, 0) && !side_dw(d);
+}
+static int validate_pitch(const pcl_mlp_stack_t* d, const char* who) {
+    PCL_REQUIRE(!pitched(*d) || pitch_ok(*d), "%s: x_ld=%d is not taken for this stack (c[0]=%d; see pcl_mlp_stack_pitch_supported)", who, d->x_ld, d->c[0]);
+    return PCL_OK;
+}
+
 }
 using namespace pcl;
+
+extern "C" int pcl_mlp_stack_pitch_supported(const pcl_mlp_stack_t* d) {
+    if (validate(d, "pcl_mlp_stack_pitch_supported")) return 0;
+    return pitched(*d) && pitch_ok(*d) ? 1 : 0;
+}
 
 static int stack_sizes_impl(const pcl_mlp_stack_t* d, size_t* save_bytes, size_t* fwd_tmp_bytes, size_t* bwd_tmp_bytes);
 static int stack_fwd_impl(const pcl_mlp_stack_t* dp);
@@ -330,6 +356,7 @@
 
 extern "C" int pcl_mlp_stack_sizes(const pcl_mlp_stack_t* d, size_t* save_bytes, size_t* fwd_tmp_bytes, size_t* bwd_tmp_bytes) {
     PCL_TRY(validate(d, "pcl_mlp_stack_sizes"));
+    PCL_TRY(validate_pitch(d, "pcl_mlp_stack_sizes"));
     const PadPlan p = narrow_supported(*d) ? PadPlan{} : pad_plan(*d);
     if (!p.on) return stack_sizes_impl(d, save_bytes, fwd_tmp_bytes, bwd_tmp_bytes);
     const pcl_mlp_stack_t q = padded_desc(*d, p, reinterpret_cast<float*>(uintptr_t(4096)), reinterpret_cast<float*>(uintptr_t(4096)));
@@ -343,6 +370,7 @@
 
 extern "C" int pcl_mlp_stack_fwd_f32(const pcl_mlp_stack_t* dp) {
     PCL_TRY(validate(dp, "pcl_mlp_stack_fwd_f32"));
+    PCL_TRY(validate_pitch(dp, "pcl_mlp_stack_fwd_f32"));
     const pcl_mlp_stack_t& d = *dp;
     const PadPlan p = narrow_supported(d) ? PadPlan{} : pad_plan(d);
     if (!p.on) return stack_fwd_impl(dp);
@@ -389,6 +417,7 @@
 
 extern "C" int pcl_mlp_stack_bwd_f32(const pcl_mlp_stack_t* dp) {
     PCL_TRY(validate(dp, "pcl_mlp_stack_bwd_f32"));
+    PCL_TRY(validate_pitch(dp, "pcl_mlp_stack_bwd_f32"));
     const pcl_mlp_stack_t& d = *dp;
     const PadPlan p = narrow_supported(d) ? PadPlan{} : pad_plan(d);
     if (!p.on) return stack_bwd_impl(dp);
@@ -473,6 +502,7 @@
     for (int l = 0; l < L; ++l) {
         const pcl_stack_layer_t& ly = d.layer[l];
         const int cin = d.c[l], cout = d.c[l + 1];
+        const int kin = l == 0 && pitched(d) ? d.x_ld : cin;
         float* Y = s.Y[l];
         int rows;
         if (l == 0 && d.grouped) {
@@ -499,7 +529,7 @@
             rows = pcl_group_linear_stat_rows(d.B, d.m);
         } else if (l == L - 1 && use_gmax(d)) {
             tagf("fwd%dx%d", cin, cout);
-            PCL_TRY(pcl_linear_fwd_gmax_f32(cur, ly.W, ly.bias, in_scale, in_shift, d.slope, P, cin, cout, d.pool, Y, t.stats, t.gmax,
+            PCL_TRY(pcl_linear_fwd_gmax_f32(cur, ly.W, ly.bias, in_scale, in_shift, d.slope, P, kin, cout, d.pool, Y, t.stats, t.gmax,
                                             t.gmin, t.gamax, t.gamin, st));
             rows = pcl_mlp_stat_rows(P, cout, 0);
         } else if (frag_fwd(d)) {
@@ -508,7 +538,7 @@
             rows = pcl_frag_stat_rows(P);
         } else {
             tagf("fwd%dx%d", cin, cout);
-            PCL_TRY(pcl_linear_fwd_rows_f32(cur, ly.W, ly.bias, in_scale, in_shift, d.slope, P, cin, cout, Y, t.stats, rmeta, nrows, st));
+            PCL_TRY(pcl_linear_fwd_rows_f32(cur, ly.W, ly.bias, in_scale, in_shift, d.slope, P, kin, cout, Y, t.stats, rmeta, nrows, st));
             rows = pcl_mlp_stat_rows(P, cout, d.grouped ? 2 : 0);
         }
         float* v = s.vec[l];
@@ -659,6 +689,7 @@
         const float* psc = l > 0 ? s.vec[l - 1] : nullptr;
         const float* psh = l > 0 ? s.vec[l - 1] + cin : nullptr;
         const float* Yl = s.Y[l];
+        const int ldp = l == 0 && pitched(d) ? d.x_ld : 0;
         if (l > 0 && fused_bwd_enabled() && pcl_linear_bwd_fused_supported(cout, cin)) {
             float* dUp = t.dU[cur_du];
             double* stn = t.stats[1 - cur_stats];
@@ -680,8 +711,8 @@
             PCL_REQUIRE(dUp, "pcl_mlp_stack_bwd_f32: need_dx without dx");
             double* stn = l > 0 ? t.stats[1 - cur_stats] : nullptr;
             tagf("pair%dx%d", cout, cin);
-            PCL_TRY(pcl_linear_bwd_pair_f32(dU, Yl, a, k1, k2, mean, sparse ? s.arg : nullptr, sparse ? t.gz : nullptr, ns, ly.W, Xprev, psc, psh, d.slope,
-                                            l > 0 ? 1 : 0, P, cout, cin, dUp, stn, l == 0 ? d.x_grad_from : 0, t.ws, t.ws_bytes, st));
+            PCL_TRY(bwd_pair_impl(dU, Yl, a, k1, k2, mean, sparse ? s.arg : nullptr, sparse ? t.gz : nullptr, ns, ly.W, Xprev, psc, psh, d.slope,
+                                  l > 0 ? 1 : 0, P, cout, cin, dUp, stn, l == 0 ? d.x_grad_from : 0, t.ws, t.ws_bytes, ldp, ldp, st));
             if (l > 0) {
                 const pcl_stack_layer_t& lp = d.layer[l - 1];
                 float* kp = t.consts[1 - cur_c];
@@ -720,15 +751,15 @@
             }
             continue;
         }
-        PCL_TRY(pcl_linear_bwd_dw_rows_f32(dU, Yl, a, k1, k2, mean, sparse ? s.arg : nullptr, sparse ? t.gz : nullptr, ns, Xprev, psc, psh, d.slope,
-                                           P, cout, cin, ly.dW, t.ws, t.ws_bytes, rmeta, nrows, 0, dw_st));
+        PCL_TRY(dw_rows_impl(dU, Yl, a, k1, k2, mean, sparse ? s.arg : nullptr, sparse ? t.gz : nullptr, ns, Xprev, psc, psh, d.slope,
+                             P, cout, cin, ly.dW, t.ws, t.ws_bytes, rmeta, nrows, 0, ldp, dw_st));
         if (l > 0 || d.need_dx) {
             float* dUp = l > 0 ? (sd ? t.dU_l[l - 1] : t.dU[cur_du]) : d.dx;
             PCL_REQUIRE(dUp, "pcl_mlp_stack_bwd_f32: need_dx without dx");
             double* stn = l > 0 ? t.stats[1 - cur_stats] : nullptr;
             tagf("dx%dx%d", cout, cin);
-            PCL_TRY(pcl_linear_bwd_dx_rows_f32(dU, Yl, a, k1, k2, mean, sparse ? s.arg : nullptr, sparse ? t.gz : nullptr, ns, ly.W, P, cout, cin,
-                                               l > 0 ? Xprev : nullptr, psc, psh, d.slope, dUp, stn, rmeta, nrows, l == 0 ? d.x_grad_from : 0, 0, st));
+            PCL_TRY(dx_rows_impl(dU, Yl, a, k1, k2, mean, sparse ? s.arg : nullptr, sparse ? t.gz : nullptr, ns, ly.W, P, cout, cin,
+                                 l > 0 ? Xprev : nullptr, psc, psh, d.slope, dUp, stn, rmeta, nrows, l == 0 ? d.x_grad_from : 0, ldp, ldp, st));
             if (l > 0) {
                 rows = pcl_mlp_stat_rows(P, cin, 1 | (rmeta ? 2 : 0));
                 dU = dUp; sparse = false; cur_du = 1 - cur_du; cur_stats = 1 - cur_stats; cur_c = 1 - cur_c;
diff --git a/pointcloudlib_amd/misc/mlp_hip.py b/pointcloudlib_amd/misc/mlp_hip.py
--- a/pointcloudlib_amd/misc/mlp_hip.py
+++ b/pointcloudlib_amd/misc/mlp_hip.py
@@ -69,6 +69,7 @@
     def forward(ctx, x, cfg, *params):
         ns, slope, eps, momentum, training, bn, last_act, rowset, x_grad_from, link = cfg[:10]
         flush_k = cfg[10] if len(cfg) > 10 else 0
+        W0_padded = cfg[11] if len(cfg) > 11 else None
         L = len(params) // 6
         dev = x.device
         x = x.contiguous()
@@ -88,7 +89,7 @@
             cout = W.shape[0]
             if l == 0 and link is None and W.shape[1] != cin:
                 assert W.shape[1] < cin, f"input has {cin} columns, first layer expects {W.shape[1]}"
-                W = W0p = torch.nn.functional.pad(W.detach(), (0, cin - W.shape[1]))
+                W = W0p = W0_padded if W0_padded is not None else torch.nn.functional.pad(W.detach(), (0, cin - W.shape[1]))
             fused_max = (l == L - 1) and ns in (32, 64) and rowset is None and not flush_k
             folded = l == 0 and link is not None
             flushed = bool(flush_k) and rowset is None and not folded
@@ -551,17 +552,17 @@
 
 class _StackPlan:
     __slots__ = ("desc", "ref", "save_bytes", "fwd_tmp", "bwd_tmp", "G", "cl", "L", "has_bias", "gsizes", "gshapes", "gtotal",
-                 "spec", "grouped", "wide", "off", "P", "c0", "defer", "last_off", "out_slope")
+                 "spec", "grouped", "wide", "off", "P", "c0", "defer", "last_off", "out_slope", "x_ld")
 
 
 _PLANS = {}
 _lib.on_switch_change(_PLANS.clear)
 
 
-def _stack_plan(module, P, c0, pool, grouped, geom, need_dx, x_grad_from, defer=False):
+def _stack_plan(module, P, c0, pool, grouped, geom, need_dx, x_grad_from, defer=False, x_ld=0):
     flush_k = int(getattr(module, "flush_k", 0))
     key = (id(module), P, c0, pool, grouped, geom, need_dx, x_grad_from, module.slope, module.last_act, defer,
-           module.eps, module.momentum, module.biases is not None, flush_k)
+           module.eps, module.momentum, module.biases is not None, flush_k, x_ld)
     plan = _PLANS.get(key)
     if plan is not None and plan.spec is module.spec:
         return plan
@@ -584,6 +585,10 @@
     d.feature = d.Wf_dense = 1
     for l in range(L):
         d.layer[l].W = d.layer[l].gamma = d.layer[l].beta = 1
+    if x_ld:
+        d.x_ld = x_ld
+        if not _lib.lib().pcl_mlp_stack_pitch_supported(ctypes.byref(d)):
+            d.x_ld = 0
     sv, ft, bt = ctypes.c_size_t(), ctypes.c_size_t(), ctypes.c_size_t()
     _lib.check(_lib.lib().pcl_mlp_stack_sizes(ctypes.byref(d), ctypes.byref(sv), ctypes.byref(ft), ctypes.byref(bt)), "pcl_mlp_stack_sizes")
     plan = _StackPlan()
@@ -595,6 +600,7 @@
         _lib.check(_lib.lib().pcl_mlp_stack_last(ctypes.byref(d), ctypes.byref(yo), ctypes.byref(so), ctypes.byref(ho)), "pcl_mlp_stack_last")
         plan.last_off = (yo.value, so.value, ho.value)
     plan.L, plan.cl, plan.spec, plan.grouped, plan.P, plan.c0 = L, spec[L], module.spec, grouped, P, c0
+    plan.x_ld = int(d.x_ld)
     plan.G = (geom[0] * geom[2]) if grouped else (P // pool if pool else 0)
     plan.has_bias = module.biases is not None
     plan.off = 3 if (grouped and geom[4]) else 0
@@ -659,11 +665,15 @@
             d.x = None
         else:
             d.x = t_in.data_ptr()
+            if plan.x_ld:
+                Wf = aux[4]
         for l in range(L):
             ly, q = d.layer[l], params[npl * l:npl * l + npl]
             ly.W, ly.gamma, ly.beta = q[0].data_ptr(), q[1].data_ptr(), q[2].data_ptr()
             ly.bias = q[3].data_ptr() if plan.has_bias else None
             ly.running_mean, ly.running_var = running[2 * l].data_ptr(), running[2 * l + 1].data_ptr()
+        if plan.x_ld:
+            d.layer[0].W = Wf.data_ptr()
         d.out = None if plan.defer else out.data_ptr()
         d.save, d.save_bytes, d.tmp, d.tmp_bytes, d.stream = save.data_ptr(), plan.save_bytes, tmp.data_ptr(), plan.fwd_tmp, st
         _lib.call("pcl_mlp_stack_fwd_f32", ctypes.byref(d), tag="stack_fwd")
@@ -724,6 +734,8 @@
                 grads.append(pieces[k + 3])
             else:
                 ly.dbias = None
+        if plan.x_ld:
+            d.layer[0].W = Wf.data_ptr()
         d.out = None if plan.defer else out.data_ptr()
         d.save, d.save_bytes, d.tmp, d.tmp_bytes = save.data_ptr(), plan.save_bytes, tmp.data_ptr(), plan.bwd_tmp
         d.gout, d.dx, d.stream = gout.data_ptr(), (None if dx is None else dx.data_ptr()), _stream()
@@ -754,6 +766,44 @@
     plan = _stack_plan(module, P, c0, ns, False, None, need_dx, x_grad_from if need_dx else 0)
     ps, running = _stack_params(module)
     return _StackFn.apply(x2, (plan, None, running), *ps)
+
+
+GROUPALL_PITCH = True
+
+
+def pitch_ld(fan_in):
+    return (int(fan_in) + 3) // 4 * 4
+
+
+def groupall_pitch_eligible(module, fan_in, on_gpu=True):
+    return bool(GROUPALL_PITCH and on_gpu and fan_in % 4 != 0 and module.weights[0].shape[1] == fan_in and module.bn and module.training
+                and module.n_layers <= _MAXL and not syncbn.active() and not int(getattr(module, "flush_k", 0)))
+
+
+def groupall_mlp(module, xyz, feature, use_xyz=True):
+    from .ops import group_all_pitched
+    B, N = xyz.shape[0], xyz.shape[1]
+    c0 = (3 if use_xyz else 0) + (0 if feature is None else feature.shape[-1])
+    if not groupall_pitch_eligible(module, c0, xyz.is_cuda and xyz.dtype == torch.float32):
+        return None
+    ld = pitch_ld(c0)
+    need_dx = feature is not None and feature.requires_grad and torch.is_grad_enabled()
+    x_from = (3 if use_xyz else 0) if need_dx else 0
+    plan = _stack_plan(module, B * N, c0, N, False, None, need_dx, x_from, x_ld=ld)
+    if not plan.x_ld:
+        return None
+    rows, Wp = group_all_pitched(xyz, feature, module.weights[0], use_xyz, ld)
+    if USE_STACK:
+        ps, running = _stack_params(module)
+        out = _StackFn.apply(rows, (plan, None, running, None, Wp), *ps)
+    else:
+        params = []
+        for i in range(module.n_layers):
+            params += [module.weights[i], None if module.biases is None else module.biases[i], module.gammas[i], module.betas[i],
+                       getattr(module, f"running_mean_{i}"), getattr(module, f"running_var_{i}")]
+        cfg = (N, module.slope, module.eps, module.momentum, module.training, module.bn, module.last_act, None, x_from, None, 0, Wp)
+        out = _FusedMLP.apply(rows, cfg, *params)
+    return out.reshape(B, 1, out.shape[-1])
 
 
 class DeferLink:
diff --git a/pointcloudlib_amd/misc/ops.py b/pointcloudlib_amd/misc/ops.py
--- a/pointcloudlib_amd/misc/ops.py
+++ b/pointcloudlib_amd/misc/ops.py
@@ -8,7 +8,7 @@
 from .. import _lib
 
 __all__ = [
-    "optimal_block", "furthest_point_sample", "ball_query", "ball_query_multi", "group_offsets_multi", "group_points", "group_points_compact", "RowSet", "group_all",
+    "optimal_block", "furthest_point_sample", "ball_query", "ball_query_multi", "group_offsets_multi", "group_points", "group_points_compact", "RowSet", "group_all", "group_all_pitched",
     "index_points",
     "knn_indices", "edge_features", "three_nn", "three_interpolate", "row_offsets", "pack_rows", "unpack_rows", "interpolate_pack",
     "row_cloud", "packed_layout", "segment_max", "mlp_segment_max", "broadcast_rows",
@@ -277,6 +277,38 @@
         return None, gfeat, None
 
 
+class _GroupAllPitch(torch.autograd.Function):
+
+    @staticmethod
+    def forward(ctx, xyz, feat, W0, use_xyz, ld):
+        xyz = _dev(xyz, "xyz")
+        feat = _dev(feat, "feature")
+        W0 = _dev(W0, "weight")
+        B, N, _ = xyz.shape
+        C = 0 if feat is None else feat.shape[2]
+        rows = torch.empty((B * N, ld), dtype=torch.float32, device=xyz.device)
+        Wp = torch.empty((W0.shape[0], ld), dtype=torch.float32, device=xyz.device)
+        _lib.call("pcl_group_all_pitch_f32", _p(xyz), _p(feat), B, N, C, int(use_xyz), ld, _p(rows), _p(W0), W0.shape[0], _p(Wp), _stream())
+        ctx.dims = (B, N, C, 3 if use_xyz else 0)
+        ctx.mark_non_differentiable(Wp)
+        ctx.set_materialize_grads(False)
+        return rows, Wp
+
+    @staticmethod
+    def backward(ctx, grows, _gwp):
+        B, N, C, off = ctx.dims
+        if C == 0 or not ctx.needs_input_grad[1] or grows is None:
+            return None, None, None, None, None
+        return None, grows.reshape(B, N, grows.shape[-1])[:, :, off:off + C], None, None, None
+
+
+def group_all_pitched(xyz, feature, W0, use_xyz=True, ld=None):
+    D = (3 if use_xyz else 0) + (0 if feature is None else feature.shape[-1])
+    if ld is None:
+        ld = (D + 3) // 4 * 4
+    return _GroupAllPitch.apply(xyz, feature, W0.detach(), bool(use_xyz), int(ld))
+
+
 class RowSet:
 
     def __init__(self, B, m, ns, row_meta, row_src, group_off):
diff --git a/pointcloudlib_amd/networks/cls/pointnet2.py b/pointcloudlib_amd/networks/cls/pointnet2.py
--- a/pointcloudlib_amd/networks/cls/pointnet2.py
+++ b/pointcloudlib_amd/networks/cls/pointnet2.py
@@ -55,8 +55,14 @@
         new_feature_list = []
         for grouper, mlp, ic in zip(self.groupers, self.mlps, idxs):
             if ic is None:
-                grouped = grouper(new_xyz, xyz, feature)
-                new_feature_list.append(mlp(grouped, group_max=grouped.shape[2]))
+                out = None
+                if mlp.resolved_backend(xyz) == "hip":
+                    from ...misc import mlp_hip
+                    out = mlp_hip.groupall_mlp(mlp, xyz, feature, grouper.use_xyz)
+                if out is None:
+                    grouped = grouper(new_xyz, xyz, feature)
+                    out = mlp(grouped, group_max=grouped.shape[2])
+                new_feature_list.append(out)
             elif self.compact_duplicates and mlp.resolved_backend(xyz) == "hip":
                 new_feature_list.append(mlp.forward_grouped(xyz, new_xyz, feature, ic[0], ic[1], ic[2], grouper.use_xyz))
             else:
```

Measured after the change: 18620 point-clouds/s (median of 6 runs). About the same (+0.9%).
